# A-SHOJAEI/preference-guided-image-captioning-alignment

Measured on AMD Instinct MI355X. Metric: DPO preference-pairs/sec, CLIP-ViT-B/32+GPT-2-M seq128, higher is better.
Workload: dtype bf16; 1 GPU; Stage-2 DPO step, 4-forward policy/reference x chosen/rejected, openai/clip-vit-base-patch32 (frozen) + gpt2-medium decoder, seq_len 128, beta 0.1, bf16 MFMA / f32 accumulate+master, AdamW+clip; pairs_per_gpu=512, seq_len=128, parallelism=dp1, grad_allreduce=none (1 GPU)

## Files before the change

### include/pgca_hip.h

```cpp
#ifndef PGCA_HIP_H
#define PGCA_HIP_H

#include <stddef.h>
#include <stdint.h>

#ifdef __cplusplus
extern "C" {
#endif

typedef enum pgca_status {
  PGCA_OK = 0,
  PGCA_ERR_INVALID = -1,
  PGCA_ERR_LAUNCH = -2
} pgca_status;

#define PGCA_ABI_VERSION 306
int pgca_version(void);
int pgca_sizeof_gemm_args(void);
const char* pgca_last_error(void);

enum { PGCA_NT = 0, PGCA_NN = 1, PGCA_TN = 2 };

enum {
  PGCA_EPI_NONE = 0,
  PGCA_EPI_GELU_NEW = 1,
  PGCA_EPI_QUICK_GELU = 2,
  PGCA_EPI_RELU = 3,
  PGCA_EPI_TANH = 4,
  PGCA_EPI_DGELU_NEW = 5,
  PGCA_EPI_DRELU = 6,
  PGCA_EPI_DTANH = 7,
  PGCA_EPI_ROWSTATS = 8,
  PGCA_EPI_DLOGITS = 9,
  PGCA_EPI_DQUICK_GELU = 10,
  PGCA_EPI_GELU_NEW_D = 11,
  PGCA_EPI_MUL_AUX = 12
};

typedef struct pgca_gemm_args {
  const void* A;
  const void* B;
  int32_t M, N, K;
  int32_t lda, ldb;
  int32_t layout;
  int32_t epilogue;
  float alpha;
  const float* bias;
  void* out_bf16;
  int32_t ld_out_bf16;
  float* out_f32;
  int32_t ld_out_f32;
  int32_t accumulate;
  const float* residual;
  int32_t ld_res;
  void* aux_out;
  const void* aux_in;
  int32_t ld_aux;
  const int64_t* targets;
  float* stat_max;
  float* stat_sum;
  int32_t stat_ld;
  float* target_val;
  const float* row_lse;
  const float* row_scale;
  int32_t out_cols;
  uint32_t drop_seed;
  uint32_t drop_threshold;
  float drop_scale;
  float* colsum_part;
  int32_t ld_colsum;
  const int32_t* drop_rows;
} pgca_gemm_args;

int pgca_gemm_bf16(const pgca_gemm_args* args, void* stream);
int pgca_gemm_plan(const pgca_gemm_args* args);
int pgca_set_option(const char* name, int32_t value);
int pgca_gemm_bf16_grouped(const pgca_gemm_args* args, int32_t count, void* stream);

#define PGCA_SKINNY_MAX_M 64
typedef struct pgca_skinny_args {
  const void* x;
  const void* W;
  int32_t M, N, K, lda, ldw;
  float* scratch;
  const float* bias;
  int32_t act;
  const float* residual;
  int32_t ld_res;
  float* out_f32;
  int32_t ld_out_f32;
  void* out_bf16;
  int32_t ld_out_bf16;
  const float* ln_gamma;
  const float* ln_beta;
  float ln_eps;
  void* ln_out_bf16;
  int32_t ld_ln;
} pgca_skinny_args;
int pgca_gemm_skinny(const pgca_skinny_args* args, void* stream);
int64_t pgca_gemm_skinny_workspace(int32_t M, int32_t N, int32_t K);
int pgca_sizeof_skinny_args(void);

int pgca_rowstats_combine(const float* stat_max, const float* stat_sum, int32_t stat_ld, int32_t nparts,
                          const float* target_val, int32_t M, float* lse, float* out_logprob, void* stream);

int pgca_layernorm_fwd(const float* x, const int32_t* row_map, int32_t M, int32_t H, const float* gamma,
                       const float* beta, float eps, void* y_bf16, float* y_f32, float* mean, float* rstd,
                       void* stream);

int pgca_layernorm_bwd_blocks(int32_t M);
int pgca_layernorm_bwd(const void* dy_bf16, const float* dy_f32, const float* x, const int32_t* row_map,
                       int32_t M, int32_t H, const float* gamma, const float* mean, const float* rstd,
                       const float* add_to, float* dx_out, void* dx_bf16, float* part, float* part_extra,
                       const uint32_t* drop_add, const uint32_t* drop_dx, const int32_t* drop_rows, void* stream);
int pgca_colsum_finish(const float* part, int32_t nparts, int32_t H, float* out, int32_t accumulate, void* stream);

int pgca_colsum_finish4(const float* part, int32_t nplanes, int32_t nparts, int32_t H, float* out0, float* out1,
                        float* out2, float* out3, int32_t accumulate, void* stream);

int pgca_colsum_blocks(int32_t M);
int pgca_colsum(const void* x_bf16, const float* x_f32, int32_t M, int32_t N, int32_t ld, float* part, void* stream);

#define PGCA_ATTN_MAX_S 512
int pgca_attention_fwd(const void* qkv, const int32_t* key_mask, int32_t B, int32_t S, int32_t heads,
                       int32_t causal, void* out, float* lse, uint32_t drop_seed, uint32_t drop_threshold,
                       float drop_scale, const int32_t* cu_seqlens, void* stream);
int pgca_attention_bwd(const void* qkv, const void* out, const void* dout, const float* lse,
                       const int32_t* key_mask, int32_t B, int32_t S, int32_t heads, int32_t causal,
                       void* dqkv, uint32_t drop_seed, uint32_t drop_threshold, float drop_scale,
                       const int32_t* cu_seqlens, void* stream);
#define PGCA_ATTN_SPLIT_MAX_S 1024
int pgca_attention_bwd_split(const void* qkv, const void* out, const void* dout, const float* lse,
                             const int32_t* key_mask, int32_t B, int32_t S, int32_t heads, int32_t causal,
                             void* dqkv, uint32_t drop_seed, uint32_t drop_threshold, float drop_scale,
                             const int32_t* cu_seqlens, void* stream);

int pgca_embed_fwd(const int64_t* ids, int32_t B, int32_t S, int32_t H, const float* wte, const float* wpe,
                   const float* attended, const float* gamma, const float* beta, float eps, float* h0,
                   float* mean, float* rstd, int32_t att_stride, const float* U, int32_t xheads,
                   const uint32_t* drop_x, const uint32_t* drop_e, const int32_t* row_ids, int32_t n_rows,
                   void* stream);
int pgca_embed_bwd(const float* g, const int64_t* ids, const int32_t* row_mask, int32_t B, int32_t S, int32_t H,
                   const float* wte, const float* attended, const float* gamma, const float* mean,
                   const float* rstd, float* dwte, float* dwpe, float* dattended, float* part, int32_t att_stride,
                   const float* U, float* dU, int32_t xheads, const uint32_t* drop_x, const uint32_t* drop_e,
                   const int32_t* cu_seqlens, void* stream);
int pgca_embed_bwd_blocks(int32_t B, int32_t S);

int pgca_patchify(const float* pixels, int32_t B, int32_t image, int32_t patch, int32_t ld_out, void* out_bf16,
                  void* stream);
int pgca_vit_assemble(const float* patch_embeds, const float* cls, const float* pos, int32_t B, int32_t T,
                      int32_t H, float* x, void* stream);
int pgca_vit_assemble_bwd(const float* dx, int32_t B, int32_t T, int32_t H, void* dpatch_bf16, float* dcls,
                          float* dpos, void* stream);

int pgca_image_preprocess(const uint8_t* images, int32_t B, int32_t H, int32_t W, int32_t S, const int32_t* xbounds,
                          const int32_t* xcoef, int32_t xk, const int32_t* ybounds, const int32_t* ycoef, int32_t yk,
                          float mean0, float mean1, float mean2, float std0, float std1, float std2, uint8_t* tmp,
                          uint8_t* resized_u8, float* out, void* stream);

int pgca_image_train_transform(const uint8_t* images, int32_t B, int32_t H, int32_t W, int32_t S, const int32_t* params,
                               const float* factors, const int32_t* xbounds, const int32_t* xcoef, int32_t xk,
                               const int32_t* ybounds, const int32_t* ycoef, int32_t yk, float mean0, float mean1,
                               float mean2, float std0, float std1, float std2, uint8_t* tmp, uint8_t* resized_u8,
                               uint8_t* aug_u8, float* out, void* stream);

int pgca_seq_reduce(const float* tok_lp, const int32_t* seq_of_row, int32_t nrows, int32_t nseq,
                    const int32_t* seq_count, int32_t mode, float* seq_lp, void* stream);
int pgca_logits_logprob(const float* logits, int32_t ld, int32_t V, const int32_t* row_map, const int64_t* targets,
                        int32_t R, float* out, void* stream);
int pgca_logits_logprob_bwd(const float* logits, int32_t ld, int32_t V, const int32_t* row_map, const int64_t* targets,
                            const float* g, int32_t R, float* dlogits, void* stream);
int pgca_dpo_loss(const float* pol_w, const float* pol_l, const float* ref_w, const float* ref_l, int32_t B,
                  float beta, float label_smoothing, float* loss, float* dpol_w, float* dpol_l, float* metrics,
                  void* stream);
int pgca_seq_batch_prepare(const int64_t* ids, const int64_t* mask, int32_t Bq, int32_t S, int32_t* counts,
                           int32_t* mask32, int32_t* row_map, int64_t* targets, int32_t* seq_of_row, int32_t* n_rows,
                           void* stream);
int pgca_seq_pack_prepare(int32_t* mask32, int32_t Bq, int32_t S, int32_t pad_to, int32_t* lens, int32_t* cu,
                          int32_t* row_ids, int32_t* n_packed, const int32_t* counts, int32_t* row_map, void* stream);
int pgca_row_scale(const float* dseq, const int32_t* seq_of_row, const int32_t* seq_count, int32_t nrows,
                   int32_t mode, float* row_scale, void* stream);

int pgca_masked_mean_fwd(const float* feats, const int32_t* mask, int32_t B, int32_t S, int32_t H, float* pooled,
                         const int32_t* cu_seqlens, void* stream);
int pgca_masked_mean_bwd(const float* dpooled, const int32_t* mask, int32_t B, int32_t S, int32_t H,
                         float* dfeats, const int32_t* cu_seqlens, void* stream);
int pgca_l2norm_fwd(const float* x, int32_t B, int32_t P, float* y, float* norm, void* stream);
int pgca_l2norm_bwd(const float* dy, const float* y, const float* norm, int32_t B, int32_t P, float* dx,
                    void* stream);
int pgca_ntxent_loss(const float* lse_r, const float* lse_c, const float* diag, int32_t n_local, int32_t n_total,
                     float* loss, void* stream);

int pgca_sqnorm_blocks(int64_t n);
int pgca_sqnorm(const float* g, int64_t n, float* part, void* stream);
int pgca_step_control(const float* part, int32_t nparts, float max_norm, float base_lr, int32_t warmup,
                      int32_t total_steps, int32_t sched_stride, float beta1, float beta2, float grad_scale,
                      const float* gate, float* ctrl, void* stream);
int pgca_clip_coef(const float* part, int32_t nparts, float max_norm, float* coef, void* stream);
int pgca_scale_dev(float* x, int64_t n, const float* coef, void* stream);
int pgca_adamw(float* p, const float* g, float* m, float* v, void* p_bf16, int64_t n, const float* ctrl,
               float weight_decay, float beta1, float beta2, float eps, float grad_scale, void* stream);
int pgca_cast_bf16(const float* x, void* y_bf16, int64_t n, void* stream);
int pgca_cast_f32(const void* x_bf16, float* y, int64_t n, void* stream);
int pgca_split_bf16(const float* x, int32_t R, int32_t P, int32_t rows_out, int32_t pattern, void* y_bf16,
                    void* stream);
int pgca_axpy(const float* x, float alpha, float* y, int64_t n, int32_t accumulate, void* stream);
int pgca_gather_rows_bf16(const void* src, const int32_t* row_map, int32_t M, int32_t H, void* dst, void* stream);

int pgca_select_token(const float* logits, int32_t ld, int32_t V, int32_t R, const int64_t* prev, int32_t ld_prev,
                      int32_t n_prev, float repetition_penalty, float temperature, int32_t top_k, float top_p,
                      const float* u, const uint8_t* done, int64_t pad_id, int64_t* next, float* next_logp,
                      void* stream);
int pgca_select_beam_candidates(const float* logits, int32_t ld, int32_t V, int32_t B, int32_t nb, const int64_t* prev,
                                int32_t ld_prev, int32_t n_prev, float repetition_penalty, int32_t warp,
                                float temperature, int32_t top_k, float top_p, const float* beam_scores, int32_t K,
                                int32_t use_noise, uint32_t noise_seed, float* cand_score, int64_t* cand_index,
                                void* stream);
typedef struct pgca_select_opts {
  int32_t no_repeat_ngram_size;
  int32_t n_ban;
  const int64_t* ban_ids;
} pgca_select_opts;
int pgca_sizeof_select_opts(void);
int pgca_select_token_ex(const float* logits, int32_t ld, int32_t V, int32_t R, const int64_t* prev, int32_t ld_prev,
                         int32_t n_prev, float repetition_penalty, float temperature, int32_t top_k, float top_p,
                         const float* u, const uint8_t* done, int64_t pad_id, int64_t* next, float* next_logp,
                         const pgca_select_opts* opts, void* stream);
int pgca_select_beam_candidates_ex(const float* logits, int32_t ld, int32_t V, int32_t B, int32_t nb,
                                   const int64_t* prev, int32_t ld_prev, int32_t n_prev, float repetition_penalty,
                                   int32_t warp, float temperature, int32_t top_k, float top_p,
                                   const float* beam_scores, int32_t K, int32_t use_noise, uint32_t noise_seed,
                                   float* cand_score, int64_t* cand_index, const pgca_select_opts* opts, void* stream);
int pgca_beam_step(const float* cand_score, const int64_t* cand_index, int32_t B, int32_t nb, int32_t V, int32_t cur,
                   int32_t L, int64_t eos, float length_penalty, int32_t early_stopping, const int64_t* running_in,
                   int64_t* running_out, float* running_beam_scores, const int64_t* sequences_in,
                   int64_t* sequences_out, float* beam_scores, uint8_t* is_sent_finished, int64_t* gen_len,
                   uint8_t* unsat, int64_t* tok, int64_t* flat_src, uint8_t* hits_all, void* stream);

#ifdef __cplusplus
}
#endif
#endif
```

### preference-guided-image-captioning-alignment_amd/csrc/gemm.hip

```cpp
#include <string>

#include "gemm_device.h"

namespace {

template <int LA, int LB>
__global__ __launch_bounds__(256, 2) void gemm_kernel(const pgca_gemm_args a, int ntm, int ntn) {
  __shared__ __attribute__((aligned(16))) unsigned char smem[2][2][TILE_BYTES];

  int tm, tn;
  group_m_tile(xcd_remap(blockIdx.x, ntm * ntn), ntm, ntn, tm, tn);
  const int m0 = tm * BM, n0 = tn * BN;

  const int t = threadIdx.x;
  const int lane = t & 63, wave = t >> 6;
  const int wm = wave >> 1, wn = wave & 1;

  const bf16_t* A = reinterpret_cast<const bf16_t*>(a.A);
  const bf16_t* B = reinterpret_cast<const bf16_t*>(a.B);

  Stage<LA> sa;
  Stage<LB> sb;
  sa.init(t, a.lda, m0, LA == 0 ? a.M : ((a.M + 7) & ~7));
  sb.init(t, a.ldb, n0, LB == 0 ? a.N : ((a.N + 7) & ~7));
  const bf16_t* abase = LA == 0 ? A + (size_t)m0 * a.lda : A + m0;
  const bf16_t* bbase = LB == 0 ? B + (size_t)n0 * a.ldb : B + n0;
  const size_t astep = LA == 0 ? (size_t)BK : (size_t)BK * a.lda;
  const size_t bstep = LB == 0 ? (size_t)BK : (size_t)BK * a.ldb;

  f32x4 acc[4][4];
#pragma unroll
  for (int i = 0; i < 4; ++i)
#pragma unroll
    for (int j = 0; j < 4; ++j) acc[i][j] = (f32x4){0.f, 0.f, 0.f, 0.f};

  const int nk = (a.K + BK - 1) / BK;
  u32x4 ra[4], rb[4];
  sa.load(abase, a.K, ra);
  sb.load(bbase, a.K, rb);
  sa.store(smem[0][0], ra);
  sb.store(smem[0][1], rb);
  __syncthreads();

  for (int kt = 0; kt < nk; ++kt) {
    const int cur = kt & 1;
    const bool more = (kt + 1) < nk;
    if (more) {
      sa.load(abase + (size_t)(kt + 1) * astep, a.K - (kt + 1) * BK, ra);
      sb.load(bbase + (size_t)(kt + 1) * bstep, a.K - (kt + 1) * BK, rb);
    }
    const unsigned char* la = smem[cur][0];
    const unsigned char* lb = smem[cur][1];
#pragma unroll
    for (int kk = 0; kk < 2; ++kk) {
      bf16x8 fa[4], fb[4];
#pragma unroll
      for (int i = 0; i < 4; ++i) fa[i] = read_frag<LA>(la, wm * 64, i, kk, lane);
#pragma unroll
      for (int j = 0; j < 4; ++j) fb[j] = read_frag<LB>(lb, wn * 64, j, kk, lane);
#pragma unroll
      for (int i = 0; i < 4; ++i)
#pragma unroll
        for (int j = 0; j < 4; ++j)
          acc[i][j] = __builtin_amdgcn_mfma_f32_16x16x32_bf16(fa[i], fb[j], acc[i][j], 0, 0, 0);
    }
    if (more) {
      sa.store(smem[cur ^ 1][0], ra);
      sb.store(smem[cur ^ 1][1], rb);
    }
    __syncthreads();
  }

  run_epilogue(a, acc, &smem[0][0][0], m0 + wm * 64, n0 + wn * 64, lane, wave);
}

__global__ void rowstats_combine_kernel(const float* __restrict__ smax, const float* __restrict__ ssum, int stat_ld,
                                        int nparts, const float* __restrict__ tval, int M, float* __restrict__ lse,
                                        float* __restrict__ out_lp) {
  const int row = blockIdx.x * (blockDim.x >> 6) + (threadIdx.x >> 6);
  const int lane = threadIdx.x & 63;
  if (row >= M) return;
  float mx = -INFINITY;
  for (int i = lane; i < nparts; i += 64) mx = fmaxf(mx, smax[(size_t)row * stat_ld + i]);
  mx = wave_max(mx);
  float s = 0.f;
  for (int i = lane; i < nparts; i += 64) {
    const float pm = smax[(size_t)row * stat_ld + i];
    if (pm > -INFINITY) s += ssum[(size_t)row * stat_ld + i] * __expf(pm - mx);
  }
  s = wave_sum(s);
  if (lane == 0) {
    const float l = mx + __logf(s);
    if (lse) lse[row] = l;
    if (out_lp) out_lp[row] = tval[row] - l;
  }
}


template <int LA, int LB, bool RAW = false>
__device__ __forceinline__ void gemm256_body(const pgca_gemm_args& a, int ntm, int ntn, int nk_per_split, int bid_in,
                                             int ksplit, unsigned char* smem2) {
  int tm, tn;
  if (RAW) {
    tm = bid_in / ntn;
    tn = bid_in - tm * ntn;
  } else {
    group_m_tile(xcd_remap(bid_in, ntm * ntn), ntm, ntn, tm, tn);
  }
  const int m0 = tm * BM2, n0 = tn * BN2;

  const int t = threadIdx.x;
  const int lane = t & 63;
  const int wave = __builtin_amdgcn_readfirstlane(t >> 6);
  const int wm = wave >> 2, wn = wave & 3;

  const bf16_t* A = reinterpret_cast<const bf16_t*>(a.A);
  const bf16_t* B = reinterpret_cast<const bf16_t*>(a.B);

  Dma<LA, BK> da;
  Dma<LB, BK> db;
  da.init(lane, wave, a.lda, m0, LA == 0 ? a.M : ((a.M + 7) & ~7));
  db.init(lane, wave, a.ldb, n0, LB == 0 ? a.N : ((a.N + 7) & ~7));
  const bf16_t* abase = LA == 0 ? A + (size_t)m0 * a.lda : A + m0;
  const bf16_t* bbase = LB == 0 ? B + (size_t)n0 * a.ldb : B + n0;
  const size_t astep = LA == 0 ? (size_t)BK : (size_t)BK * a.lda;
  const size_t bstep = LB == 0 ? (size_t)BK : (size_t)BK * a.ldb;

  f32x4 acc[2][4][4];
#pragma unroll
  for (int h = 0; h < 2; ++h)
#pragma unroll
    for (int i = 0; i < 4; ++i)
#pragma unroll
      for (int j = 0; j < 4; ++j) acc[h][i][j] = (f32x4){0.f, 0.f, 0.f, 0.f};

  const int kt0 = ksplit * nk_per_split;
  const int nk = min(nk_per_split, a.K / BK - kt0);
  abase += (size_t)kt0 * astep;
  bbase += (size_t)kt0 * bstep;
#ifdef PGCA_GEMM_TIMING
  unsigned long long ts0, ts1, ts2, ts3;
#endif
  TSTAMP(ts0);
  da.issue(abase, smem2, wave);
  db.issue(bbase, smem2 + TILE2_BYTES, wave);
  dma_wait();
  __syncthreads();
  TSTAMP(ts1);

  for (int kt = 0; kt < nk; ++kt) {
    const int cur = kt & 1;
    if (kt + 1 < nk) {
      unsigned char* nxt = smem2 + (cur ^ 1) * 2 * TILE2_BYTES;
      da.issue(abase + (size_t)(kt + 1) * astep, nxt, wave);
      db.issue(bbase + (size_t)(kt + 1) * bstep, nxt + TILE2_BYTES, wave);
    }
    const unsigned char* la = smem2 + cur * 2 * TILE2_BYTES;
    const unsigned char* lb = la + TILE2_BYTES;
#pragma unroll
    for (int kk = 0; kk < 2; ++kk) {
      bf16x8 fb[4];
#pragma unroll
      for (int j = 0; j < 4; ++j) fb[j] = read_frag<LB, 512>(lb, wn * 64, j, kk, lane);
      mma_half<LA>(la, wm * 128, kk, lane, fb, acc[0]);
      mma_half<LA>(la, wm * 128 + 64, kk, lane, fb, acc[1]);
    }
    dma_wait();
    __syncthreads();
  }

  TSTAMP(ts2);
  run_epilogue(a, acc[0], smem2, m0 + wm * 128, n0 + wn * 64, lane, wave);
  run_epilogue(a, acc[1], smem2, m0 + wm * 128 + 64, n0 + wn * 64, lane, wave);
#ifdef PGCA_GEMM_TIMING
  dma_wait();
  TSTAMP(ts3);
  if (a.stat_max && a.epilogue != PGCA_EPI_ROWSTATS && lane == 0) {
    float* o = a.stat_max + ((size_t)blockIdx.x * 8 + wave) * 8;
    o[0] = (float)(ts1 - ts0); o[1] = (float)(ts2 - ts1); o[2] = (float)(ts3 - ts2); o[3] = (float)nk;
  }
#endif
}

template <int LA, int LB>
__global__ __launch_bounds__(512, 2) void gemm256_kernel(const pgca_gemm_args a, int ntm, int ntn, int nk_per_split) {
  extern __shared__ __attribute__((aligned(16))) unsigned char smem2[];
  gemm256_body<LA, LB>(a, ntm, ntn, nk_per_split, blockIdx.x, blockIdx.y, smem2);
}

struct pgca_group_param {
  pgca_gemm_args a[4];
  int start[5];
  int ntm[4], ntn[4];
};

__global__ __launch_bounds__(512, 2) void gemm256_group_tn_kernel(const pgca_group_param gp) {
  extern __shared__ __attribute__((aligned(16))) unsigned char smem2[];
  const int b = xcd_remap(blockIdx.x, gp.start[4]);
  int p = 0;
  if (b >= gp.start[1]) p = 1;
  if (b >= gp.start[2]) p = 2;
  if (b >= gp.start[3]) p = 3;
#define PGCA_SEL(F) (p == 0 ? gp.a[0].F : p == 1 ? gp.a[1].F : p == 2 ? gp.a[2].F : gp.a[3].F)
  pgca_gemm_args a = {};
  a.A = PGCA_SEL(A);
  a.B = PGCA_SEL(B);
  a.M = PGCA_SEL(M);
  a.N = PGCA_SEL(N);
  a.K = PGCA_SEL(K);
  a.lda = PGCA_SEL(lda);
  a.ldb = PGCA_SEL(ldb);
  a.out_f32 = PGCA_SEL(out_f32);
  a.ld_out_f32 = PGCA_SEL(ld_out_f32);
  a.alpha = PGCA_SEL(alpha);
  a.accumulate = PGCA_SEL(accumulate);
  a.layout = PGCA_TN;
  a.epilogue = PGCA_EPI_NONE;
#undef PGCA_SEL
  const int ntm = p == 0 ? gp.ntm[0] : p == 1 ? gp.ntm[1] : p == 2 ? gp.ntm[2] : gp.ntm[3];
  const int ntn = p == 0 ? gp.ntn[0] : p == 1 ? gp.ntn[1] : p == 2 ? gp.ntn[2] : gp.ntn[3];
  const int st = p == 0 ? gp.start[0] : p == 1 ? gp.start[1] : p == 2 ? gp.start[2] : gp.start[3];
  const int l = b - st;
  int tm, tn;
  if (ntm <= ntn) {
    tn = l / ntm;
    tm = l - tn * ntm;
  } else {
    tm = l / ntn;
    tn = l - tm * ntn;
  }
  gemm256_body<1, 1, true>(a, ntm, ntn, a.K / BK, tm * ntn + tn, 0, smem2);
}

constexpr size_t GEMM256_LDS = 4 * TILE2_BYTES;

int plan_variant(const pgca_gemm_args& a) {
  const int forced = gemm_tuning().schedule;
  if (forced >= 0) return forced == 6 ? 6 : 0;
  return a.layout == PGCA_TN ? 0 : 6;
}

}

namespace pgca {
GemmTuning& gemm_tuning() {
  static GemmTuning t = [] {
    auto env = [](const char* name, int dflt) {
      const char* e = getenv(name);
      return e ? atoi(e) : dflt;
    };
    GemmTuning v;
    v.tile = env("PGCA_GEMM_TILE", 0);
    v.schedule = env("PGCA_GEMM_RING", -1);
    v.group = env("PGCA_GEMM_NO_GROUP", 0) ? 0 : 1;
    v.stagger = env("PGCA_GEMM_STAGGER", 0);
    v.pair_order = 0;
    return v;
  }();
  return t;
}

GemmPlan plan_gemm(const pgca_gemm_args& a) {
  GemmPlan p;
  p.ncols = a.epilogue == PGCA_EPI_DLOGITS ? a.out_cols : a.N;
  const int ntm2 = (a.M + BM2 - 1) / BM2, ntn2 = (p.ncols + BN2 - 1) / BN2;
  const int force = gemm_tuning().tile;
  const int nk_total = a.K / BK;
  int splits = 1;
  const bool splittable = a.epilogue == PGCA_EPI_NONE && a.accumulate && a.out_f32 && !a.out_bf16 && !a.bias &&
                          !a.residual;
  if (splittable && ntm2 * ntn2 > 0 && ntm2 * ntn2 < 192) {
    splits = 256 / (ntm2 * ntn2);
    if (splits > nk_total / 8) splits = nk_total / 8;
    if (splits > 16) splits = 16;
    if (splits < 1) splits = 1;
  }
  const bool want256 = force ? force == 256 : (ntm2 * ntn2 * splits >= 192);
  if ((a.K % BK) == 0 && want256 && a.M >= 8 && p.ncols >= 8) {
    p.tile = 256;
    p.variant = plan_variant(a);
    p.splits = splits;
    p.ntm = ntm2;
    p.ntn = ntn2;
    p.nk_per_split = (nk_total + splits - 1) / splits;
    p.grid_y = (nk_total + p.nk_per_split - 1) / p.nk_per_split;
  } else {
    p.tile = 128;
    p.variant = 0;
    p.splits = p.grid_y = 1;
    p.ntm = (a.M + BM - 1) / BM;
    p.ntn = (p.ncols + BN - 1) / BN;
    p.nk_per_split = (a.K + BK - 1) / BK;
  }
  return p;
}
}

extern "C" int pgca_set_option(const char* name, int32_t value) {
  if (!name) {
    set_error("pgca_set_option: null name");
    return PGCA_ERR_INVALID;
  }
  GemmTuning& t = gemm_tuning();
  const std::string n(name);
  if (n == "gemm_tile" && (value == 0 || value == 128 || value == 256)) t.tile = value;
  else if (n == "gemm_schedule" && (value == -1 || value == 0 || value == 6)) t.schedule = value;
  else if (n == "gemm_group" && (value == 0 || value == 1)) t.group = value;
  else if (n == "gemm_stagger" && value >= 0 && value <= 64) t.stagger = value;
  else if (n == "gemm_pair_order" && (value == 0 || value == 1)) t.pair_order = value;
  else {
    set_error("pgca_set_option: unknown option or value out of range (%s = %d)", name, value);
    return PGCA_ERR_INVALID;
  }
  return PGCA_OK;
}

extern "C" int pgca_gemm_plan(const pgca_gemm_args* args) {
  const GemmPlan p = plan_gemm(*args);
  if (p.tile != 256) return 12801;
  return p.variant * 1000000 + 25600 + p.splits;
}

static int check_gemm_args(const pgca_gemm_args& a) {
  if (!a.A || !a.B || a.M <= 0 || a.N <= 0 || a.K <= 0) {
    set_error("pgca_gemm_bf16: null operand or empty shape (M=%d N=%d K=%d)", a.M, a.N, a.K);
    return PGCA_ERR_INVALID;
  }
  if ((a.lda & 7) || (a.ldb & 7) || ((uintptr_t)a.A & 15) || ((uintptr_t)a.B & 15)) {
    set_error("pgca_gemm_bf16: lda/ldb must be multiples of 8 and operands 16-B aligned (lda=%d ldb=%d)", a.lda,
              a.ldb);
    return PGCA_ERR_INVALID;
  }
  const bool a_kcontig = a.layout != PGCA_TN, b_kcontig = a.layout == PGCA_NT;
  if ((a_kcontig || b_kcontig) && (a.K & 7)) {
    set_error("pgca_gemm_bf16: K=%d must be a multiple of 8 for K-contiguous operands", a.K);
    return PGCA_ERR_INVALID;
  }
  if (a_kcontig ? a.lda < a.K : a.lda < ((a.M + 7) & ~7)) {
    set_error("pgca_gemm_bf16: lda=%d too small", a.lda);
    return PGCA_ERR_INVALID;
  }
  if (b_kcontig ? a.ldb < a.K : a.ldb < ((a.N + 7) & ~7)) {
    set_error("pgca_gemm_bf16: ldb=%d too small", a.ldb);
    return PGCA_ERR_INVALID;
  }
  if (a.epilogue == PGCA_EPI_ROWSTATS) {
    if (!a.stat_max || !a.stat_sum || a.stat_ld < 2 * ((a.N + BN - 1) / BN)) {
      set_error("pgca_gemm_bf16: ROWSTATS needs stat buffers with stat_ld >= %d", 2 * ((a.N + BN - 1) / BN));
      return PGCA_ERR_INVALID;
    }
  } else if (a.epilogue == PGCA_EPI_DLOGITS) {
    if (!a.row_lse || !a.row_scale || !a.targets || !a.out_bf16 || a.out_cols < a.N || a.ld_out_bf16 < a.out_cols) {
      set_error("pgca_gemm_bf16: DLOGITS needs row_lse,row_scale,targets,out_bf16 and out_cols >= N");
      return PGCA_ERR_INVALID;
    }
  } else {
    if (!a.out_bf16 && !a.out_f32) {
      set_error("pgca_gemm_bf16: no output buffer");
      return PGCA_ERR_INVALID;
    }
    if (((a.epilogue >= PGCA_EPI_DGELU_NEW && a.epilogue <= PGCA_EPI_DTANH) || a.epilogue == PGCA_EPI_DQUICK_GELU ||
         a.epilogue == PGCA_EPI_MUL_AUX) &&
        !a.aux_in) {
      set_error("pgca_gemm_bf16: derivative epilogue needs aux_in");
      return PGCA_ERR_INVALID;
    }
  }
  if (a.colsum_part && ((a.epilogue != PGCA_EPI_DGELU_NEW && a.epilogue != PGCA_EPI_MUL_AUX) || a.ld_colsum < a.N ||
                        a.accumulate == 2)) {
    set_error("pgca_gemm_bf16: colsum_part needs the DGELU_NEW / MUL_AUX epilogue, ld_colsum >= N and no split-K");
    return PGCA_ERR_INVALID;
  }
  return PGCA_OK;
}

extern "C" int pgca_gemm_bf16(const pgca_gemm_args* args, void* stream) {
  const pgca_gemm_args& a = *args;
  if (const int rc = check_gemm_args(a)) return rc;
  const GemmPlan p = plan_gemm(a);
  hipStream_t s = (hipStream_t)stream;
  if (p.tile == 128)
    return with_layout(a.layout, [&](auto la, auto lb) {
      hipLaunchKernelGGL((gemm_kernel<decltype(la)::value, decltype(lb)::value>), dim3(p.ntm * p.ntn), dim3(256), 0, s,
                         a, p.ntm, p.ntn);
      return check_launch("pgca_gemm_bf16");
    });
  pgca_gemm_args b = a;
  if (p.splits > 1) b.accumulate = 2;
  if (p.variant == 6) return launch_gemm256s(b, p, stream);
  return with_layout(a.layout, [&](auto la, auto lb) {
    constexpr auto kernel = gemm256_kernel<decltype(la)::value, decltype(lb)::value>;
    if (raise_lds_limit<kernel>(GEMM256_LDS, "gemm256")) return (int)PGCA_ERR_LAUNCH;
    hipLaunchKernelGGL(kernel, dim3(p.ntm * p.ntn, p.grid_y), dim3(512), GEMM256_LDS, s, b, p.ntm, p.ntn,
                       p.nk_per_split);
    return check_launch("pgca_gemm_bf16(256)");
  });
}

extern "C" int pgca_gemm_bf16_grouped(const pgca_gemm_args* args, int32_t count, void* stream) {
  if (!args || count <= 0) {
    set_error("pgca_gemm_bf16_grouped: no problems");
    return PGCA_ERR_INVALID;
  }
  if (count == 2 && gemm_tuning().group) {
    const pgca_gemm_args &a = args[0], &b = args[1];
    const bool alike = (a.layout == PGCA_NT || a.layout == PGCA_NN) && b.layout == a.layout && a.M == b.M &&
                       a.N == b.N && a.K == b.K && a.epilogue != PGCA_EPI_DLOGITS && b.epilogue != PGCA_EPI_DLOGITS;
    const GemmPlan pa = alike ? plan_gemm(a) : GemmPlan{}, pb = alike ? plan_gemm(b) : GemmPlan{};
    if (alike && pa.tile == 256 && pb.tile == 256 && pa.splits == 1 && pb.splits == 1 && pa.variant == 6 &&
        pb.variant == 6) {
      for (int i = 0; i < 2; ++i) {
        const int rc = check_gemm_args(args[i]);
        if (rc) return rc;
      }
      return launch_gemm256s_pair(a, b, pa, stream);
    }
  }
  bool groupable = count <= 4 && gemm_tuning().group;
  for (int i = 0; i < count && groupable; ++i) {
    const pgca_gemm_args& a = args[i];
    groupable = a.layout == PGCA_TN && (a.K % BK) == 0 && a.M >= 8 && a.N >= 8 && a.epilogue == PGCA_EPI_NONE &&
                a.out_f32 && !a.out_bf16 && !a.bias && !a.residual && !a.drop_threshold &&
                check_gemm_args(a) == PGCA_OK;
  }
  if (!groupable) {
    for (int i = 0; i < count; ++i) {
      const int rc = pgca_gemm_bf16(&args[i], stream);
      if (rc) return rc;
    }
    return PGCA_OK;
  }
  if (raise_lds_limit<gemm256_group_tn_kernel>(GEMM256_LDS, "gemm256")) return PGCA_ERR_LAUNCH;
  pgca_group_param gp;
  int total = 0;
  for (int i = 0; i < 4; ++i) {
    if (i < count) {
      gp.a[i] = args[i];
      gp.ntm[i] = (args[i].M + BM2 - 1) / BM2;
      gp.ntn[i] = (args[i].N + BN2 - 1) / BN2;
      gp.start[i] = total;
      total += gp.ntm[i] * gp.ntn[i];
    } else {
      gp.a[i] = args[count - 1];
      gp.ntm[i] = gp.ntn[i] = 1;
      gp.start[i] = 0x7fffffff;
    }
  }
  gp.start[4] = total;
  hipLaunchKernelGGL(gemm256_group_tn_kernel, dim3(total), dim3(512), GEMM256_LDS, (hipStream_t)stream, gp);
  return check_launch("pgca_gemm_bf16_grouped");
}

extern "C" int pgca_rowstats_combine(const float* stat_max, const float* stat_sum, int32_t stat_ld, int32_t nparts,
                                     const float* target_val, int32_t M, float* lse, float* out_logprob,
                                     void* stream) {
  if (!stat_max || !stat_sum || M <= 0 || nparts <= 0 || (out_logprob && !target_val)) {
    set_error("pgca_rowstats_combine: bad arguments");
    return PGCA_ERR_INVALID;
  }
  hipLaunchKernelGGL(rowstats_combine_kernel, dim3((M + 3) / 4), dim3(256), 0, (hipStream_t)stream, stat_max,
                     stat_sum, stat_ld, nparts, target_val, M, lse, out_logprob);
  return check_launch("pgca_rowstats_combine");
}
```

### preference-guided-image-captioning-alignment_amd/csrc/gemm_device.h

```cpp
#pragma once
#include <stdlib.h>

#include <type_traits>

#include "common.h"

namespace pgca {
struct GemmPlan {
  int tile;
  int variant;
  int splits;
  int ntm, ntn;
  int nk_per_split;
  int grid_y;
  int ncols;
};
GemmPlan plan_gemm(const pgca_gemm_args& a);
int launch_gemm256s(const pgca_gemm_args& a, const GemmPlan& p, void* stream);
int launch_gemm256s_pair(const pgca_gemm_args& a0, const pgca_gemm_args& a1, const GemmPlan& p, void* stream);

struct GemmTuning {
  int tile;
  int schedule;
  int group;
  int pair_order;
  int stagger;
};
GemmTuning& gemm_tuning();
}

using namespace pgca;

namespace {

template <typename F>
int with_layout(int layout, F&& f) {
  using S0 = std::integral_constant<int, 0>;
  using S1 = std::integral_constant<int, 1>;
  switch (layout) {
    case PGCA_NT: return f(S0{}, S0{});
    case PGCA_NN: return f(S0{}, S1{});
    case PGCA_TN: return f(S1{}, S1{});
    default: set_error("pgca_gemm_bf16: unknown layout %d", layout); return PGCA_ERR_INVALID;
  }
}

template <auto KERNEL>
int raise_lds_limit(size_t bytes, const char* what) {
  static const bool ok = hipFuncSetAttribute((const void*)KERNEL, hipFuncAttributeMaxDynamicSharedMemorySize,
                                             (int)bytes) == hipSuccess;
  if (!ok) {
    (void)hipGetLastError();
    set_error("%s: cannot raise dynamic LDS limit", what);
    return PGCA_ERR_LAUNCH;
  }
  return PGCA_OK;
}

constexpr int BM = 128, BN = 128, BK = 64;
constexpr int TILE_BYTES = 128 * 64 * 2;
constexpr int BM2 = 256, BN2 = 256;
constexpr int TILE2_BYTES = 256 * 64 * 2;
constexpr unsigned OOB = 0x80000000u;

__device__ __forceinline__ int xcd_remap(int b, int total) {
  const int xcd = b & 7, q = total >> 3, r = total & 7;
  return (xcd < r ? xcd * (q + 1) : r * (q + 1) + (xcd - r) * q) + (b >> 3);
}
constexpr int GROUP_M = 8;
__device__ __forceinline__ void group_m_tile(int bid, int ntm, int ntn, int& tm, int& tn) {
  const int per_group = GROUP_M * ntn;
  const int group = bid / per_group;
  const int first_m = group * GROUP_M;
  const int gsize = min(GROUP_M, ntm - first_m);
  const int in_group = bid - group * per_group;
  tm = first_m + in_group % gsize;
  tn = in_group / gsize;
}

#define PGCA_CLOCK(insn, v) asm volatile(insn " %0\n\ts_waitcnt lgkmcnt(0)" : "=s"(v)::"memory")
#ifdef PGCA_GEMM_TIMING
#define TSTAMP(v) PGCA_CLOCK("s_memtime", v)
#define TSTAMP_REAL(v) PGCA_CLOCK("s_memrealtime", v)
#else
#define TSTAMP(v)
#define TSTAMP_REAL(v)
#endif
#ifdef PGCA_GEMM_TIMING2
#define PSTAMP(v) PGCA_CLOCK("s_memtime", v)
#else
#define PSTAMP(v)
#endif

__device__ __forceinline__ __amdgpu_buffer_rsrc_t make_rsrc(const void* p) {
  return __builtin_amdgcn_make_buffer_rsrc(const_cast<void*>(p), 0, 0x7ffffff0, 0x00020000);
}

template <int KS>
struct Stage {
  unsigned goff[4];
  unsigned loff[4];
  bool vspace[4];
  int kpos[4];

  __device__ __forceinline__ void init(int t, int ld, int origin, int extent) {
    if (KS == 0) {
      const int r = t >> 3, c = t & 7;
#pragma unroll
      for (int i = 0; i < 4; ++i) {
        const int row = r + 32 * i;
        goff[i] = (unsigned)(row * ld + c * 8) * 2u;
        loff[i] = (unsigned)(row * 128 + ((c ^ (row & 7)) << 4));
        vspace[i] = (origin + row) < extent;
        kpos[i] = c * 8;
      }
    } else {
      const int kr = t >> 4, c16 = t & 15;
#pragma unroll
      for (int i = 0; i < 4; ++i) {
        const int k = kr + 16 * i;
        const int h = (k & 3) | (((k >> 3) & 1) << 2);
        goff[i] = (unsigned)(k * ld + c16 * 8) * 2u;
        loff[i] = (unsigned)(k * 256 + (((c16 >> 1) ^ h) << 5) + ((c16 & 1) << 4));
        vspace[i] = (origin + c16 * 8) < extent;
        kpos[i] = k;
      }
    }
  }
  __device__ __forceinline__ void load(const bf16_t* base, int krem, u32x4 (&r)[4]) const {
    __amdgpu_buffer_rsrc_t rs = make_rsrc(base);
#pragma unroll
    for (int i = 0; i < 4; ++i) {
      const bool ok = vspace[i] && (kpos[i] < krem);
      r[i] = __builtin_amdgcn_raw_buffer_load_b128(rs, ok ? goff[i] : OOB, 0, 0);
    }
  }
  __device__ __forceinline__ void store(unsigned char* lds, const u32x4 (&r)[4]) const {
#pragma unroll
    for (int i = 0; i < 4; ++i) *reinterpret_cast<u32x4*>(lds + loff[i]) = r[i];
  }
};

template <int KS, int KSTRIDE = 256>
__device__ __forceinline__ bf16x8 read_frag(const unsigned char* lds, int wbase, int sub, int kk, int lane) {
  if (KS == 0) {
    const int row = wbase + sub * 16 + (lane & 15);
    const int c = kk * 4 + (lane >> 4);
    return *reinterpret_cast<const bf16x8*>(lds + row * 128 + ((c ^ (lane & 7)) << 4));
  } else {
    const int g = lane >> 4, q = (lane & 15) >> 2, p = lane & 3;
    const int k = kk * 32 + 8 * g + q;
    const int h = q | ((g & 1) << 2);
    const int s32 = (wbase >> 4) + sub;
    const unsigned char* a0 = lds + k * KSTRIDE + ((s32 ^ h) << 5) + 8 * p;
    return tr_frag(a0, a0 + 4 * KSTRIDE);
  }
}

}

#include "gemm_epilogue.h"

namespace {

__device__ __forceinline__ int swz4p(int q) { return (0x78 >> (2 * q)) & 3; }

template <int KS, int BKT>
struct Dma {
  static constexpr int NP = BKT / 16;
  unsigned goff[NP];
  __device__ __forceinline__ void init(int lane, int wave, int ld, int origin, int extent) {
#pragma unroll
    for (int i = 0; i < NP; ++i) {
      const int j = wave * NP + i;
      if (KS == 0) {
        const int r = BKT == 64 ? 8 * j + (lane >> 3) : 16 * j + (lane >> 2);
        const int c = BKT == 64 ? (lane & 7) ^ (lane >> 3) : (lane & 3) ^ swz4p((lane >> 4) & 3);
        const int rg = min(origin + r, extent - 1) - origin;
        goff[i] = (unsigned)(rg * ld + c * 8) * 2u;
      } else {
        const int k = 2 * j + (lane >> 5);
        const int c16 = lane & 31;
        const int h = (k & 3) | (((k >> 3) & 1) << 2);
        const int col = (((c16 >> 1) ^ h) << 4) + ((c16 & 1) << 3);
        const int cg = min(origin + col, extent - 8) - origin;
        goff[i] = (unsigned)(k * ld + cg) * 2u;
      }
    }
  }
  __device__ __forceinline__ void issue(const bf16_t* base, unsigned char* tile, int wave) const {
    const unsigned long long b = (unsigned long long)base;
    u32x4 rs;
    rs[0] = (unsigned)b;
    rs[1] = (unsigned)(b >> 32) & 0xffffu;
    rs[2] = 0x7ffffff0u;
    rs[3] = 0x00020000u;
    const unsigned lds0 = (unsigned)(size_t)LDS_PTR(tile) + (unsigned)wave * (NP * 1024u);
#pragma unroll
    for (int i = 0; i < NP; ++i) {
      if constexpr (BKT == 64) {
        asm volatile("s_nop 4\n\ts_mov_b32 m0, %0\n\ts_nop 0\n\tbuffer_load_dwordx4 %1, %2, 0 offen lds"
                     :
                     : "s"(lds0 + i * 1024u), "v"(goff[i]), "s"(rs)
                     : "memory");
      } else {
        asm volatile("s_mov_b32 m0, %0\n\ts_nop 0\n\tbuffer_load_dwordx4 %1, %2, 0 offen lds"
                     :
                     : "s"(lds0 + i * 1024u), "v"(goff[i]), "s"(rs)
                     : "memory");
      }
    }
  }
};

__device__ __forceinline__ void dma_wait() { asm volatile("s_waitcnt vmcnt(0)" ::: "memory"); }

template <int LA>
__device__ __forceinline__ void mma_half(const unsigned char* la, int row0, int kk, int lane, const bf16x8 (&fb)[4],
                                         f32x4 (&acc)[4][4]) {
  bf16x8 fa[4];
#pragma unroll
  for (int i = 0; i < 4; ++i) fa[i] = read_frag<LA, 512>(la, row0, i, kk, lane);
#pragma unroll
  for (int i = 0; i < 4; ++i)
#pragma unroll
    for (int j = 0; j < 4; ++j) acc[i][j] = __builtin_amdgcn_mfma_f32_16x16x32_bf16(fa[i], fb[j], acc[i][j], 0, 0, 0);
}

}
```

### preference-guided-image-captioning-alignment_amd/csrc/gemm_pair.hip

```cpp
#include "gemm_phase_body.h"

namespace {

struct pgca_pair_param {
  pgca_gemm_args a[2];
  int ntm, ntn, nk, stagger;
  int order;
};

template <int LA, int LB>
__global__ __launch_bounds__(512, 2) void gemm256s_pair_kernel(const pgca_pair_param gp) {
  extern __shared__ __attribute__((aligned(16))) unsigned char smems[];
  const int ntm = gp.ntm, ntn = gp.ntn, nwg = ntm * ntn;
  const int b = xcd_remap(blockIdx.x, 2 * nwg);
  int p, bid;
  if (gp.order == 0) {
    p = b >= nwg;
    bid = b - (p ? nwg : 0);
  } else {
    const int per_group = GROUP_M * ntn;
    const int g = b / (2 * per_group);
    const int size = min(GROUP_M, ntm - g * GROUP_M) * ntn;
    const int rem = b - g * 2 * per_group;
    p = rem >= size;
    bid = g * per_group + rem - (p ? size : 0);
  }
  p = __builtin_amdgcn_readfirstlane(p);
  bid = __builtin_amdgcn_readfirstlane(bid);
  const char* kernarg = (const char*)__builtin_amdgcn_kernarg_segment_ptr();
  const pgca_gemm_args a = *(const pgca_gemm_args*)(kernarg + offsetof(pgca_pair_param, a) +
                                                    (p ? sizeof(pgca_gemm_args) : 0));
  if (a.epilogue > PGCA_EPI_TANH && a.epilogue != PGCA_EPI_GELU_NEW_D) return;
  gemm256s_body<LA, LB>(a, ntm, ntn, gp.nk, gp.stagger, bid, smems);
}

}

int pgca::launch_gemm256s_pair(const pgca_gemm_args& a0, const pgca_gemm_args& a1, const GemmPlan& p, void* stream) {
  auto forward_epilogue = [](int e) { return (e >= PGCA_EPI_NONE && e <= PGCA_EPI_TANH) || e == PGCA_EPI_GELU_NEW_D; };
  if (!forward_epilogue(a0.epilogue) || !forward_epilogue(a1.epilogue)) {
    const int rc = launch_gemm256s(a0, p, stream);
    return rc ? rc : launch_gemm256s(a1, p, stream);
  }
  pgca_pair_param gp;
  gp.a[0] = a0;
  gp.a[1] = a1;
  gp.ntm = p.ntm;
  gp.ntn = p.ntn;
  gp.nk = p.nk_per_split;
  gp.stagger = 2 * p.ntm * p.ntn >= 3 * 256 ? gemm_tuning().stagger : 0;
  gp.order = gemm_tuning().pair_order;
  auto launch = [&](auto lb) {
    constexpr auto kernel = gemm256s_pair_kernel<0, decltype(lb)::value>;
    if (raise_lds_limit<kernel>(GEMM256S_LDS, "gemm256s pair")) return (int)PGCA_ERR_LAUNCH;
    hipLaunchKernelGGL(kernel, dim3(2 * p.ntm * p.ntn), dim3(512), GEMM256S_LDS, (hipStream_t)stream, gp);
    return check_launch("pgca_gemm_bf16_grouped(256 phase-staggered pair)");
  };
  return a0.layout == PGCA_NT ? launch(std::integral_constant<int, 0>{}) : launch(std::integral_constant<int, 1>{});
}
```

### preference-guided-image-captioning-alignment_amd/csrc/gemm_phase.hip

```cpp
#include "gemm_phase_body.h"

namespace {

template <int LA, int LB>
__global__ __launch_bounds__(512, 2) void gemm256s_kernel(const pgca_gemm_args a, int ntm, int ntn, int nk_per_split,
                                                          int stagger) {
  extern __shared__ __attribute__((aligned(16))) unsigned char smems[];
  gemm256s_body<LA, LB>(a, ntm, ntn, nk_per_split, stagger, xcd_remap(blockIdx.x, ntm * ntn), smems);
}

}

int pgca::launch_gemm256s(const pgca_gemm_args& a, const GemmPlan& p, void* stream) {
  return with_layout(a.layout, [&](auto la, auto lb) {
    constexpr auto kernel = gemm256s_kernel<decltype(la)::value, decltype(lb)::value>;
    if (raise_lds_limit<kernel>(GEMM256S_LDS, "gemm256s")) return (int)PGCA_ERR_LAUNCH;
    const int stagger = (p.ntm * p.ntn >= 3 * 256 && p.grid_y == 1) ? gemm_tuning().stagger : 0;
    hipLaunchKernelGGL(kernel, dim3(p.ntm * p.ntn, p.grid_y), dim3(512), GEMM256S_LDS, (hipStream_t)stream, a, p.ntm,
                       p.ntn, p.nk_per_split, stagger);
    return check_launch("pgca_gemm_bf16(256 phase-staggered)");
  });
}
```

### preference-guided-image-captioning-alignment_amd/csrc/gemm_phase_body.h

```cpp
#pragma once
#include <stddef.h>

#include "gemm_device.h"

namespace {

constexpr int PBK = 32, PSTAGES = 4;
constexpr int PTILE_BYTES = 256 * PBK * 2;

template <int KS>
using DmaP = Dma<KS, PBK>;

template <int KS>
__device__ __forceinline__ bf16x8 read_frag_p(const unsigned char* lds, int wbase, int sub, int lane) {
  if (KS == 0) {
    const int row = wbase + sub * 16 + (lane & 15);
    const int pos = (lane >> 4) ^ swz4p((lane >> 2) & 3);
    return *reinterpret_cast<const bf16x8*>(lds + row * 64 + pos * 16);
  } else {
    return read_frag<1, 512>(lds, wbase, sub, 0, lane);
  }
}


template <int N>
__device__ __forceinline__ void wait_vm_p() {
  asm volatile("s_waitcnt vmcnt(%0)" ::"n"(N) : "memory");
}

#ifndef PGCA_FILL_L
#define PGCA_FILL_L 0
#endif
#ifndef PGCA_FILL_M
#define PGCA_FILL_M 0
#endif
template <int N>
__device__ __forceinline__ void valu_fill(float (&d)[8]) {
#pragma unroll
  for (int i = 0; i < N; ++i) asm volatile("v_fmac_f32 %0, %1, %1" : "+v"(d[i & 7]) : "v"(d[(i + 3) & 7]));
}
#define PGCA_PBAR()                       \
  do {                                    \
    __builtin_amdgcn_sched_barrier(0);    \
    __builtin_amdgcn_s_barrier();         \
    __builtin_amdgcn_sched_barrier(0);    \
  } while (0)

template <int LA, int LB>
__device__ __forceinline__ void gemm256s_body(const pgca_gemm_args& a, int ntm, int ntn, int nk_per_split, int stagger,
                                              int bid, unsigned char* smems) {
#ifdef PGCA_GEMM_TIMING
  unsigned long long ts0, ts1, ts2, ts3, tr0, tr3;
#endif
  TSTAMP(ts0);
  TSTAMP_REAL(tr0);

  if (stagger > 0 && gridDim.y == 1 && blockIdx.x < 256) {
    const int slot = (blockIdx.x >> 3) & 3;
    for (int i = 0; i < slot * stagger; ++i) __builtin_amdgcn_s_sleep(16);
  }

  int tm, tn;
  group_m_tile(bid, ntm, ntn, tm, tn);
  const int m0 = tm * BM2, n0 = tn * BN2;

  const int t = threadIdx.x;
  const int lane = t & 63;
  const int wave = __builtin_amdgcn_readfirstlane(t >> 6);
  const int wm = wave >> 2, wn = wave & 3;

  const bf16_t* A = reinterpret_cast<const bf16_t*>(a.A);
  const bf16_t* B = reinterpret_cast<const bf16_t*>(a.B);

  DmaP<LA> da;
  DmaP<LB> db;
  da.init(lane, wave, a.lda, m0, LA == 0 ? a.M : ((a.M + 7) & ~7));
  db.init(lane, wave, a.ldb, n0, LB == 0 ? a.N : ((a.N + 7) & ~7));
  const bf16_t* abase = LA == 0 ? A + (size_t)m0 * a.lda : A + m0;
  const bf16_t* bbase = LB == 0 ? B + (size_t)n0 * a.ldb : B + n0;
  const size_t astep = LA == 0 ? (size_t)PBK : (size_t)PBK * a.lda;
  const size_t bstep = LB == 0 ? (size_t)PBK : (size_t)PBK * a.ldb;

  f32x4 acc[2][4][4];
#pragma unroll
  for (int h = 0; h < 2; ++h)
#pragma unroll
    for (int i = 0; i < 4; ++i)
#pragma unroll
      for (int j = 0; j < 4; ++j) acc[h][i][j] = (f32x4){0.f, 0.f, 0.f, 0.f};

  const int kt0 = blockIdx.y * nk_per_split * 2;
  const int nk = min(nk_per_split * 2, a.K / PBK - kt0);
  abase += (size_t)kt0 * astep;
  bbase += (size_t)kt0 * bstep;

  da.issue(abase, smems, wave);
  db.issue(bbase, smems + PTILE_BYTES, wave);
  da.issue(abase + astep, smems + 2 * PTILE_BYTES, wave);
  db.issue(bbase + bstep, smems + 3 * PTILE_BYTES, wave);
  if (2 < nk) {
    da.issue(abase + 2 * astep, smems + 4 * PTILE_BYTES, wave);
    wait_vm_p<6>();
  } else {
    wait_vm_p<4>();
  }
  PGCA_PBAR();
  PGCA_PBAR();
  if (wm == 1) PGCA_PBAR();

  TSTAMP(ts1);
#ifdef PGCA_GEMM_TIMING2
  unsigned long long q0 = 0, q1 = 0, q2 = 0, q3 = 0, q4 = 0, q5 = 0, q6 = 0, q7 = 0, q8 = 0;
  unsigned long long aL0 = 0, aB1 = 0, aM0 = 0, aB2 = 0, aL1 = 0, aB3 = 0, aM1 = 0, aB4 = 0;
#endif
  float fill[8] = {1.f, 2.f, 3.f, 4.f, 5.f, 6.f, 7.f, 8.f};
  for (int kt = 0; kt < nk; ++kt) {
    PSTAMP(q0);
    const unsigned char* la = smems + (kt & 3) * 2 * PTILE_BYTES;
    const unsigned char* lb = la + PTILE_BYTES;
    bf16x8 fa[4], fb[4];
#pragma unroll
    for (int j = 0; j < 4; ++j) fb[j] = read_frag_p<LB>(lb, wn * 64, j, lane);
#pragma unroll
    for (int i = 0; i < 4; ++i) fa[i] = read_frag_p<LA>(la, wm * 128, i, lane);
    __builtin_amdgcn_sched_barrier(0);
    if (kt >= 1 && kt + 2 < nk) db.issue(bbase + (size_t)(kt + 2) * bstep, smems + ((kt + 2) & 3) * 2 * PTILE_BYTES + PTILE_BYTES, wave);
    if (kt == 0 && 2 < nk) db.issue(bbase + 2 * bstep, smems + 5 * PTILE_BYTES, wave);
    if (PGCA_FILL_L) valu_fill<PGCA_FILL_L>(fill);
    PSTAMP(q1);
    PGCA_PBAR();
    asm volatile("s_waitcnt lgkmcnt(0)" ::: "memory");
    __builtin_amdgcn_sched_barrier(0);
    PSTAMP(q2);
    __builtin_amdgcn_s_setprio(1);
#pragma unroll
    for (int i = 0; i < 4; ++i)
#pragma unroll
      for (int j = 0; j < 4; ++j) {
        acc[0][i][j] = __builtin_amdgcn_mfma_f32_16x16x32_bf16(fa[i], fb[j], acc[0][i][j], 0, 0, 0);
        if (PGCA_FILL_M) valu_fill<PGCA_FILL_M>(fill);
      }
    __builtin_amdgcn_s_setprio(0);
    PSTAMP(q3);
    PGCA_PBAR();
    PSTAMP(q4);
#pragma unroll
    for (int i = 0; i < 4; ++i) fa[i] = read_frag_p<LA>(la, wm * 128 + 64, i, lane);
    __builtin_amdgcn_sched_barrier(0);
    if (kt + 3 < nk) {
      da.issue(abase + (size_t)(kt + 3) * astep, smems + ((kt + 3) & 3) * 2 * PTILE_BYTES, wave);
      wait_vm_p<6>();
    } else if (kt + 2 < nk) {
      wait_vm_p<4>();
    } else {
      wait_vm_p<0>();
    }
    if (PGCA_FILL_L) valu_fill<PGCA_FILL_L>(fill);
    PSTAMP(q5);
    PGCA_PBAR();
    asm volatile("s_waitcnt lgkmcnt(0)" ::: "memory");
    __builtin_amdgcn_sched_barrier(0);
    PSTAMP(q6);
    __builtin_amdgcn_s_setprio(1);
#pragma unroll
    for (int i = 0; i < 4; ++i)
#pragma unroll
      for (int j = 0; j < 4; ++j) {
        acc[1][i][j] = __builtin_amdgcn_mfma_f32_16x16x32_bf16(fa[i], fb[j], acc[1][i][j], 0, 0, 0);
        if (PGCA_FILL_M) valu_fill<PGCA_FILL_M>(fill);
      }
    __builtin_amdgcn_s_setprio(0);
    PSTAMP(q7);
    PGCA_PBAR();
    PSTAMP(q8);
#ifdef PGCA_GEMM_TIMING2
    aL0 += q1 - q0; aB1 += q2 - q1; aM0 += q3 - q2; aB2 += q4 - q3;
    aL1 += q5 - q4; aB3 += q6 - q5; aM1 += q7 - q6; aB4 += q8 - q7;
#endif
  }
#ifdef PGCA_GEMM_TIMING2
  if (a.stat_sum && a.epilogue != PGCA_EPI_ROWSTATS && lane == 0) {
    float* o = a.stat_sum + ((size_t)blockIdx.x * 8 + wave) * 8;
    const float inv = 1.f / (float)nk;
    o[0] = aL0 * inv; o[1] = aB1 * inv; o[2] = aM0 * inv; o[3] = aB2 * inv;
    o[4] = aL1 * inv; o[5] = aB3 * inv; o[6] = aM1 * inv; o[7] = aB4 * inv;
  }
#endif
  if (PGCA_FILL_L || PGCA_FILL_M) {
    if (fill[0] + fill[1] + fill[2] + fill[3] + fill[4] + fill[5] + fill[6] + fill[7] == 12345.678f) acc[0][0][0][0] += 1.f;
  }
  if (wm == 0) PGCA_PBAR();
  __syncthreads();

  TSTAMP(ts2);
  run_epilogue(a, acc[0], smems, m0 + wm * 128, n0 + wn * 64, lane, wave);
  run_epilogue(a, acc[1], smems, m0 + wm * 128 + 64, n0 + wn * 64, lane, wave);
#ifdef PGCA_GEMM_TIMING
  dma_wait();
  TSTAMP(ts3);
  if (a.stat_max && a.epilogue != PGCA_EPI_ROWSTATS && lane == 0) {
    float* o = a.stat_max + ((size_t)blockIdx.x * 8 + wave) * 8;
    o[0] = (float)(ts1 - ts0); o[1] = (float)(ts2 - ts1); o[2] = (float)(ts3 - ts2); o[3] = (float)(nk / 2);
    o[4] = (float)(ts0 & 0xFFFFFFFull); o[5] = (float)(ts3 & 0xFFFFFFFull);
    TSTAMP_REAL(tr3);
    o[6] = (float)(ts3 - ts0); o[7] = (float)(tr3 - tr0);
  }
#endif
}

constexpr size_t GEMM256S_LDS = (size_t)2 * PSTAGES * PTILE_BYTES;

}
```

### preference-guided-image-captioning-alignment_amd/engine.py

```python
from __future__ import annotations

import logging
import math
import os
from contextlib import contextmanager
from dataclasses import dataclass
from types import SimpleNamespace
from typing import Dict, List, Optional, Tuple

import torch

from . import hip
from .arch import GptArch, ModelArch, VitArch
from .params import ParamStore, Segment, VOCAB_TILE

logger = logging.getLogger(__name__)

F32, BF16, I32, I64 = torch.float32, torch.bfloat16, torch.int32, torch.int64
ATTN_BWD_MAX_S = 1024
ATTN_BWD_ONEPASS_MAX_S = 512


def attention_backward(qkv, out, dout, lse, key_mask, B, S, heads, causal, dqkv, drop=None, cu=None):
    fn = hip.attention_bwd if S <= ATTN_BWD_ONEPASS_MAX_S else hip.attention_bwd_split
    fn(qkv, out, dout, lse, key_mask, B, S, heads, causal, dqkv, drop=drop, cu=cu)


class Workspace:

    GROW = 1.125

    def __init__(self, device):
        self.device = torch.device(device)
        self.bufs: Dict[str, torch.Tensor] = {}
        self._stamps: Dict[str, tuple] = {}
        self.serial: Dict[str, int] = {}
        self._recorders: List[set] = []

    def _touch(self, key: str, fresh: bool) -> None:
        if fresh:
            self.serial[key] = self.serial.get(key, 0) + 1
        for r in self._recorders:
            r.add(key)

    def get(self, key: str, shape, dtype, zero: bool = False) -> torch.Tensor:
        shape = tuple(int(s) for s in shape)
        n = 1
        for s in shape:
            n *= s
        t = self.bufs.get(key)
        fresh = t is None or t.dtype != dtype or t.numel() < n
        if fresh:
            grow = t is not None and t.dtype == dtype
            t = torch.empty(max(int(n * self.GROW) if grow else n, 1), dtype=dtype, device=self.device)
            self.bufs[key] = t
        self._touch(key, fresh)
        v = t[:n].view(shape)
        if zero:
            v.zero_()
        return v

    def cached(self, key: str, stamp: tuple, make) -> torch.Tensor:
        fresh = key not in self.bufs or self._stamps.get(key) != stamp
        if fresh:
            self.bufs[key] = make()
            self._stamps[key] = stamp
        self._touch(key, fresh)
        return self.bufs[key]

    @contextmanager
    def recording(self):
        keys: set = set()
        self._recorders.append(keys)
        try:
            yield keys
        finally:
            self._recorders.remove(keys)

    def stamp(self, keys) -> tuple:
        return tuple((k, self.serial.get(k, 0)) for k in sorted(keys))

    def nbytes(self) -> int:
        return sum(t.numel() * t.element_size() for t in self.bufs.values())


KIND_EMBD, KIND_ATTN, KIND_RESID_ATTN, KIND_RESID_MLP, KIND_VPROJ, KIND_XATTN, KIND_HEAD = range(7)
TOWER_DECODER, TOWER_TEXT, TOWER_VHEAD, TOWER_THEAD = range(4)
_M32 = 0xFFFFFFFF


def _hash32(x: int) -> int:
    x &= _M32
    x ^= x >> 16
    x = (x * 0x7FEB352D) & _M32
    x ^= x >> 15
    x = (x * 0x846CA68B) & _M32
    x ^= x >> 16
    return x


class DropoutPlan:

    GPT_KINDS = (KIND_EMBD, KIND_ATTN, KIND_RESID_ATTN, KIND_RESID_MLP)

    def __init__(self, p: float = 0.0, base_seed: int = 0, p_gpt: Optional[float] = None):
        self.p, self.base_seed, self.step, self.active = float(p), int(base_seed), 0, True
        self.p_gpt = float(p) if p_gpt is None else float(p_gpt)

    def _p(self, kind: int) -> float:
        return self.p_gpt if kind in self.GPT_KINDS else self.p

    def _site(self, step: int, tower: int, layer: int, kind: int):
        seed = _hash32(_hash32(self.base_seed * 0x9E3779B1 + step) ^ ((tower << 24) | ((layer & 0xFFFF) << 8) | kind))
        return hip.drop_args(seed, self._p(kind))

    @property
    def on(self) -> bool:
        return self.active and (self.p > 0.0 or self.p_gpt > 0.0)

    def site(self, tower: int, layer: int, kind: int):
        if not self.on:
            return None
        return self._site(self.step, tower, layer, kind)

    def bind(self, tower: int):
        if not self.on:
            return None
        step = self.step
        return lambda layer, kind: self._site(step, tower, layer, kind)


PACK_PAD = 64


@dataclass
class RowPack:
    cu: torch.Tensor
    row_ids: torch.Tensor
    mask: torch.Tensor
    lens: torch.Tensor
    n: int
    Mp: int
    Bq: int
    S: int

    @property
    def nseq(self) -> int:
        return self.Bq + n_filler_seqs(self.S)


def n_filler_seqs(S: int) -> int:
    return (PACK_PAD - 1 + S - 1) // S


@dataclass
class SeqBatch:
    ids: torch.Tensor
    mask: torch.Tensor
    row_map: torch.Tensor
    targets: torch.Tensor
    seq_of_row: torch.Tensor
    counts: torch.Tensor
    n_rows: int
    Bq: int
    S: int
    pack: Optional[RowPack] = None
    row_map_packed: Optional[torch.Tensor] = None


class PendingRowPack:

    def __init__(self, mask1, lens, cu, row_ids, n_host, event, Bq, S):
        self._f, self._n, self._ev, self.Bq, self.S = (mask1, lens, cu, row_ids), n_host, event, Bq, S

    def result(self) -> RowPack:
        self._ev.synchronize()
        n, Mp = int(self._n[0]), int(self._n[1])
        mask1, lens, cu, row_ids = self._f
        return RowPack(cu=cu, row_ids=row_ids[:max(Mp, 1)], mask=mask1, lens=lens, n=n, Mp=Mp, Bq=self.Bq, S=self.S)


def _issue_pack(mask1: torch.Tensor, Bq: int, S: int, counts=None, row_map=None):
    dev = mask1.device
    cap = (Bq * S + PACK_PAD - 1) // PACK_PAD * PACK_PAD
    lens = torch.empty(Bq, dtype=I32, device=dev)
    cu = torch.empty(Bq + n_filler_seqs(S) + 1, dtype=I32, device=dev)
    row_ids = torch.empty(cap, dtype=I32, device=dev)
    n_dev = torch.empty(2, dtype=I32, device=dev)
    hip.seq_pack_prepare(mask1, Bq, S, PACK_PAD, lens, cu, row_ids, n_dev, counts=counts, row_map=row_map)
    return lens, cu, row_ids, n_dev


def prepare_row_pack_async(mask32: torch.Tensor) -> PendingRowPack:
    Bq, S = mask32.shape
    mask1 = torch.empty(Bq + n_filler_seqs(S), S, dtype=I32, device=mask32.device)
    mask1[:Bq].copy_(mask32)
    lens, cu, row_ids, n_dev = _issue_pack(mask1, Bq, S)
    n_host = torch.empty(2, dtype=I32, pin_memory=True)
    n_host.copy_(n_dev, non_blocking=True)
    ev = torch.cuda.Event()
    ev.record()
    return PendingRowPack(mask1, lens, cu, row_ids, n_host, ev, Bq, S)


def make_row_pack(mask32: torch.Tensor) -> RowPack:
    return prepare_row_pack_async(mask32).result()


class PendingSeqBatch:

    def __init__(self, ids, mask1, row_map, targets, seq_of_row, counts, n_host, event, Bq, S, pack=None):
        self._f = (ids, mask1, row_map, targets, seq_of_row, counts)
        self._n, self._ev, self.Bq, self.S, self._pack = n_host, event, Bq, S, pack

    def result(self) -> "SeqBatch":
        self._ev.synchronize()
        n = int(self._n[0])
        if n <= 0:
            raise ValueError("no scored token in the batch (every caption has <= 1 real token)")
        ids, mask1, row_map, targets, seq_of_row, counts = self._f
        pack, rmp = None, None
        if self._pack is not None:
            lens, cu, row_ids, rmp = self._pack
            npk, Mp = int(self._n[1]), int(self._n[2])
            pack = RowPack(cu=cu, row_ids=row_ids[:Mp], mask=mask1, lens=lens, n=npk, Mp=Mp, Bq=self.Bq, S=self.S)
            rmp = rmp[:n]
        return SeqBatch(ids=ids, mask=mask1[:self.Bq], row_map=row_map[:n], targets=targets[:n],
                        seq_of_row=seq_of_row[:n], counts=counts, n_rows=n, Bq=self.Bq, S=self.S, pack=pack,
                        row_map_packed=rmp)


def prepare_seq_batch_async(ids: torch.Tensor, mask: torch.Tensor, device, pack: bool = True) -> PendingSeqBatch:
    dev = torch.device(device)
    ids_d = ids.detach().to(dev, I64, non_blocking=True).contiguous()
    mask_d = mask.detach().to(dev, I64, non_blocking=True).contiguous()
    Bq, S = ids_d.shape
    if S < 2:
        raise ValueError("sequences need at least 2 positions (the first token is never scored)")
    cap = Bq * (S - 1)
    mask1 = torch.empty(Bq + n_filler_seqs(S), S, dtype=I32, device=dev)
    counts = torch.empty(Bq, dtype=I32, device=dev)
    row_map = torch.empty(cap, dtype=I32, device=dev)
    targets = torch.empty(cap, dtype=I64, device=dev)
    seq_of_row = torch.empty(cap, dtype=I32, device=dev)
    n_dev = torch.empty(3, dtype=I32, device=dev)
    hip.seq_batch_prepare(ids_d, mask_d, Bq, S, counts, mask1, row_map, targets, seq_of_row, n_dev)
    pk = None
    if pack:
        rmp = row_map.clone()
        lens, cu, row_ids, n2 = _issue_pack(mask1, Bq, S, counts=counts, row_map=rmp)
        n_dev[1:].copy_(n2)
        pk = (lens, cu, row_ids, rmp)
    n_host = torch.empty(3, dtype=I32, pin_memory=True)
    n_host.copy_(n_dev, non_blocking=True)
    ev = torch.cuda.Event()
    ev.record()
    return PendingSeqBatch(ids_d, mask1, row_map, targets, seq_of_row, counts, n_host, ev, Bq, S, pk)


def make_seq_batch(ids: torch.Tensor, mask: torch.Tensor, device, pack: bool = True) -> SeqBatch:
    return prepare_seq_batch_async(ids, mask, device, pack).result()


def _bias_grad(ws: Workspace, M: int, N: int, ld: int, gout: torch.Tensor, x_bf16=None, x_f32=None) -> None:
    nb = hip.colsum_blocks(M)
    part = ws.get("colsum_part", (nb, N), F32)
    hip.colsum(M, N, ld, part, x_bf16=x_bf16, x_f32=x_f32)
    hip.colsum_finish(part, nb, N, gout, accumulate=True)


def _ln_param_grads(part: torch.Tensor, nb: int, H: int, *outs: torch.Tensor) -> None:
    hip.colsum_finish4(part, len(outs), nb, H, outs, accumulate=True)


def _rows(pack: Optional[RowPack], Bq: int, S: int) -> SimpleNamespace:
    if pack is None:
        return SimpleNamespace(M=Bq * S, cu=None, ids=None, nseq=Bq, embed={})
    return SimpleNamespace(M=pack.Mp, cu=pack.cu, ids=pack.row_ids, nseq=pack.nseq,
                           embed=dict(row_ids=pack.row_ids, n_rows=pack.Mp))


def _dsite(drop, layer: int, kind: int):
    return drop(layer, kind) if drop is not None else None


class _P:
    __slots__ = ("w", "b", "g")

    def __init__(self, seg: Segment, name: Optional[str], at=None):
        offset, shape = at if at is not None else seg.index[name]
        n = math.prod(shape)
        self.w, self.b, self.g = (None if flat is None else flat[offset:offset + n].view(shape)
                                  for flat in (seg.fp32, seg.bf16, seg.grad))

    @classmethod
    def span(cls, seg: Segment, offset: int, shape) -> "_P":
        return cls(seg, None, (offset, tuple(shape)))


RECOMPUTE_MODES = ("none", "mlp", "block")


def check_recompute(mode) -> str:
    if mode not in RECOMPUTE_MODES:
        raise ValueError(f"recompute must be one of {RECOMPUTE_MODES}, got {mode!r}")
    return mode


@dataclass
class DecodeState:
    kv: List[torch.Tensor]
    kv_all: torch.Tensor
    att: torch.Tensor
    cu: torch.Tensor
    R: int
    smax: int
    t: int = 0
    lnf_done: bool = False
    keys: frozenset = frozenset()


def _drive(steps):
    while True:
        try:
            args, kw = next(steps)
        except StopIteration as e:
            return e.value
        hip.gemm(*args, **kw)


def _drive_pair(steps0, steps1):
    out = [None, None]
    while True:
        g = []
        for i, steps in enumerate((steps0, steps1)):
            try:
                g.append(next(steps))
            except StopIteration as e:
                out[i] = e.value
        if not g:
            return out
        if len(g) != 2:
            raise RuntimeError("paired forward: the two trunks do not have the same sequence of GEMMs")
        hip.gemm_pair(g[0], g[1])


class GptTrunk:

    GELU_PAIR = os.environ.get("PGCA_GELU_PAIR", "1") != "0"

    def __init__(self, store: ParamStore, prefix: str, arch: GptArch, ws: Workspace, tag: str):
        self.arch, self.ws, self.tag = arch, ws, tag
        seg = store.seg_of(prefix + ".ln_f.weight")
        self.seg = seg
        self.layers = []
        for i in range(arch.layers):
            p = f"{prefix}.h.{i}"
            self.layers.append({k: _P(seg, p + n) for k, n in (
                ("ln1w", ".ln_1.weight"), ("ln1b", ".ln_1.bias"), ("wqkv", ".attn.c_attn.weight"),
                ("bqkv", ".attn.c_attn.bias"), ("wo", ".attn.c_proj.weight"), ("bo", ".attn.c_proj.bias"),
                ("ln2w", ".ln_2.weight"), ("ln2b", ".ln_2.bias"), ("wfc", ".mlp.c_fc.weight"),
                ("bfc", ".mlp.c_fc.bias"), ("wpr", ".mlp.c_proj.weight"), ("bpr", ".mlp.c_proj.bias"))})
        self.lnf_w, self.lnf_b = _P(seg, prefix + ".ln_f.weight"), _P(seg, prefix + ".ln_f.bias")
        self.saved: Optional[dict] = None
        starts = [seg.index[f"{prefix}.h.{i}.ln_1.weight"][0] for i in range(arch.layers)]
        starts.append(seg.index[prefix + ".ln_f.weight"][0])
        self.layer_ranges = [(starts[i], starts[i + 1]) for i in range(arch.layers)]
        self.grad_hook = None
        self.overlap_wgrad = True
        self._recompute_mode = "none"
        self._wgrad_stream: Optional[torch.cuda.Stream] = None

    @property
    def recompute(self) -> str:
        return self._recompute_mode

    @recompute.setter
    def recompute(self, mode: str) -> None:
        self._recompute_mode = check_recompute(mode)
        self.saved = None

    def _buf(self, name, shape, dtype, zero=False):
        return self.ws.get(f"{self.tag}.{name}", shape, dtype, zero)

    def forward(self, h0: torch.Tensor, mask: Optional[torch.Tensor], Bq: int, S: int, save: bool,
                drop=None, pack: Optional[RowPack] = None) -> torch.Tensor:
        return _drive(self.forward_steps(h0, mask, Bq, S, save, drop, pack))

    def forward_steps(self, h0: torch.Tensor, mask: Optional[torch.Tensor], Bq: int, S: int, save: bool,
                      drop=None, pack: Optional[RowPack] = None):
        a, H = self.arch, self.arch.hidden
        if S > a.n_pos:
            raise ValueError(f"sequence length {S} exceeds GPT-2's {a.n_pos} learned positions")
        if save and S > ATTN_BWD_MAX_S:
            raise ValueError(f"training needs sequence length <= {ATTN_BWD_MAX_S} (the longest the attention backward is "
                             f"built and tested for); got {S}")
        rw = _rows(pack, Bq, S)
        M = rw.M
        if pack is not None:
            mask = pack.mask
        sv = {"M": M, "Bq": Bq, "S": S, "mask": mask, "drop": drop, "pack": pack} if save else None
        h = h0
        for li in range(len(self.layers)):
            hn = self._buf(f"l{li + 1}.hin", (M, H), F32) if save else None
            s, hn = yield from self._layer_steps(li, h, rw, mask, S, drop, save, hn=hn)
            if save:
                sv[li] = s if self.recompute == "none" else {k: s[k] for k in self._KEPT[self.recompute]}
            h = hn
        if save:
            sv["hL"] = h
            self.saved = sv
        return h

    _KEPT = {"mlp": ("hin", "ln1", "m1", "r1", "qkv", "att", "lse", "hm", "m2", "r2"), "block": ("hin",)}
    _WGRAD_OPERANDS = ("ln1", "att", "ln2", "act")

    def _key(self, li: int, name: str, save: bool) -> str:
        if not save:
            return name
        if self.recompute == "none" or name in self._KEPT[self.recompute]:
            return f"l{li}.{name}"
        return (f"rc{li & 1}." if name in self._WGRAD_OPERANDS else "rc.") + name

    def _layer_fwd(self, *args, **kw):
        return _drive(self._layer_steps(*args, **kw))

    def _layer_steps(self, li: int, h: torch.Tensor, rw: SimpleNamespace, mask, S: int, drop, save: bool,
                     hn: Optional[torch.Tensor] = None, hm: Optional[torch.Tensor] = None, proj: bool = True):
        a, H, I = self.arch, self.arch.hidden, self.arch.inner
        P, M = self.layers[li], rw.M
        s = {"hin": h}

        def buf(name, shape, dtype):
            s[name] = self._buf(self._key(li, name, save), shape, dtype)
            return s[name]

        if hm is None:
            ln1, m1, r1 = buf("ln1", (M, H), BF16), buf("m1", (M,), F32), buf("r1", (M,), F32)
            hip.layernorm_fwd(h, M, H, P["ln1w"].w, P["ln1b"].w, a.eps, y_bf16=ln1, mean=m1, rstd=r1)
            qkv = buf("qkv", (M, 3 * H), BF16)
            yield (ln1, P["wqkv"].b, M, 3 * H, H, hip.NN), dict(bias=P["bqkv"].w, out_bf16=qkv)
            att = buf("att", (M, H), BF16)
            lse = buf("lse", (rw.nseq, a.heads, S), F32)
            hip.attention_fwd(qkv, mask, rw.nseq, S, a.heads, True, att, lse, drop=_dsite(drop, li, KIND_ATTN), cu=rw.cu)
            hm = buf("hm", (M, H), F32) if save else h
            yield (att, P["wo"].b, M, H, H, hip.NN), dict(bias=P["bo"].w, residual=h, out_f32=hm,
                                                          drop=_dsite(drop, li, KIND_RESID_ATTN), drop_rows=rw.ids)
        s["hm"] = hm
        ln2, m2, r2 = buf("ln2", (M, H), BF16), buf("m2", (M,), F32), buf("r2", (M,), F32)
        hip.layernorm_fwd(hm, M, H, P["ln2w"].w, P["ln2b"].w, a.eps, y_bf16=ln2, mean=m2, rstd=r2)
        act = buf("act", (M, I), BF16)
        pre = buf("pre", (M, I), BF16) if save else None
        s["pre"] = pre
        yield (ln2, P["wfc"].b, M, I, H, hip.NN), dict(
            epilogue=hip.EPI_GELU_NEW_D if (save and self.GELU_PAIR) else hip.EPI_GELU_NEW,
            bias=P["bfc"].w, out_bf16=act, aux_out=pre)
        if not proj:
            return s, None
        if hn is None:
            hn = hm
        yield (act, P["wpr"].b, M, H, I, hip.NN), dict(bias=P["bpr"].w, residual=hm, out_f32=hn,
                                                       drop=_dsite(drop, li, KIND_RESID_MLP), drop_rows=rw.ids)
        return s, hn

    def _recompute(self, li: int, sv: dict, rw: SimpleNamespace) -> dict:
        kept = sv[li]
        s, _ = self._layer_fwd(li, kept["hin"], rw, sv["mask"], sv["S"], sv["drop"], True,
                               hm=kept.get("hm"), proj=False)
        return {**s, **kept}

    SKINNY_ROWS = 32

    def decode_cache(self, R: int, smax: int) -> DecodeState:
        a, H = self.arch, self.arch.hidden
        if smax > a.n_pos:
            raise ValueError(f"{smax} positions exceed GPT-2's {a.n_pos} learned positions")
        kv_all = self._buf("gen.kv", (len(self.layers), R * smax, 3 * H), BF16)
        att = self._buf("gen.att", (R * smax, H), BF16)
        cu = self.ws.cached(f"{self.tag}.gen.cu.{R}x{smax}", (R, smax),
                            lambda: (torch.arange(R + 1, dtype=I32, device=self.ws.device) * smax).contiguous())
        return DecodeState(kv=list(kv_all), kv_all=kv_all, att=att, cu=cu, R=R, smax=smax)

    def decode_step(self, x: torch.Tensor, st: DecodeState, t: int) -> torch.Tensor:
        a, H, I = self.arch, self.arch.hidden, self.arch.inner
        R, smax = st.R, st.smax
        if not 0 <= t < smax:
            raise ValueError(f"position {t} outside the cache ({smax})")
        y = self._buf("gen.y", (R, H), BF16)
        act = self._buf("gen.act", (R, I), BF16)
        att = st.att
        att_t = att.view(-1)[t * H:]
        L = len(self.layers)
        if R <= min(self.SKINNY_ROWS, hip.SKINNY_MAX_M) and I <= 8192 and 3 * H <= 8192:
            need = max(hip.gemm_skinny_workspace(R, n, k) for n, k in ((3 * H, H), (H, H), (I, H), (H, I))) // 4
            sc = self._buf("gen.scratch", (need,), F32)
            P0 = self.layers[0]
            hip.layernorm_fwd(x, R, H, P0["ln1w"].w, P0["ln1b"].w, a.eps, y_bf16=y)
            for li, P in enumerate(self.layers):
                kv = st.kv[li]
                hip.gemm_skinny(y, P["wqkv"].b, R, 3 * H, H, sc, bias=P["bqkv"].w, out_bf16=kv.view(-1)[t * 3 * H:],
                                ld_out_bf16=smax * 3 * H)
                hip.attention_fwd(kv, None, R, t + 1, a.heads, True, att, None, cu=st.cu)
                hip.gemm_skinny(att_t, P["wo"].b, R, H, H, sc, lda=smax * H, bias=P["bo"].w, residual=x, out_f32=x,
                                ln=(P["ln2w"].w, P["ln2b"].w, a.eps), ln_out=y)
                hip.gemm_skinny(y, P["wfc"].b, R, I, H, sc, bias=P["bfc"].w, act=hip.EPI_GELU_NEW, out_bf16=act)
                nxt = (self.layers[li + 1]["ln1w"].w, self.layers[li + 1]["ln1b"].w) if li + 1 < L else \
                    (self.lnf_w.w, self.lnf_b.w)
                hip.gemm_skinny(act, P["wpr"].b, R, H, I, sc, bias=P["bpr"].w, residual=x, out_f32=x,
                                ln=(nxt[0], nxt[1], a.eps), ln_out=y)
            st.lnf_done = True
            return x
        st.lnf_done = False
        for li, P in enumerate(self.layers):
            kv = st.kv[li]
            hip.layernorm_fwd(x, R, H, P["ln1w"].w, P["ln1b"].w, a.eps, y_bf16=y)
            hip.gemm(y, P["wqkv"].b, R, 3 * H, H, hip.NN, bias=P["bqkv"].w, out_bf16=kv.view(-1)[t * 3 * H:],
                     ld_out_bf16=smax * 3 * H)
            hip.attention_fwd(kv, None, R, t + 1, a.heads, True, att, None, cu=st.cu)
            hip.gemm(att_t, P["wo"].b, R, H, H, hip.NN, lda=smax * H, bias=P["bo"].w, residual=x, out_f32=x)
            hip.layernorm_fwd(x, R, H, P["ln2w"].w, P["ln2b"].w, a.eps, y_bf16=y)
            hip.gemm(y, P["wfc"].b, R, I, H, hip.NN, epilogue=hip.EPI_GELU_NEW, bias=P["bfc"].w, out_bf16=act)
            hip.gemm(act, P["wpr"].b, R, H, I, hip.NN, bias=P["bpr"].w, residual=x, out_f32=x)
        return x

    def decode_reorder(self, st: DecodeState, src: torch.Tensor) -> None:
        v = st.kv_all.view(len(self.layers), st.R, st.smax, -1)[:, :, :st.t + 1]
        v.copy_(v.index_select(1, src))

    def top_drop(self):
        drop = self.saved.get("drop") if self.saved else None
        return drop(len(self.layers) - 1, KIND_RESID_MLP) if drop is not None else None

    def backward(self, g: torch.Tensor, g_bf: torch.Tensor) -> torch.Tensor:
        sv = self.saved
        assert sv is not None, "forward(save=True) must precede backward"
        a, H, I = self.arch, self.arch.hidden, self.arch.inner
        M, Bq, S = sv["M"], sv["Bq"], sv["S"]
        rw = _rows(sv["pack"], Bq, S)
        ws = self.ws
        nb = hip.layernorm_bwd_blocks(M)
        part4 = ws.get("ln_part", (4, nb, H), F32)
        part, partx = part4[:2], part4[2:]
        drop = sv["drop"]
        L = len(self.layers)
        main = torch.cuda.current_stream()
        side = None
        if self.overlap_wgrad and g.is_cuda:
            if self._wgrad_stream is None:
                self._wgrad_stream = torch.cuda.Stream()
            side = self._wgrad_stream
        done: Dict[int, torch.cuda.Event] = {}

        def settle(layer: int) -> None:
            ev = done.pop(layer, None)
            if ev is not None:
                main.wait_event(ev)
                if self.grad_hook is not None:
                    self.grad_hook(layer)

        for li in range(L - 1, -1, -1):
            P = self.layers[li]
            par = "1" if (li & 1) else "0"
            settle(li + 2)
            s = sv[li] if self.recompute == "none" else self._recompute(li, sv, rw)
            dpre = self._buf("dpre" + par, (M, I), BF16)
            nbr = (M + 63) // 64
            dpre_cs = self._buf("dpre_colsum", (nbr, I), F32)
            hip.gemm(g_bf, P["wpr"].b, M, I, H, hip.NT, epilogue=hip.EPI_MUL_AUX if self.GELU_PAIR else hip.EPI_DGELU_NEW,
                     aux_in=s["pre"], out_bf16=dpre, colsum_part=dpre_cs)
            hip.colsum_finish(dpre_cs, nbr, I, P["bfc"].g, accumulate=True)
            wgrads = [(s["act"], g_bf, I, H, M, P["wpr"].g)]
            dln = self._buf("dln", (M, H), BF16)
            hip.gemm(dpre, P["wfc"].b, M, H, I, hip.NT, out_bf16=dln)
            wgrads.append((s["ln2"], dpre, H, I, M, P["wfc"].g))
            g2 = self._buf("g_b" if (li & 1) else "g_a", (M, H), F32)
            g2_bf = self._buf("gbf_b" if (li & 1) else "gbf_a", (M, H), BF16)
            hip.layernorm_bwd(s["hm"], M, H, P["ln2w"].w, s["m2"], s["r2"], g2, dy_bf16=dln, add_to=g, dx_bf16=g2_bf,
                              part=part, part_extra=partx, drop_add=_dsite(drop, li, KIND_RESID_MLP),
                              drop_dx=_dsite(drop, li, KIND_RESID_ATTN), drop_rows=rw.ids)
            _ln_param_grads(part4, nb, H, P["ln2w"].g, P["ln2b"].g, P["bpr"].g, P["bo"].g)
            datt = self._buf("datt", (M, H), BF16)
            hip.gemm(g2_bf, P["wo"].b, M, H, H, hip.NT, out_bf16=datt)
            wgrads.append((s["att"], g2_bf, H, H, M, P["wo"].g))
            dqkv = self._buf("dqkv" + par, (M, 3 * H), BF16)
            attention_backward(s["qkv"], s["att"], datt, s["lse"], sv["mask"], rw.nseq, S, a.heads, True, dqkv,
                               drop=_dsite(drop, li, KIND_ATTN), cu=rw.cu)
            hip.gemm(dqkv, P["wqkv"].b, M, H, 3 * H, hip.NT, out_bf16=dln)
            wgrads.append((s["ln1"], dqkv, H, 3 * H, M, P["wqkv"].g))
            if side is not None:
                side.wait_stream(main)
                with torch.cuda.stream(side):
                    hip.gemm_wgrad_group(wgrads)
                    ev = torch.cuda.Event()
                    ev.record(side)
                done[li] = ev
            else:
                hip.gemm_wgrad_group(wgrads)
            _bias_grad(ws, M, 3 * H, 3 * H, P["bqkv"].g, x_bf16=dqkv)
            g3 = self._buf("g_c" if (li & 1) else "g_d", (M, H), F32)
            g3_bf = self._buf("gbf_c" if (li & 1) else "gbf_d", (M, H), BF16)
            settle(li + 1)
            hip.layernorm_bwd(s["hin"], M, H, P["ln1w"].w, s["m1"], s["r1"], g3, dy_bf16=dln, add_to=g2,
                              dx_bf16=g3_bf, part=part,
                              drop_dx=_dsite(drop, li - 1, KIND_RESID_MLP) if li > 0 else None, drop_rows=rw.ids)
            _ln_param_grads(part, nb, H, P["ln1w"].g, P["ln1b"].g)
            g, g_bf = g3, g3_bf
            if side is None and self.grad_hook is not None:
                self.grad_hook(li)
        for layer in sorted(done, reverse=True):
            settle(layer)
        return g


class ProjHead:

    def __init__(self, store: ParamStore, prefix: str, in_dim: int, proj: int, ws: Workspace, tag: str):
        seg = store.seg_of(prefix + ".0.weight")
        self.seg, self.ws, self.tag, self.inn, self.P = seg, ws, tag, in_dim, proj
        self.w0, self.b0 = _P(seg, prefix + ".0.weight"), _P(seg, prefix + ".0.bias")
        self.w3, self.b3 = _P(seg, prefix + ".3.weight"), _P(seg, prefix + ".3.bias")
        self.lnw, self.lnb = _P(seg, prefix + ".4.weight"), _P(seg, prefix + ".4.bias")
        self.saved = None

    def forward(self, x_bf: torch.Tensor, B: int, save: bool, drop=None) -> torch.Tensor:
        ws, t, Pd = self.ws, self.tag, self.P
        h1 = ws.get(t + ".h1", (B, Pd), BF16)
        hip.gemm(x_bf, self.w0.b, B, Pd, self.inn, hip.NT, epilogue=hip.EPI_RELU, bias=self.b0.w, out_bf16=h1,
                 drop=drop)
        h2 = ws.get(t + ".h2", (B, Pd), F32)
        hip.gemm(h1, self.w3.b, B, Pd, Pd, hip.NT, bias=self.b3.w, out_f32=h2)
        emb = ws.get(t + ".emb", (B, Pd), F32)
        mean, rstd = ws.get(t + ".mean", (B,), F32), ws.get(t + ".rstd", (B,), F32)
        hip.layernorm_fwd(h2, B, Pd, self.lnw.w, self.lnb.w, 1e-5, y_f32=emb, mean=mean, rstd=rstd)
        if save:
            self.saved = dict(x=x_bf, h1=h1, h2=h2, mean=mean, rstd=rstd, B=B, drop=drop)
        return emb

    def backward(self, demb: torch.Tensor, need_dx: bool) -> Optional[torch.Tensor]:
        s, ws, t, Pd = self.saved, self.ws, self.tag, self.P
        B = s["B"]
        nb = hip.layernorm_bwd_blocks(B)
        part = ws.get("ln_part_small", (2, nb, Pd), F32)
        dh2 = ws.get(t + ".dh2", (B, Pd), F32)
        dh2_bf = ws.get(t + ".dh2bf", (B, Pd), BF16)
        hip.layernorm_bwd(s["h2"], B, Pd, self.lnw.w, s["mean"], s["rstd"], dh2, dy_f32=demb, dx_bf16=dh2_bf, part=part)
        _ln_param_grads(part, nb, Pd, self.lnw.g, self.lnb.g)
        hip.gemm(dh2_bf, s["h1"], Pd, Pd, B, hip.TN, lda=Pd, ldb=Pd, out_f32=self.w3.g, accumulate=True)
        _bias_grad(ws, B, Pd, Pd, self.b3.g, x_f32=dh2)
        dh1 = ws.get(t + ".dh1", (B, Pd), BF16)
        hip.gemm(dh2_bf, self.w3.b, B, Pd, Pd, hip.NN, epilogue=hip.EPI_DRELU, aux_in=s["h1"], out_bf16=dh1,
                 drop=s["drop"])
        hip.gemm(dh1, s["x"], Pd, self.inn, B, hip.TN, lda=Pd, ldb=self.inn, out_f32=self.w0.g, accumulate=True)
        _bias_grad(ws, B, Pd, Pd, self.b0.g, x_bf16=dh1)
        if not need_dx:
            return None
        dx = ws.get(t + ".dx", (B, self.inn), F32)
        hip.gemm(dh1, self.w0.b, B, self.inn, Pd, hip.NN, out_f32=dx)
        return dx


class VisionTower:

    def __init__(self, store: ParamStore, arch: VitArch, ws: Workspace):
        self.arch, self.ws = arch, ws
        p = "vision_encoder.vision_model"
        seg = store.seg_of(p + ".post_layernorm.weight")
        self.seg = seg
        self.trainable = seg.grad is not None
        self.cls, self.pos, self.wpatch, self.pre_w, self.pre_b, self.post_w, self.post_b = (_P(seg, p + n) for n in (
            ".embeddings.class_embedding", ".embeddings.position_embedding.weight", ".embeddings.patch_embedding.weight",
            ".pre_layrnorm.weight", ".pre_layrnorm.bias", ".post_layernorm.weight", ".post_layernorm.bias"))
        self.patch_k = arch.patch_dim if arch.patch_dim % 8 == 0 else (arch.patch_dim + 63) // 64 * 64
        self._wpatch_pad, self._wpatch_ver = None, -1
        H = arch.hidden
        self.layers = []
        for i in range(arch.layers):
            q = f"{p}.encoder.layers.{i}"
            wq_off = seg.index[q + ".self_attn.q_proj.weight"][0]
            bq_off = seg.index[q + ".self_attn.q_proj.bias"][0]
            assert seg.index[q + ".self_attn.v_proj.weight"][0] == wq_off + 2 * H * H, "q,k,v must be contiguous"
            assert seg.index[q + ".self_attn.v_proj.bias"][0] == bq_off + 2 * H
            L = {k: _P(seg, q + n) for k, n in (
                ("wo", ".self_attn.out_proj.weight"), ("bo", ".self_attn.out_proj.bias"),
                ("ln1w", ".layer_norm1.weight"), ("ln1b", ".layer_norm1.bias"),
                ("ln2w", ".layer_norm2.weight"), ("ln2b", ".layer_norm2.bias"),
                ("w1", ".mlp.fc1.weight"), ("b1", ".mlp.fc1.bias"), ("w2", ".mlp.fc2.weight"), ("b2", ".mlp.fc2.bias"))}
            L["wqkv"], L["bqkv"] = _P.span(seg, wq_off, (3 * H, H)), _P.span(seg, bq_off, (3 * H,))
            self.layers.append(L)
        self.saved: Optional[dict] = None

    def _patch_weight(self) -> torch.Tensor:
        w = self.wpatch.b.view(self.arch.hidden, self.arch.patch_dim)
        if self.patch_k == self.arch.patch_dim:
            return w
        if self._wpatch_pad is None or self._wpatch_ver != self.seg.bf16_version:
            if self._wpatch_pad is None:
                self._wpatch_pad = torch.zeros(self.arch.hidden, self.patch_k, dtype=BF16, device=self.ws.device)
            self._wpatch_pad[:, :self.arch.patch_dim].copy_(w)
            self._wpatch_ver = self.seg.bf16_version
        return self._wpatch_pad

    def forward(self, pixels: torch.Tensor, save: bool = False) -> Tuple[torch.Tensor, torch.Tensor, torch.Tensor]:
        a, ws = self.arch, self.ws
        save = bool(save) and self.trainable
        B = pixels.shape[0]
        H, T, G, D = a.hidden, a.tokens, a.grid, a.patch_dim
        if save and T > ATTN_BWD_MAX_S:
            raise ValueError(f"a trainable vision tower needs <= {ATTN_BWD_MAX_S} tokens per image (the longest the "
                             f"attention backward is built and tested for); got {T}")
        M = B * T
        Kp = self.patch_k
        cols = ws.get("vit.cols", (B * G * G, Kp), BF16)
        hip.patchify(pixels, B, a.image, a.patch, cols, ld_out=Kp)
        pe = ws.get("vit.pe", (B * G * G, H), F32)
        hip.gemm(cols, self._patch_weight(), B * G * G, H, Kp, hip.NT, out_f32=pe)
        x0 = ws.get("vit.x0", (M, H), F32)
        hip.vit_assemble(pe, self.cls.w, self.pos.w, B, T, H, x0)
        x = ws.get("vit.x", (M, H), F32)
        m0, r0 = (ws.get(n, (M,), F32) if save else None for n in ("vit.m0", "vit.r0"))
        hip.layernorm_fwd(x0, M, H, self.pre_w.w, self.pre_b.w, a.eps, y_f32=x, mean=m0, rstd=r0)
        sv = dict(B=B, M=M, cols=cols, x0=x0, m0=m0, r0=r0) if save else None
        for li, P in enumerate(self.layers):
            k = f"vit.l{li}." if save else "vit."
            y = ws.get(k + "y", (M, H), BF16)
            qkv = ws.get(k + "qkv", (M, 3 * H), BF16)
            att = ws.get(k + "att", (M, H), BF16)
            act = ws.get(k + "act", (M, a.mlp), BF16)
            m1, r1, m2, r2 = (ws.get(k + n, (M,), F32) if save else None for n in ("m1", "r1", "m2", "r2"))
            lse = ws.get(k + "lse", (B, a.heads, T), F32) if save else None
            hip.layernorm_fwd(x, M, H, P["ln1w"].w, P["ln1b"].w, a.eps, y_bf16=y, mean=m1, rstd=r1)
            hip.gemm(y, P["wqkv"].b, M, 3 * H, H, hip.NT, bias=P["bqkv"].w, out_bf16=qkv)
            hip.attention_fwd(qkv, None, B, T, a.heads, False, att, lse)
            xm = ws.get(k + "xm", (M, H), F32) if save else x
            hip.gemm(att, P["wo"].b, M, H, H, hip.NT, bias=P["bo"].w, residual=x, out_f32=xm)
            y2 = ws.get(k + "y2", (M, H), BF16) if save else y
            hip.layernorm_fwd(xm, M, H, P["ln2w"].w, P["ln2b"].w, a.eps, y_bf16=y2, mean=m2, rstd=r2)
            pre = ws.get(k + "pre", (M, a.mlp), BF16) if save else None
            hip.gemm(y2, P["w1"].b, M, a.mlp, H, hip.NT, epilogue=hip.EPI_QUICK_GELU, bias=P["b1"].w, out_bf16=act,
                     aux_out=pre)
            xn = ws.get(f"vit.l{li + 1}.xin", (M, H), F32) if save else x
            hip.gemm(act, P["w2"].b, M, H, a.mlp, hip.NT, bias=P["b2"].w, residual=xm, out_f32=xn)
            if save:
                sv[li] = dict(xin=x, y1=y, qkv=qkv, att=att, act=act, m1=m1, r1=r1, m2=m2, r2=r2, lse=lse, xm=xm, y2=y2,
                              pre=pre)
            x = xn
        cls_rows = ws.cached("vit.clsrows", (B, T), lambda: (torch.arange(B, dtype=I32, device=ws.device) * T).contiguous())
        pooled = ws.get("vit.pooled", (B, H), F32)
        pooled_bf = ws.get("vit.pooledbf", (B, H), BF16)
        mp, rp = (ws.get(n, (B,), F32) if save else None for n in ("vit.mp", "vit.rp"))
        hip.layernorm_fwd(x, B, H, self.post_w.w, self.post_b.w, a.eps, row_map=cls_rows, y_f32=pooled, y_bf16=pooled_bf,
                          mean=mp, rstd=rp)
        if save:
            sv.update(xL=x, cls_rows=cls_rows, mp=mp, rp=rp)
        self.saved = sv
        return x.view(B, T, H), pooled, pooled_bf

    def backward(self, dpooled: torch.Tensor) -> None:
        sv = self.saved
        if sv is None:
            raise RuntimeError("VisionTower.backward needs forward(save=True) on a trainable tower")
        a, ws = self.arch, self.ws
        B, M = sv["B"], sv["M"]
        H, T, I = a.hidden, a.tokens, a.mlp
        nb = hip.layernorm_bwd_blocks(M)
        part = ws.get("vit.ln_part", (2, nb, H), F32)
        g = ws.get("vit.g_a", (M, H), F32)
        g.zero_()
        nbp = hip.layernorm_bwd_blocks(B)
        partp = ws.get("vit.ln_part_cls", (2, nbp, H), F32)
        hip.layernorm_bwd(sv["xL"], B, H, self.post_w.w, sv["mp"], sv["rp"], g, dy_f32=dpooled, row_map=sv["cls_rows"],
                          part=partp)
        _ln_param_grads(partp, nbp, H, self.post_w.g, self.post_b.g)
        g_bf = ws.get("vit.gbf_a", (M, H), BF16)
        hip.cast_bf16(g, g_bf, M * H)
        dpre = ws.get("vit.dpre", (M, I), BF16)
        dln = ws.get("vit.dln", (M, H), BF16)
        datt = ws.get("vit.datt", (M, H), BF16)
        dqkv = ws.get("vit.dqkv", (M, 3 * H), BF16)
        for li in range(len(self.layers) - 1, -1, -1):
            P, s = self.layers[li], sv[li]
            hip.gemm(g_bf, P["w2"].b, M, I, H, hip.NN, epilogue=hip.EPI_DQUICK_GELU, aux_in=s["pre"], out_bf16=dpre)
            hip.gemm(g_bf, s["act"], H, I, M, hip.TN, lda=H, ldb=I, out_f32=P["w2"].g, accumulate=True)
            _bias_grad(ws, M, H, H, P["b2"].g, x_f32=g)
            hip.gemm(dpre, P["w1"].b, M, H, I, hip.NN, out_bf16=dln)
            hip.gemm(dpre, s["y2"], I, H, M, hip.TN, lda=I, ldb=H, out_f32=P["w1"].g, accumulate=True)
            _bias_grad(ws, M, I, I, P["b1"].g, x_bf16=dpre)
            g2 = ws.get("vit.g_b", (M, H), F32)
            g2_bf = ws.get("vit.gbf_b", (M, H), BF16)
            hip.layernorm_bwd(s["xm"], M, H, P["ln2w"].w, s["m2"], s["r2"], g2, dy_bf16=dln, add_to=g, dx_bf16=g2_bf,
                              part=part)
            _ln_param_grads(part, nb, H, P["ln2w"].g, P["ln2b"].g)
            hip.gemm(g2_bf, P["wo"].b, M, H, H, hip.NN, out_bf16=datt)
            hip.gemm(g2_bf, s["att"], H, H, M, hip.TN, lda=H, ldb=H, out_f32=P["wo"].g, accumulate=True)
            _bias_grad(ws, M, H, H, P["bo"].g, x_f32=g2)
            attention_backward(s["qkv"], s["att"], datt, s["lse"], None, B, T, a.heads, False, dqkv)
            hip.gemm(dqkv, P["wqkv"].b, M, H, 3 * H, hip.NN, out_bf16=dln)
            hip.gemm(dqkv, s["y1"], 3 * H, H, M, hip.TN, lda=3 * H, ldb=H, out_f32=P["wqkv"].g, accumulate=True)
            _bias_grad(ws, M, 3 * H, 3 * H, P["bqkv"].g, x_bf16=dqkv)
            hip.layernorm_bwd(s["xin"], M, H, P["ln1w"].w, s["m1"], s["r1"], g, dy_bf16=dln, add_to=g2, dx_bf16=g_bf,
                              part=part)
            _ln_param_grads(part, nb, H, P["ln1w"].g, P["ln1b"].g)
        dx0 = ws.get("vit.g_b", (M, H), F32)
        hip.layernorm_bwd(sv["x0"], M, H, self.pre_w.w, sv["m0"], sv["r0"], dx0, dy_f32=g, part=part)
        _ln_param_grads(part, nb, H, self.pre_w.g, self.pre_b.g)
        Np, D, Kp = B * (T - 1), a.patch_dim, self.patch_k
        dpe = ws.get("vit.dpe", (Np, H), BF16)
        hip.vit_assemble_bwd(dx0, B, T, H, dpe, self.cls.g, self.pos.g)
        hip.gemm(dpe, sv["cols"], H, D, Np, hip.TN, lda=H, ldb=Kp, out_f32=self.wpatch.g.view(H, D),
                 accumulate=True)


class CaptionDecoderEngine:

    LM_CHUNK = int(os.environ.get("PGCA_LM_CHUNK", "8192"))

    def __init__(self, store: ParamStore, arch: ModelArch, ws: Workspace, tag: str):
        self.arch, self.ws, self.tag = arch, ws, tag
        g = arch.gpt
        p = "caption_decoder"
        t = p + ".lm_model.transformer"
        seg = store.seg_of(t + ".wte.weight")
        self.seg = seg
        self.trunk = GptTrunk(store, t, g, ws, tag + ".trunk")
        self.wte, self.wpe = _P(seg, t + ".wte.weight"), _P(seg, t + ".wpe.weight")
        self.V = arch.dec_vocab
        self.Vp = (self.V + VOCAB_TILE - 1) // VOCAB_TILE * VOCAB_TILE
        self.wte_pad_bf = seg.padded(seg.bf16, t + ".wte.weight")
        self.vp_w, self.vp_b = _P(seg, p + ".vision_projection.0.weight"), _P(seg, p + ".vision_projection.0.bias")
        self.inw, self.inb = _P(seg, p + ".cross_attention.in_proj_weight"), _P(seg, p + ".cross_attention.in_proj_bias")
        self.ow, self.ob = _P(seg, p + ".cross_attention.out_proj.weight"), _P(seg, p + ".cross_attention.out_proj.bias")
        self.anw, self.anb = _P(seg, p + ".attention_norm.weight"), _P(seg, p + ".attention_norm.bias")
        self.saved = None
        self._dec: Optional[DecodeState] = None
        self._graphs: dict = {}
        self.graph_captures = 0
        self.graph_replays = 0

    def _buf(self, name, shape, dtype, zero=False):
        return self.ws.get(f"{self.tag}.{name}", shape, dtype, zero)

    def _prefix(self, emb: torch.Tensor, Bq: int, drop=None):
        H, Pd, XH = self.arch.gpt.hidden, self.arch.proj_dim, self.arch.xattn_heads
        dh = H // XH
        emb_bf = self._buf("emb_bf", (Bq, Pd), BF16)
        hip.cast_bf16(emb, emb_bf, Bq * Pd)
        pv = self._buf("pv", (Bq, H), BF16)
        pv_raw = self._buf("pv_raw", (Bq, H), BF16) if drop is not None else None
        hip.gemm(emb_bf, self.vp_w.b, Bq, H, Pd, hip.NT, epilogue=hip.EPI_TANH, bias=self.vp_b.w, out_bf16=pv,
                 aux_out=pv_raw, drop=_dsite(drop, 0, KIND_VPROJ))
        vv = self._buf("vv", (Bq, H), BF16)
        hip.gemm(pv, self.inw.b[2 * H:], Bq, H, H, hip.NT, bias=self.inb.w[2 * H:], out_bf16=vv)
        if drop is None:
            att = self._buf("attended", (Bq, H), F32)
            hip.gemm(vv, self.ow.b, Bq, H, H, hip.NT, bias=self.ob.w, out_f32=att)
            return dict(emb_bf=emb_bf, pv=pv, pv_raw=pv, vv=vv, att=att, U=None)
        U = self._buf("U", (Bq, XH, H), F32)
        for h in range(XH):
            hip.gemm(vv[:, h * dh:], self.ow.b[:, h * dh:], Bq, H, dh, hip.NT, lda=H, ldb=H, out_f32=U[:, h],
                     ld_out_f32=XH * H)
        return dict(emb_bf=emb_bf, pv=pv, pv_raw=pv_raw, vv=vv, att=None, U=U)

    def hidden(self, emb: torch.Tensor, sb: SeqBatch, save: bool, drop=None, packed: bool = False) -> torch.Tensor:
        Bq, S = sb.Bq, sb.S
        pack = sb.pack if packed else None
        if packed and pack is None:
            raise ValueError("packed=True needs a SeqBatch prepared with pack=True")
        h0, keep = self._embed(emb, sb, drop, pack)
        hL = self.trunk.forward(h0, sb.mask, Bq, S, save, drop, pack=pack)
        if save:
            self.saved = dict(hL=hL, **keep)
        return hL

    def _embed(self, emb: torch.Tensor, sb: SeqBatch, drop, pack: Optional[RowPack]):
        H, Bq, S, XH = self.arch.gpt.hidden, sb.Bq, sb.S, self.arch.xattn_heads
        rw = _rows(pack, Bq, S)
        M = rw.M
        pf = self._prefix(emb, Bq, drop)
        h0 = self._buf("h0", (M, H), F32)
        m0, r0 = self._buf("m0", (M,), F32), self._buf("r0", (M,), F32)
        if drop is None:
            hip.embed_fwd(sb.ids, Bq, S, H, self.wte.w, self.wpe.w, h0, attended=pf["att"], gamma=self.anw.w,
                          beta=self.anb.w, eps=1e-5, mean=m0, rstd=r0, **rw.embed)
        else:
            hip.embed_fwd(sb.ids, Bq, S, H, self.wte.w, self.wpe.w, h0, attended=self.ob.w, att_stride=0,
                          gamma=self.anw.w, beta=self.anb.w, eps=1e-5, mean=m0, rstd=r0, U=pf["U"], xheads=XH,
                          drop_x=drop(0, KIND_XATTN), drop_e=drop(0, KIND_EMBD), **rw.embed)
        return h0, dict(sb=sb, m0=m0, r0=r0, drop=drop, pack=pack, **pf)

    def token_logprobs(self, hL: torch.Tensor, sb: SeqBatch, save: bool, packed: bool = False) -> torch.Tensor:
        a = self.arch.gpt
        H, Mc = a.hidden, sb.n_rows
        hf = self._buf("hf", (Mc, H), BF16)
        mf, rf = self._buf("mf", (Mc,), F32), self._buf("rf", (Mc,), F32)
        hip.layernorm_fwd(hL, Mc, H, self.trunk.lnf_w.w, self.trunk.lnf_b.w, a.eps,
                          row_map=sb.row_map_packed if packed else sb.row_map, y_bf16=hf, mean=mf, rstd=rf)
        nparts = 2 * (self.Vp // 128)
        smax = self._buf("smax", (Mc, nparts), F32)
        ssum = self._buf("ssum", (Mc, nparts), F32)
        tval = self._buf("tval", (Mc,), F32)
        hip.gemm(hf, self.wte.b, Mc, self.V, H, hip.NT, epilogue=hip.EPI_ROWSTATS, targets=sb.targets, stat_max=smax,
                 stat_sum=ssum, stat_ld=nparts, target_val=tval)
        lse = self._buf("lse", (Mc,), F32)
        tok = self._buf("tok_lp", (Mc,), F32)
        hip.rowstats_combine(smax, ssum, nparts, 2 * ((self.V + 127) // 128), tval, Mc, lse=lse, out_logprob=tok)
        if save:
            self.saved.update(hf=hf, mf=mf, rf=rf, lse=lse)
        return tok

    def sequence_logprobs(self, emb: torch.Tensor, sb: SeqBatch, reduce: str, save: bool, drop=None,
                          packed: Optional[bool] = None) -> torch.Tensor:
        packed = (sb.pack is not None) if packed is None else bool(packed)
        return self._reduce(self.hidden(emb, sb, save, drop, packed), sb, reduce, save, packed)

    def _reduce(self, hL: torch.Tensor, sb: SeqBatch, reduce: str, save: bool, packed: bool) -> torch.Tensor:
        tok = self.token_logprobs(hL, sb, save, packed)
        out = self._buf("seq_lp", (sb.Bq,), F32)
        hip.seq_reduce(tok, sb.seq_of_row, sb.n_rows, sb.Bq, sb.counts, 1 if reduce == "mean" else 0, out)
        if save:
            self.saved["reduce"] = reduce
        return out

    @staticmethod
    def sequence_logprobs_pair(pol: "CaptionDecoderEngine", ref: "CaptionDecoderEngine", emb: torch.Tensor,
                               remb: torch.Tensor, sb: SeqBatch, reduce: str, save: bool, drop, packed: bool):
        pack = sb.pack if packed else None
        if packed and pack is None:
            raise ValueError("packed=True needs a SeqBatch prepared with pack=True")
        rh0, _ = ref._embed(remb, sb, None, pack)
        h0, keep = pol._embed(emb, sb, drop, pack)
        hL, rhL = _drive_pair(pol.trunk.forward_steps(h0, sb.mask, sb.Bq, sb.S, save, drop, pack=pack),
                              ref.trunk.forward_steps(rh0, sb.mask, sb.Bq, sb.S, False, None, pack=pack))
        if save:
            pol.saved = dict(hL=hL, **keep)
        ref_lp = ref._reduce(rhL, sb, reduce, False, packed)
        return pol._reduce(hL, sb, reduce, save, packed), ref_lp

    def logits(self, emb: torch.Tensor, sb: SeqBatch) -> torch.Tensor:
        a = self.arch.gpt
        H, M = a.hidden, sb.Bq * sb.S
        hL = self.hidden(emb, sb, False)
        hf = self._buf("hf_full", (M, H), BF16)
        hip.layernorm_fwd(hL, M, H, self.trunk.lnf_w.w, self.trunk.lnf_b.w, a.eps, y_bf16=hf)
        out = torch.empty(M, self.V, dtype=F32, device=self.ws.device)
        hip.gemm(hf, self.wte.b, M, self.V, H, hip.NT, out_f32=out)
        return out.view(sb.Bq, sb.S, self.V)

    def prefix_embedding(self, emb: torch.Tensor) -> torch.Tensor:
        B = emb.shape[0]
        H, Pd = self.arch.gpt.hidden, self.arch.proj_dim
        emb_bf = self._buf("gen.emb_bf", (B, Pd), BF16)
        hip.cast_bf16(emb.contiguous(), emb_bf, B * Pd)
        pv = torch.empty(B, H, dtype=F32, device=self.ws.device)
        hip.gemm(emb_bf, self.vp_w.b, B, H, Pd, hip.NT, epilogue=hip.EPI_TANH, bias=self.vp_b.w, out_f32=pv)
        return pv

    def next_token_logits(self, pv: torch.Tensor, ids: torch.Tensor) -> torch.Tensor:
        a = self.arch.gpt
        B, t = ids.shape
        H, S = a.hidden, t + 1
        full = torch.zeros(B, S, dtype=I64, device=self.ws.device)
        if t:
            full[:, 1:] = ids
        h0 = self._buf("gen.h0", (B * S, H), F32)
        hip.embed_fwd(full, B, S, H, self.wte.w, self.wpe.w, h0)
        h0.view(B, S, H)[:, 0, :] = pv + self.wpe.w[0]
        hL = self.trunk.forward(h0, None, B, S, save=False)
        rows = (torch.arange(B, dtype=I32, device=self.ws.device) * S + (S - 1)).contiguous()
        hf = self._buf("gen.hf", (B, H), BF16)
        hip.layernorm_fwd(hL, B, H, self.trunk.lnf_w.w, self.trunk.lnf_b.w, a.eps, row_map=rows, y_bf16=hf)
        ldv = (self.V + 3) // 4 * 4
        out = torch.empty(B, ldv, dtype=F32, device=self.ws.device)
        hip.gemm(hf, self.wte.b, B, self.V, H, hip.NT, out_f32=out, ld_out_f32=ldv)
        return out[:, :self.V]

    def decode_begin(self, pv: torch.Tensor, max_positions: int) -> torch.Tensor:
        R = pv.shape[0]
        with self.ws.recording() as keys:
            self._dec = self.trunk.decode_cache(R, int(max_positions))
            x = self._buf("gen.x", (R, self.arch.gpt.hidden), F32)
            torch.add(pv, self.wpe.w[0], out=x)
            out = self._decode_logits(x)
        self._dec.keys = frozenset(keys)
        return out

    use_graphs = True

    def _advance_eager(self, tok: torch.Tensor, t: int) -> torch.Tensor:
        st = self._dec
        x = self._buf("gen.x", (st.R, self.arch.gpt.hidden), F32)
        torch.index_select(self.wte.w, 0, tok, out=x)
        x.add_(self.wpe.w[t])
        return self._decode_logits(x)

    def _graph_stamp(self, keys) -> tuple:
        return (self.ws.stamp(keys), self.seg.bf16.data_ptr(), self.wte.w.data_ptr(), self.wpe.w.data_ptr())

    def decode_advance(self, tokens: torch.Tensor) -> torch.Tensor:
        st = self._dec
        st.t += 1
        t = st.t
        if not (self.use_graphs and tokens.is_cuda):
            return self._advance_eager(tokens, t)
        with self.ws.recording() as keys:
            tok_in = self._buf("gen.tok_in", (st.R,), I64)
        tok_in.copy_(tokens)
        cache = self._graphs
        key = (st.R, st.smax, t)
        g = cache.get(key)
        if g is not None:
            if g[2] == self._graph_stamp(g[3]):
                g[0].replay()
                self.graph_replays += 1
                return g[1]
            for k in [k for k, v in cache.items() if v[2] != self._graph_stamp(v[3])]:
                del cache[k]
        with self.ws.recording() as step_keys:
            out = self._advance_eager(tok_in, t)
        keys = frozenset(keys | st.keys | step_keys)
        try:
            graph = torch.cuda.CUDAGraph()
            with torch.cuda.graph(graph):
                out_g = self._advance_eager(tok_in, t)
            cache[key] = (graph, out_g, self._graph_stamp(keys), keys)
            self.graph_captures += 1
        except Exception as e:
            logger.warning("decode graphs turned off, every step now launches eagerly: capturing step %d of a %d x %d "
                           "decode raised %s: %s", t, st.R, st.smax, type(e).__name__, e)
            self.use_graphs = False
            torch.cuda.synchronize()
        return out

    def decode_reorder(self, src: torch.Tensor) -> None:
        self.trunk.decode_reorder(self._dec, src)

    def _decode_logits(self, x: torch.Tensor) -> torch.Tensor:
        a, st = self.arch.gpt, self._dec
        R, H = st.R, a.hidden
        self.trunk.decode_step(x, st, st.t)
        if st.lnf_done:
            hf = self.trunk._buf("gen.y", (R, H), BF16)
        else:
            hf = self._buf("gen.hf", (R, H), BF16)
            hip.layernorm_fwd(x, R, H, self.trunk.lnf_w.w, self.trunk.lnf_b.w, a.eps, y_bf16=hf)
        ldv = (self.V + 3) // 4 * 4
        out = self._buf("gen.logits", (R, ldv), F32)
        hip.gemm(hf, self.wte.b, R, self.V, H, hip.NT, out_f32=out, ld_out_f32=ldv)
        return out[:, :self.V]

    def backward(self, dseq: torch.Tensor) -> torch.Tensor:
        s = self.saved
        sb: SeqBatch = s["sb"]
        a = self.arch.gpt
        H, Pd, Bq, S, Mc = a.hidden, self.arch.proj_dim, sb.Bq, sb.S, sb.n_rows
        pack: Optional[RowPack] = s["pack"]
        rw = _rows(pack, Bq, S)
        M = rw.M
        ws = self.ws
        rs = self._buf("row_scale", (Mc,), F32)
        hip.row_scale(dseq, sb.seq_of_row, sb.counts, Mc, (1 if s["reduce"] == "mean" else 0) | 2, rs)
        dhf = self._buf("dhf32", (Mc, H), F32, zero=True)
        ck = min(self.LM_CHUNK, Mc)
        dl = self._buf("dlogits", (ck, self.Vp), BF16)
        for r0 in range(0, Mc, ck):
            n = min(ck, Mc - r0)
            hfc = s["hf"][r0:r0 + n]
            hip.gemm(hfc, self.wte.b, n, self.V, H, hip.NT, epilogue=hip.EPI_DLOGITS, targets=sb.targets[r0:r0 + n],
                     row_lse=s["lse"][r0:r0 + n], row_scale=rs[r0:r0 + n], out_bf16=dl, ld_out_bf16=self.Vp,
                     out_cols=self.Vp)
            hip.gemm(dl, self.wte_pad_bf, n, H, self.Vp, hip.NN, lda=self.Vp, ldb=H, out_f32=dhf[r0:r0 + n], accumulate=True)
            hip.gemm(dl, hfc, self.V, H, n, hip.TN, lda=self.Vp, ldb=H, out_f32=self.wte.g, accumulate=True)
        g = self.trunk._buf("g_top", (M, H), F32, zero=True)
        g_bf = self.trunk._buf("gbf_top", (M, H), BF16, zero=True)
        nb = hip.layernorm_bwd_blocks(Mc)
        part = ws.get("ln_part_f", (2, nb, H), F32)
        hip.layernorm_bwd(s["hL"], Mc, H, self.trunk.lnf_w.w, s["mf"], s["rf"], g, dy_f32=dhf,
                          row_map=sb.row_map_packed if pack is not None else sb.row_map, dx_bf16=g_bf, part=part,
                          drop_dx=self.trunk.top_drop(), drop_rows=rw.ids)
        _ln_param_grads(part, nb, H, self.trunk.lnf_w.g, self.trunk.lnf_b.g)
        g0 = self.trunk.backward(g, g_bf)
        drop = s["drop"]
        XH = self.arch.xattn_heads
        dh = H // XH
        datt = self._buf("datt", (Bq, H), F32, zero=True)
        nbe = hip.embed_bwd_blocks(Bq, S)
        parte = ws.get("ln_part_e", (2, nbe, H), F32)
        dvv = self._buf("dvv", (Bq, H), BF16)
        if drop is None:
            hip.embed_bwd(g0, sb.ids, sb.mask, Bq, S, H, self.wte.g, self.wpe.g, wte=self.wte.w, attended=s["att"],
                          gamma=self.anw.w, mean=s["m0"], rstd=s["r0"], dattended=datt, part=parte, cu=rw.cu)
            _ln_param_grads(parte, nbe, H, self.anw.g, self.anb.g)
            datt_bf = self._buf("datt_bf", (Bq, H), BF16)
            hip.cast_bf16(datt, datt_bf, Bq * H)
            hip.gemm(datt_bf, s["vv"], H, H, Bq, hip.TN, lda=H, ldb=H, out_f32=self.ow.g, accumulate=True)
            _bias_grad(ws, Bq, H, H, self.ob.g, x_f32=datt)
            hip.gemm(datt_bf, self.ow.b, Bq, H, H, hip.NN, out_bf16=dvv)
        else:
            dU = self._buf("dU", (Bq, XH, H), F32, zero=True)
            hip.embed_bwd(g0, sb.ids, sb.mask, Bq, S, H, self.wte.g, self.wpe.g, wte=self.wte.w, attended=self.ob.w,
                          att_stride=0, gamma=self.anw.w, mean=s["m0"], rstd=s["r0"], dattended=datt, part=parte,
                          U=s["U"], dU=dU, xheads=XH, drop_x=drop(0, KIND_XATTN), drop_e=drop(0, KIND_EMBD), cu=rw.cu)
            _ln_param_grads(parte, nbe, H, self.anw.g, self.anb.g)
            _bias_grad(ws, Bq, H, H, self.ob.g, x_f32=datt)
            dU_bf = self._buf("dU_bf", (Bq, XH, H), BF16)
            hip.cast_bf16(dU, dU_bf, Bq * XH * H)
            for h in range(XH):
                hip.gemm(dU_bf[:, h], s["vv"][:, h * dh:], H, dh, Bq, hip.TN, lda=XH * H, ldb=H,
                         out_f32=self.ow.g[:, h * dh:], ld_out_f32=H, accumulate=True)
                hip.gemm(dU_bf[:, h], self.ow.b[:, h * dh:], Bq, dh, H, hip.NN, lda=XH * H, ldb=H,
                         out_bf16=dvv[:, h * dh:], ld_out_bf16=H)
        hip.gemm(dvv, s["pv"], H, H, Bq, hip.TN, lda=H, ldb=H, out_f32=self.inw.g[2 * H:], accumulate=True)
        _bias_grad(ws, Bq, H, H, self.inb.g[2 * H:], x_bf16=dvv)
        dpv = self._buf("dpv", (Bq, H), BF16)
        hip.gemm(dvv, self.inw.b[2 * H:], Bq, H, H, hip.NN, epilogue=hip.EPI_DTANH, aux_in=s["pv_raw"], out_bf16=dpv,
                 drop=_dsite(drop, 0, KIND_VPROJ))
        hip.gemm(dpv, s["emb_bf"], H, Pd, Bq, hip.TN, lda=H, ldb=Pd, out_f32=self.vp_w.g, accumulate=True)
        _bias_grad(ws, Bq, H, H, self.vp_b.g, x_bf16=dpv)
        demb = self._buf("demb", (Bq, Pd), F32)
        hip.gemm(dpv, self.vp_w.b, Bq, Pd, H, hip.NN, out_f32=demb)
        return demb


class TextTowerEngine:

    def __init__(self, store: ParamStore, arch: ModelArch, ws: Workspace, tag: str):
        self.arch, self.ws, self.tag = arch, ws, tag
        t = "text_encoder.text_model"
        seg = store.seg_of(t + ".wte.weight")
        self.seg = seg
        self.trunk = GptTrunk(store, t, arch.gpt, ws, tag + ".trunk")
        self.wte, self.wpe = _P(seg, t + ".wte.weight"), _P(seg, t + ".wpe.weight")
        self.head = ProjHead(store, "text_encoder.projection", arch.gpt.hidden, arch.proj_dim, ws, tag + ".head")
        self.saved = None

    def _buf(self, name, shape, dtype, zero=False):
        return self.ws.get(f"{self.tag}.{name}", shape, dtype, zero)

    def forward(self, ids: torch.Tensor, mask: torch.Tensor, save: bool, drop=None, head_drop=None,
                pack: Optional[RowPack] = None):
        a = self.arch.gpt
        B, S = ids.shape
        H = a.hidden
        rw = _rows(pack, B, S)
        M = rw.M
        h0 = self._buf("h0", (M, H), F32)
        hip.embed_fwd(ids, B, S, H, self.wte.w, self.wpe.w, h0, drop_e=_dsite(drop, 0, KIND_EMBD), **rw.embed)
        hL = self.trunk.forward(h0, mask, B, S, save and self.seg.grad is not None, drop, pack=pack)
        feats = self._buf("feats", (M, H), F32)
        mf, rf = self._buf("mf", (M,), F32), self._buf("rf", (M,), F32)
        hip.layernorm_fwd(hL, M, H, self.trunk.lnf_w.w, self.trunk.lnf_b.w, a.eps, y_f32=feats, mean=mf, rstd=rf)
        pooled = self._buf("pooled", (B, H), F32)
        hip.masked_mean_fwd(feats, mask, B, S, H, pooled, cu=rw.cu)
        pooled_bf = self._buf("pooled_bf", (B, H), BF16)
        hip.cast_bf16(pooled, pooled_bf, B * H)
        emb = self.head.forward(pooled_bf, B, save, head_drop)
        if save:
            self.saved = dict(ids=ids, mask=mask, hL=hL, mf=mf, rf=rf, B=B, S=S, drop=drop, pack=pack)
        return (feats if pack is not None else feats.view(B, S, H)), pooled, emb

    def backward(self, demb: torch.Tensor) -> None:
        s, a, ws = self.saved, self.arch.gpt, self.ws
        B, S, H = s["B"], s["S"], a.hidden
        pack: Optional[RowPack] = s["pack"]
        rw = _rows(pack, B, S)
        M = rw.M
        if self.seg.grad is None:
            self.head.backward(demb, need_dx=False)
            return
        dpooled = self.head.backward(demb, need_dx=True)
        dfeats = self._buf("dfeats", (M, H), F32)
        hip.masked_mean_bwd(dpooled, s["mask"], B, S, H, dfeats, cu=rw.cu)
        if pack is not None and pack.Mp > pack.n:
            dfeats[pack.n:].zero_()
        g = self.trunk._buf("g_top", (M, H), F32)
        g_bf = self.trunk._buf("gbf_top", (M, H), BF16)
        nb = hip.layernorm_bwd_blocks(M)
        part = ws.get("ln_part_f", (2, nb, H), F32)
        hip.layernorm_bwd(s["hL"], M, H, self.trunk.lnf_w.w, s["mf"], s["rf"], g, dy_f32=dfeats, dx_bf16=g_bf, part=part,
                          drop_dx=self.trunk.top_drop(), drop_rows=rw.ids)
        _ln_param_grads(part, nb, H, self.trunk.lnf_w.g, self.trunk.lnf_b.g)
        g0 = self.trunk.backward(g, g_bf)
        hip.embed_bwd(g0, s["ids"], s["mask"], B, S, H, self.wte.g, self.wpe.g, drop_e=_dsite(s["drop"], 0, KIND_EMBD),
                      cu=rw.cu)


class NTXentEngine:

    def __init__(self, ws: Workspace, proj_dim: int, temperature: float, tag: str = "ntx"):
        self.ws, self.P, self.tau, self.tag = ws, proj_dim, float(temperature), tag
        if proj_dim % 8:
            raise ValueError("projection_dim must be a multiple of 8 (K alignment of the similarity GEMM)")
        self.saved = None
        self._consts = {}

    def _buf(self, name, shape, dtype, zero=False):
        return self.ws.get(f"{self.tag}.{name}", shape, dtype, zero)

    def normalize(self, emb: torch.Tensor, which: str):
        B, P = emb.shape
        y, n = self._buf(which + ".y", (B, P), F32), self._buf(which + ".n", (B,), F32)
        hip.l2norm_fwd(emb, B, P, y, n)
        return y, n

    def _stats(self, a_bf, b_all_bf, B, N, targets, which):
        nparts = 2 * ((N + 127) // 128)
        smax, ssum = self._buf(which + ".smax", (B, nparts), F32), self._buf(which + ".ssum", (B, nparts), F32)
        tval, lse = self._buf(which + ".tval", (B,), F32), self._buf(which + ".lse", (B,), F32)
        hip.gemm(a_bf, b_all_bf, B, N, 3 * self.P, hip.NT, epilogue=hip.EPI_ROWSTATS, alpha=1.0 / self.tau,
                 targets=targets, stat_max=smax, stat_sum=ssum, stat_ld=nparts, target_val=tval)
        hip.rowstats_combine(smax, ssum, nparts, nparts, tval, B, lse=lse)
        return lse, tval

    def forward(self, img_n: torch.Tensor, txt_n: torch.Tensor, img_all: Optional[torch.Tensor] = None,
                txt_all: Optional[torch.Tensor] = None, offset: int = 0):
        B, P = img_n.shape
        img_all = img_n if img_all is None else img_all
        txt_all = txt_n if txt_all is None else txt_all
        N = img_all.shape[0]
        bf = {}
        Np = (N + 7) // 8 * 8
        for k, t, rows, pattern in (("i", img_n, B, 0), ("t", txt_n, B, 0), ("ia", img_all, Np, 1), ("ta", txt_all, Np, 1)):
            bf[k] = self._buf("bf3." + k, (rows, 3 * P), BF16)
            hip.split_bf16(t, t.shape[0], P, rows, pattern, bf[k])
        tg = self.ws.cached(self.tag + ".targets", (B, offset),
                            lambda: (torch.arange(B, dtype=I64, device=self.ws.device) + offset).contiguous())
        lse_r, diag = self._stats(bf["i"], bf["ta"], B, N, tg, "r")
        lse_c, _ = self._stats(bf["t"], bf["ia"], B, N, tg, "c")
        loss = self._buf("loss", (1,), F32)
        hip.ntxent_loss(lse_r, lse_c, diag, B, N, loss)
        self.saved = dict(bf=bf, B=B, N=N, offset=offset, lse_r=lse_r, lse_c=lse_c, tg=tg)
        return loss, lse_r, lse_c

    def _const(self, name: str, n: int, value: float) -> torch.Tensor:
        key = (n, float(value))
        t = self._buf(name, (n,), F32)
        if self._consts.get(name) != key:
            t.fill_(value)
            self._consts[name] = key
        return t

    def backward(self, lse_r_all: Optional[torch.Tensor] = None, lse_c_all: Optional[torch.Tensor] = None,
                 loss_scale: float = 1.0):
        s, P = self.saved, self.P
        B, N, off, bf = s["B"], s["N"], s["offset"], s["bf"]
        lse_r_all = s["lse_r"] if lse_r_all is None else lse_r_all
        lse_c_all = s["lse_c"] if lse_c_all is None else lse_c_all
        c = loss_scale / (2.0 * N)
        inv_tau = 1.0 / self.tau
        Np = (N + 7) // 8 * 8
        Bp = (B + 7) // 8 * 8
        K3 = 3 * P
        cB = self._const("cB", B, c)
        cN = self._const("cN", N, c)
        def local_targets():
            j = torch.arange(N, dtype=I64, device=self.ws.device) - off
            return torch.where((j >= 0) & (j < B), j, torch.full_like(j, -1)).contiguous()
        tgN = self.ws.cached(self.tag + ".targetsN", (N, off, B), local_targets)
        def G(name, shape):
            return self._buf(name, shape, BF16), self._buf(name + "_lo", shape, BF16)
        g1, g1l = G("g1", (B, Np))
        g2, g2l = G("g2", (B, Np))
        hip.gemm(bf["i"], bf["ta"], B, N, K3, hip.NT, epilogue=hip.EPI_DLOGITS, alpha=inv_tau, targets=s["tg"],
                 row_lse=s["lse_r"], row_scale=cB, out_bf16=g1, ld_out_bf16=Np, out_cols=Np, aux_out=g1l, ld_aux=Np)
        hip.gemm(bf["t"], bf["ia"], B, N, K3, hip.NT, epilogue=hip.EPI_DLOGITS, alpha=inv_tau, targets=s["tg"],
                 row_lse=s["lse_c"], row_scale=cB, out_bf16=g2, ld_out_bf16=Np, out_cols=Np, aux_out=g2l, ld_aux=Np)
        g1t, g1tl = G("g1t", (N, Bp))
        g2t, g2tl = G("g2t", (N, Bp))
        hip.gemm(bf["ia"], bf["t"], N, B, K3, hip.NT, epilogue=hip.EPI_DLOGITS, alpha=inv_tau, targets=tgN,
                 row_lse=lse_r_all, row_scale=cN, out_bf16=g1t, ld_out_bf16=Bp, out_cols=Bp, aux_out=g1tl, ld_aux=Bp)
        hip.gemm(bf["ta"], bf["i"], N, B, K3, hip.NT, epilogue=hip.EPI_DLOGITS, alpha=inv_tau, targets=tgN,
                 row_lse=lse_c_all, row_scale=cN, out_bf16=g2t, ld_out_bf16=Bp, out_cols=Bp, aux_out=g2tl, ld_aux=Bp)
        dI = self._buf("dI", (B, P), F32)
        dT = self._buf("dT", (B, P), F32)
        first = True
        for part in (0, 1):
            ta, ia = bf["ta"][:, part * P:], bf["ia"][:, part * P:]
            for a1, a2t, b2, b1t in ((g1, g2t, g2, g1t), (g1l, g2tl, g2l, g1tl)):
                hip.gemm(a1, ta, B, P, Np, hip.NN, lda=Np, ldb=K3, alpha=inv_tau, out_f32=dI, accumulate=not first)
                hip.gemm(a2t, ta, B, P, N, hip.TN, lda=Bp, ldb=K3, alpha=inv_tau, out_f32=dI, accumulate=True)
                hip.gemm(b2, ia, B, P, Np, hip.NN, lda=Np, ldb=K3, alpha=inv_tau, out_f32=dT, accumulate=not first)
                hip.gemm(b1t, ia, B, P, N, hip.TN, lda=Bp, ldb=K3, alpha=inv_tau, out_f32=dT, accumulate=True)
                first = False
        return dI, dT
```

### preference-guided-image-captioning-alignment_amd/hip.py

```python
from __future__ import annotations

import ctypes as C
import os
from typing import Optional

import torch

_HERE = os.path.dirname(os.path.abspath(__file__))
LIB_PATH = os.environ.get("PGCA_LIB") or os.path.join(_HERE, "libpgca_hip.so")

NT, NN, TN = 0, 1, 2
EPI_NONE, EPI_GELU_NEW, EPI_QUICK_GELU, EPI_RELU, EPI_TANH = 0, 1, 2, 3, 4
EPI_DGELU_NEW, EPI_DRELU, EPI_DTANH, EPI_ROWSTATS, EPI_DLOGITS, EPI_DQUICK_GELU = 5, 6, 7, 8, 9, 10
EPI_GELU_NEW_D, EPI_MUL_AUX = 11, 12

_vp, _i32, _i64, _f32 = C.c_void_p, C.c_int32, C.c_int64, C.c_float


class GemmArgs(C.Structure):
    _fields_ = [
        ("A", _vp), ("B", _vp),
        ("M", _i32), ("N", _i32), ("K", _i32),
        ("lda", _i32), ("ldb", _i32),
        ("layout", _i32), ("epilogue", _i32),
        ("alpha", _f32),
        ("bias", _vp),
        ("out_bf16", _vp), ("ld_out_bf16", _i32),
        ("out_f32", _vp), ("ld_out_f32", _i32),
        ("accumulate", _i32),
        ("residual", _vp), ("ld_res", _i32),
        ("aux_out", _vp), ("aux_in", _vp), ("ld_aux", _i32),
        ("targets", _vp), ("stat_max", _vp), ("stat_sum", _vp), ("stat_ld", _i32),
        ("target_val", _vp), ("row_lse", _vp), ("row_scale", _vp),
        ("out_cols", _i32),
        ("drop_seed", C.c_uint32), ("drop_threshold", C.c_uint32), ("drop_scale", _f32),
        ("colsum_part", _vp), ("ld_colsum", _i32),
        ("drop_rows", _vp),
    ]


class SkinnyArgs(C.Structure):
    _fields_ = [
        ("x", _vp), ("W", _vp),
        ("M", _i32), ("N", _i32), ("K", _i32), ("lda", _i32), ("ldw", _i32),
        ("scratch", _vp), ("bias", _vp), ("act", _i32),
        ("residual", _vp), ("ld_res", _i32),
        ("out_f32", _vp), ("ld_out_f32", _i32),
        ("out_bf16", _vp), ("ld_out_bf16", _i32),
        ("ln_gamma", _vp), ("ln_beta", _vp), ("ln_eps", _f32),
        ("ln_out_bf16", _vp), ("ld_ln", _i32),
    ]


class SelectOpts(C.Structure):
    _fields_ = [("no_repeat_ngram_size", _i32), ("n_ban", _i32), ("ban_ids", _vp)]


SKINNY_MAX_M = 64

_SIGS = {
    "pgca_gemm_bf16": [C.POINTER(GemmArgs), _vp],
    "pgca_gemm_plan": [C.POINTER(GemmArgs)],
    "pgca_set_option": [C.c_char_p, _i32],
    "pgca_gemm_bf16_grouped": [C.POINTER(GemmArgs), _i32, _vp],
    "pgca_gemm_skinny": [C.POINTER(SkinnyArgs), _vp],
    "pgca_rowstats_combine": [_vp, _vp, _i32, _i32, _vp, _i32, _vp, _vp, _vp],
    "pgca_layernorm_fwd": [_vp, _vp, _i32, _i32, _vp, _vp, _f32, _vp, _vp, _vp, _vp, _vp],
    "pgca_layernorm_bwd_blocks": [_i32],
    "pgca_layernorm_bwd": [_vp, _vp, _vp, _vp, _i32, _i32, _vp, _vp, _vp, _vp, _vp, _vp, _vp, _vp, _vp, _vp, _vp, _vp],
    "pgca_colsum_finish": [_vp, _i32, _i32, _vp, _i32, _vp],
    "pgca_colsum_finish4": [_vp, _i32, _i32, _i32, _vp, _vp, _vp, _vp, _i32, _vp],
    "pgca_colsum_blocks": [_i32],
    "pgca_colsum": [_vp, _vp, _i32, _i32, _i32, _vp, _vp],
    "pgca_attention_fwd": [_vp, _vp, _i32, _i32, _i32, _i32, _vp, _vp, C.c_uint32, C.c_uint32, _f32, _vp, _vp],
    "pgca_attention_bwd": [_vp, _vp, _vp, _vp, _vp, _i32, _i32, _i32, _i32, _vp, C.c_uint32, C.c_uint32, _f32, _vp, _vp],
    "pgca_attention_bwd_split": [_vp, _vp, _vp, _vp, _vp, _i32, _i32, _i32, _i32, _vp, C.c_uint32, C.c_uint32, _f32, _vp,
                                 _vp],
    "pgca_embed_fwd": [_vp, _i32, _i32, _i32, _vp, _vp, _vp, _vp, _vp, _f32, _vp, _vp, _vp, _i32, _vp, _i32, _vp, _vp,
                       _vp, _i32, _vp],
    "pgca_embed_bwd": [_vp, _vp, _vp, _i32, _i32, _i32, _vp, _vp, _vp, _vp, _vp, _vp, _vp, _vp, _vp, _i32, _vp, _vp,
                       _i32, _vp, _vp, _vp, _vp],
    "pgca_embed_bwd_blocks": [_i32, _i32],
    "pgca_patchify": [_vp, _i32, _i32, _i32, _i32, _vp, _vp],
    "pgca_image_preprocess": [_vp, _i32, _i32, _i32, _i32, _vp, _vp, _i32, _vp, _vp, _i32, _f32, _f32, _f32, _f32, _f32, _f32,
                              _vp, _vp, _vp, _vp],
    "pgca_image_train_transform": [_vp, _i32, _i32, _i32, _i32, _vp, _vp, _vp, _vp, _i32, _vp, _vp, _i32, _f32, _f32, _f32,
                                   _f32, _f32, _f32, _vp, _vp, _vp, _vp, _vp],
    "pgca_vit_assemble": [_vp, _vp, _vp, _i32, _i32, _i32, _vp, _vp],
    "pgca_vit_assemble_bwd": [_vp, _i32, _i32, _i32, _vp, _vp, _vp, _vp],
    "pgca_seq_reduce": [_vp, _vp, _i32, _i32, _vp, _i32, _vp, _vp],
    "pgca_logits_logprob": [_vp, _i32, _i32, _vp, _vp, _i32, _vp, _vp],
    "pgca_logits_logprob_bwd": [_vp, _i32, _i32, _vp, _vp, _vp, _i32, _vp, _vp],
    "pgca_dpo_loss": [_vp, _vp, _vp, _vp, _i32, _f32, _f32, _vp, _vp, _vp, _vp, _vp],
    "pgca_row_scale": [_vp, _vp, _vp, _i32, _i32, _vp, _vp],
    "pgca_seq_batch_prepare": [_vp, _vp, _i32, _i32, _vp, _vp, _vp, _vp, _vp, _vp, _vp],
    "pgca_seq_pack_prepare": [_vp, _i32, _i32, _i32, _vp, _vp, _vp, _vp, _vp, _vp, _vp],
    "pgca_masked_mean_fwd": [_vp, _vp, _i32, _i32, _i32, _vp, _vp, _vp],
    "pgca_masked_mean_bwd": [_vp, _vp, _i32, _i32, _i32, _vp, _vp, _vp],
    "pgca_l2norm_fwd": [_vp, _i32, _i32, _vp, _vp, _vp],
    "pgca_l2norm_bwd": [_vp, _vp, _vp, _i32, _i32, _vp, _vp],
    "pgca_ntxent_loss": [_vp, _vp, _vp, _i32, _i32, _vp, _vp],
    "pgca_sqnorm_blocks": [_i64],
    "pgca_sqnorm": [_vp, _i64, _vp, _vp],
    "pgca_step_control": [_vp, _i32, _f32, _f32, _i32, _i32, _i32, _f32, _f32, _f32, _vp, _vp, _vp],
    "pgca_clip_coef": [_vp, _i32, _f32, _vp, _vp],
    "pgca_scale_dev": [_vp, _i64, _vp, _vp],
    "pgca_adamw": [_vp, _vp, _vp, _vp, _vp, _i64, _vp, _f32, _f32, _f32, _f32, _f32, _vp],
    "pgca_cast_bf16": [_vp, _vp, _i64, _vp],
    "pgca_cast_f32": [_vp, _vp, _i64, _vp],
    "pgca_split_bf16": [_vp, _i32, _i32, _i32, _i32, _vp, _vp],
    "pgca_axpy": [_vp, _f32, _vp, _i64, _i32, _vp],
    "pgca_gather_rows_bf16": [_vp, _vp, _i32, _i32, _vp, _vp],
    "pgca_select_token": [_vp, _i32, _i32, _i32, _vp, _i32, _i32, _f32, _f32, _i32, _f32, _vp, _vp, _i64, _vp, _vp, _vp],
    "pgca_select_beam_candidates": [_vp, _i32, _i32, _i32, _i32, _vp, _i32, _i32, _f32, _i32, _f32, _i32, _f32, _vp, _i32,
                                    _i32, C.c_uint32, _vp, _vp, _vp],
    "pgca_select_token_ex": [_vp, _i32, _i32, _i32, _vp, _i32, _i32, _f32, _f32, _i32, _f32, _vp, _vp, _i64, _vp, _vp,
                             C.POINTER(SelectOpts), _vp],
    "pgca_select_beam_candidates_ex": [_vp, _i32, _i32, _i32, _i32, _vp, _i32, _i32, _f32, _i32, _f32, _i32, _f32, _vp,
                                       _i32, _i32, C.c_uint32, _vp, _vp, C.POINTER(SelectOpts), _vp],
    "pgca_beam_step": [_vp, _vp, _i32, _i32, _i32, _i32, _i32, _i64, _f32, _i32, _vp, _vp, _vp, _vp, _vp, _vp, _vp, _vp,
                       _vp, _vp, _vp, _vp, _vp],
}
EXPORTS = ["pgca_version", "pgca_last_error", "pgca_sizeof_gemm_args", "pgca_sizeof_skinny_args",
           "pgca_sizeof_select_opts", "pgca_gemm_skinny_workspace"] + list(_SIGS)
ABI_VERSION = 306

_lib = None


def load() -> C.CDLL:
    global _lib
    if _lib is not None:
        return _lib
    if not os.path.exists(LIB_PATH):
        raise RuntimeError(
            f"{LIB_PATH} is missing: the MI355X path has no fallback. Build it with "
            "`python -m pgca_amd.build` (hipcc --offload-arch=gfx950).")
    lib = C.CDLL(LIB_PATH)
    lib.pgca_version.restype = C.c_int
    lib.pgca_last_error.restype = C.c_char_p
    if lib.pgca_version() != ABI_VERSION:
        raise RuntimeError(f"{LIB_PATH} has ABI version {lib.pgca_version()}, this binding expects {ABI_VERSION}: "
                           "rebuild it with `python -m pgca_amd.build --force`")
    lib.pgca_sizeof_gemm_args.restype = C.c_int
    if lib.pgca_sizeof_gemm_args() != C.sizeof(GemmArgs):
        raise RuntimeError(f"pgca_gemm_args is {lib.pgca_sizeof_gemm_args()} bytes in {LIB_PATH} but "
                           f"{C.sizeof(GemmArgs)} in the binding: stale library, rebuild it")
    lib.pgca_sizeof_skinny_args.restype = C.c_int
    if lib.pgca_sizeof_skinny_args() != C.sizeof(SkinnyArgs):
        raise RuntimeError(f"pgca_skinny_args is {lib.pgca_sizeof_skinny_args()} bytes in {LIB_PATH} but "
                           f"{C.sizeof(SkinnyArgs)} in the binding: stale library, rebuild it")
    lib.pgca_sizeof_select_opts.restype = C.c_int
    if lib.pgca_sizeof_select_opts() != C.sizeof(SelectOpts):
        raise RuntimeError(f"pgca_select_opts is {lib.pgca_sizeof_select_opts()} bytes in {LIB_PATH} but "
                           f"{C.sizeof(SelectOpts)} in the binding: stale library, rebuild it")
    lib.pgca_gemm_skinny_workspace.restype = C.c_int64
    lib.pgca_gemm_skinny_workspace.argtypes = [_i32, _i32, _i32]
    for name, sig in _SIGS.items():
        fn = getattr(lib, name)
        fn.argtypes = sig
        fn.restype = C.c_int
    _lib = lib
    return lib


def _check(rc: int, what: str) -> None:
    if rc != 0:
        raise RuntimeError(f"{what} failed ({rc}): {load().pgca_last_error().decode()}")


def _p(t: Optional[torch.Tensor]):
    return None if t is None else t.data_ptr()


def _stream():
    return torch.cuda.current_stream().cuda_stream


def _gemm_args(A: torch.Tensor, B: torch.Tensor, M: int, N: int, K: int, layout: int, *, lda: int = None,
               ldb: int = None, epilogue: int = EPI_NONE, alpha: float = 1.0, bias: torch.Tensor = None,
               out_bf16: torch.Tensor = None, ld_out_bf16: int = None, out_f32: torch.Tensor = None,
               ld_out_f32: int = None, accumulate: bool = False, residual: torch.Tensor = None, ld_res: int = None,
               aux_out: torch.Tensor = None, aux_in: torch.Tensor = None, ld_aux: int = None,
               targets: torch.Tensor = None, stat_max: torch.Tensor = None, stat_sum: torch.Tensor = None,
               stat_ld: int = 0, target_val: torch.Tensor = None, row_lse: torch.Tensor = None,
               row_scale: torch.Tensor = None, out_cols: int = 0, drop=None, colsum_part: torch.Tensor = None,
               drop_rows: torch.Tensor = None, into: GemmArgs = None) -> GemmArgs:
    a = GemmArgs() if into is None else into
    a.A, a.B = A.data_ptr(), B.data_ptr()
    a.M, a.N, a.K = M, N, K
    a.lda = lda if lda is not None else (K if layout != TN else M)
    a.ldb = ldb if ldb is not None else (K if layout == NT else N)
    a.layout, a.epilogue, a.alpha = layout, epilogue, alpha
    a.bias = _p(bias)
    a.out_bf16, a.ld_out_bf16 = _p(out_bf16), (ld_out_bf16 if ld_out_bf16 is not None else N)
    a.out_f32, a.ld_out_f32 = _p(out_f32), (ld_out_f32 if ld_out_f32 is not None else N)
    a.accumulate = 1 if accumulate else 0
    a.residual, a.ld_res = _p(residual), (ld_res if ld_res is not None else N)
    a.aux_out, a.aux_in, a.ld_aux = _p(aux_out), _p(aux_in), (ld_aux if ld_aux is not None else N)
    a.targets, a.stat_max, a.stat_sum, a.stat_ld = _p(targets), _p(stat_max), _p(stat_sum), stat_ld
    a.target_val, a.row_lse, a.row_scale = _p(target_val), _p(row_lse), _p(row_scale)
    a.out_cols = out_cols
    if drop is not None:
        a.drop_seed, a.drop_threshold, a.drop_scale = drop
        a.drop_rows = _p(drop_rows)
    if colsum_part is not None:
        a.colsum_part, a.ld_colsum = colsum_part.data_ptr(), colsum_part.shape[1]
    return a


def _probe_begin(first: GemmArgs):
    probe = gemm_probe
    if probe is None or not probe.want(first.layout, first.epilogue, load().pgca_gemm_plan(C.byref(first))):
        return None
    e0, e1 = torch.cuda.Event(enable_timing=True), torch.cuda.Event(enable_timing=True)
    e0.record()
    return probe, e0, e1


def _probe_end(bracket, flops: float) -> None:
    if bracket is not None:
        probe, e0, e1 = bracket
        e1.record()
        probe.add(e0, e1, flops)


def gemm(A: torch.Tensor, B: torch.Tensor, M: int, N: int, K: int, layout: int, **kw) -> None:
    a = _gemm_args(A, B, M, N, K, layout, **kw)
    bracket = _probe_begin(a)
    _check(load().pgca_gemm_bf16(C.byref(a), _stream()), "pgca_gemm_bf16")
    _probe_end(bracket, 2.0 * M * N * K)


def gemm_pair(g0, g1) -> None:
    arr = (GemmArgs * 2)()
    for a, (args, kw) in zip(arr, (g0, g1)):
        _gemm_args(*args, **kw, into=a)
    bracket = _probe_begin(arr[0])
    _check(load().pgca_gemm_bf16_grouped(arr, 2, _stream()), "pgca_gemm_bf16_grouped")
    _probe_end(bracket, sum(2.0 * a.M * a.N * a.K for a in arr))


def _wgrad_group_args(problems):
    arr = (GemmArgs * len(problems))()
    for a, (X, dY, M, N, K, gout) in zip(arr, problems):
        _gemm_args(X, dY, M, N, K, TN, out_f32=gout, accumulate=True, into=a)
    return arr


def gemm_wgrad_group(problems) -> None:
    _check(load().pgca_gemm_bf16_grouped(_wgrad_group_args(problems), len(problems), _stream()),
           "pgca_gemm_bf16_grouped")


def gemm_skinny(x, W, M, N, K, scratch, *, lda=None, ldw=None, bias=None, act=EPI_NONE, residual=None, ld_res=None,
                out_f32=None, ld_out_f32=None, out_bf16=None, ld_out_bf16=None, ln=None, ln_out=None, ld_ln=None):
    a = SkinnyArgs()
    a.x, a.W = x.data_ptr(), W.data_ptr()
    a.M, a.N, a.K = M, N, K
    a.lda, a.ldw = (K if lda is None else lda), (N if ldw is None else ldw)
    a.scratch, a.bias, a.act = scratch.data_ptr(), _p(bias), act
    a.residual, a.ld_res = _p(residual), (N if ld_res is None else ld_res)
    a.out_f32, a.ld_out_f32 = _p(out_f32), (N if ld_out_f32 is None else ld_out_f32)
    a.out_bf16, a.ld_out_bf16 = _p(out_bf16), (N if ld_out_bf16 is None else ld_out_bf16)
    if ln is not None:
        a.ln_gamma, a.ln_beta, a.ln_eps = ln[0].data_ptr(), ln[1].data_ptr(), float(ln[2])
        a.ln_out_bf16, a.ld_ln = ln_out.data_ptr(), (N if ld_ln is None else ld_ln)
    _check(load().pgca_gemm_skinny(C.byref(a), _stream()), "pgca_gemm_skinny")


def gemm_skinny_workspace(M: int, N: int, K: int) -> int:
    return int(load().pgca_gemm_skinny_workspace(M, N, K))


def drop_args(seed: int, p: float):
    if p <= 0.0:
        return None
    return (seed & 0xFFFFFFFF, min(0xFFFFFFFF, int(p * 4294967296.0)), 1.0 / (1.0 - p))


def set_option(name: str, value: int) -> None:
    _check(load().pgca_set_option(name.encode(), int(value)), "pgca_set_option")


gemm_probe = None


def rowstats_combine(stat_max, stat_sum, stat_ld, nparts, target_val, M, lse=None, out_logprob=None):
    _check(load().pgca_rowstats_combine(_p(stat_max), _p(stat_sum), stat_ld, nparts, _p(target_val), M, _p(lse),
                                        _p(out_logprob), _stream()), "pgca_rowstats_combine")


def layernorm_fwd(x, M, H, gamma, beta, eps=1e-5, row_map=None, y_bf16=None, y_f32=None, mean=None, rstd=None):
    _check(load().pgca_layernorm_fwd(_p(x), _p(row_map), M, H, _p(gamma), _p(beta), eps, _p(y_bf16), _p(y_f32),
                                     _p(mean), _p(rstd), _stream()), "pgca_layernorm_fwd")


def layernorm_bwd_blocks(M: int) -> int:
    return load().pgca_layernorm_bwd_blocks(M)


def layernorm_bwd(x, M, H, gamma, mean, rstd, dx_out, *, dy_bf16=None, dy_f32=None, row_map=None, add_to=None,
                  dx_bf16=None, part=None, part_extra=None, drop_add=None, drop_dx=None, drop_rows=None):
    _check(load().pgca_layernorm_bwd(_p(dy_bf16), _p(dy_f32), _p(x), _p(row_map), M, H, _p(gamma), _p(mean),
                                     _p(rstd), _p(add_to), _p(dx_out), _p(dx_bf16), _p(part), _p(part_extra),
                                     _drop_words(drop_add), _drop_words(drop_dx), _p(drop_rows), _stream()),
           "pgca_layernorm_bwd")


def colsum_finish(part, nparts, H, out, accumulate=False):
    _check(load().pgca_colsum_finish(_p(part), nparts, H, _p(out), 1 if accumulate else 0, _stream()),
           "pgca_colsum_finish")


def colsum_finish4(part, nplanes, nparts, H, outs, accumulate=False):
    o = list(outs) + [None] * (4 - len(outs))
    _check(load().pgca_colsum_finish4(_p(part), nplanes, nparts, H, _p(o[0]), _p(o[1]), _p(o[2]), _p(o[3]),
                                      1 if accumulate else 0, _stream()), "pgca_colsum_finish4")


def colsum_blocks(M: int) -> int:
    return load().pgca_colsum_blocks(M)


def colsum(M, N, ld, part, x_bf16=None, x_f32=None):
    _check(load().pgca_colsum(_p(x_bf16), _p(x_f32), M, N, ld, _p(part), _stream()), "pgca_colsum")


_NODROP = (0, 0, 1.0)


def _drop_words(d):
    if d is None:
        return None
    import struct
    arr = (C.c_uint32 * 3)(d[0], d[1], struct.unpack("<I", struct.pack("<f", d[2]))[0])
    return C.cast(arr, C.c_void_p)


def attention_fwd(qkv, key_mask, B, S, heads, causal, out, lse=None, drop=None, cu=None):
    d = drop or _NODROP
    _check(load().pgca_attention_fwd(_p(qkv), _p(key_mask), B, S, heads, 1 if causal else 0, _p(out), _p(lse),
                                     d[0], d[1], d[2], _p(cu), _stream()), "pgca_attention_fwd")


def attention_bwd(qkv, out, dout, lse, key_mask, B, S, heads, causal, dqkv, drop=None, cu=None):
    d = drop or _NODROP
    _check(load().pgca_attention_bwd(_p(qkv), _p(out), _p(dout), _p(lse), _p(key_mask), B, S, heads,
                                     1 if causal else 0, _p(dqkv), d[0], d[1], d[2], _p(cu), _stream()),
           "pgca_attention_bwd")


def attention_bwd_split(qkv, out, dout, lse, key_mask, B, S, heads, causal, dqkv, drop=None, cu=None):
    d = drop or _NODROP
    _check(load().pgca_attention_bwd_split(_p(qkv), _p(out), _p(dout), _p(lse), _p(key_mask), B, S, heads,
                                           1 if causal else 0, _p(dqkv), d[0], d[1], d[2], _p(cu), _stream()),
           "pgca_attention_bwd_split")


def embed_fwd(ids, B, S, H, wte, wpe, h0, attended=None, gamma=None, beta=None, eps=1e-5, mean=None, rstd=None,
              att_stride=None, U=None, xheads=0, drop_x=None, drop_e=None, row_ids=None, n_rows=0):
    _check(load().pgca_embed_fwd(_p(ids), B, S, H, _p(wte), _p(wpe), _p(attended), _p(gamma), _p(beta), eps, _p(h0),
                                 _p(mean), _p(rstd), H if att_stride is None else att_stride, _p(U), xheads,
                                 _drop_words(drop_x), _drop_words(drop_e), _p(row_ids), n_rows, _stream()),
           "pgca_embed_fwd")


def embed_bwd_blocks(B: int, S: int) -> int:
    return load().pgca_embed_bwd_blocks(B, S)


def embed_bwd(g, ids, row_mask, B, S, H, dwte, dwpe, wte=None, attended=None, gamma=None, mean=None, rstd=None,
              dattended=None, part=None, att_stride=None, U=None, dU=None, xheads=0, drop_x=None, drop_e=None,
              cu=None):
    _check(load().pgca_embed_bwd(_p(g), _p(ids), _p(row_mask), B, S, H, _p(wte), _p(attended), _p(gamma), _p(mean),
                                 _p(rstd), _p(dwte), _p(dwpe), _p(dattended), _p(part),
                                 H if att_stride is None else att_stride, _p(U), _p(dU), xheads, _drop_words(drop_x),
                                 _drop_words(drop_e), _p(cu), _stream()), "pgca_embed_bwd")


def patchify(pixels, B, image, patch, out_bf16, ld_out=None):
    ld = 3 * patch * patch if ld_out is None else ld_out
    _check(load().pgca_patchify(_p(pixels), B, image, patch, ld, _p(out_bf16), _stream()), "pgca_patchify")


def image_preprocess(images_u8, B, H, W, S, xbounds, xcoef, ybounds, ycoef, mean, std, tmp, out, resized_u8=None):
    _check(load().pgca_image_preprocess(_p(images_u8), B, H, W, S, _p(xbounds), _p(xcoef), xcoef.shape[1], _p(ybounds),
                                        _p(ycoef), ycoef.shape[1], mean[0], mean[1], mean[2], std[0], std[1], std[2],
                                        _p(tmp), _p(resized_u8), _p(out), _stream()), "pgca_image_preprocess")


def image_train_transform(images_u8, B, H, W, S, params, factors, xbounds, xcoef, ybounds, ycoef, mean, std, tmp, resized_u8,
                          out, aug_u8=None):
    _check(load().pgca_image_train_transform(_p(images_u8), B, H, W, S, _p(params), _p(factors), _p(xbounds), _p(xcoef),
                                             xcoef.shape[-1], _p(ybounds), _p(ycoef), ycoef.shape[-1], mean[0], mean[1],
                                             mean[2], std[0], std[1], std[2], _p(tmp), _p(resized_u8), _p(aug_u8), _p(out),
                                             _stream()), "pgca_image_train_transform")


def vit_assemble(patch_embeds, cls, pos, B, T, H, x):
    _check(load().pgca_vit_assemble(_p(patch_embeds), _p(cls), _p(pos), B, T, H, _p(x), _stream()),
           "pgca_vit_assemble")


def vit_assemble_bwd(dx, B, T, H, dpatch_bf16, dcls, dpos):
    _check(load().pgca_vit_assemble_bwd(_p(dx), B, T, H, _p(dpatch_bf16), _p(dcls), _p(dpos), _stream()),
           "pgca_vit_assemble_bwd")


def seq_reduce(tok_lp, seq_of_row, nrows, nseq, seq_count, mode, seq_lp):
    _check(load().pgca_seq_reduce(_p(tok_lp), _p(seq_of_row), nrows, nseq, _p(seq_count), mode, _p(seq_lp),
                                  _stream()), "pgca_seq_reduce")


def logits_logprob_bwd(logits, ld, V, row_map, targets, g, R, dlogits):
    _check(load().pgca_logits_logprob_bwd(_p(logits), ld, V, _p(row_map), _p(targets), _p(g), R, _p(dlogits), _stream()),
           "pgca_logits_logprob_bwd")


def logits_logprob(logits, ld, V, row_map, targets, R, out):
    _check(load().pgca_logits_logprob(_p(logits), ld, V, _p(row_map), _p(targets), R, _p(out), _stream()),
           "pgca_logits_logprob")


def _select_opts(no_repeat_ngram_size, ban_ids):
    n_ban = 0 if ban_ids is None else int(ban_ids.numel())
    return SelectOpts(int(no_repeat_ngram_size), n_ban, _p(ban_ids) if n_ban else None)


def select_token(logits, V, R, prev, n_prev, repetition_penalty, temperature, top_k, top_p, u, done, pad_id, next_ids,
                 next_logp, no_repeat_ngram_size=0, ban_ids=None):
    opts = _select_opts(no_repeat_ngram_size, ban_ids)
    _check(load().pgca_select_token_ex(_p(logits), logits.stride(0), V, R, _p(prev), prev.stride(0) if n_prev else 0,
                                       n_prev, repetition_penalty, temperature, top_k, top_p, _p(u), _p(done), pad_id,
                                       _p(next_ids), _p(next_logp), C.byref(opts), _stream()), "pgca_select_token_ex")


def select_beam_candidates(logits, V, B, nb, prev, n_prev, repetition_penalty, warp, temperature, top_k, top_p,
                           beam_scores, K, use_noise, noise_seed, cand_score, cand_index, no_repeat_ngram_size=0,
                           ban_ids=None):
    opts = _select_opts(no_repeat_ngram_size, ban_ids)
    _check(load().pgca_select_beam_candidates_ex(_p(logits), logits.stride(0), V, B, nb, _p(prev),
                                                 prev.stride(0) if n_prev else 0, n_prev, repetition_penalty, int(warp),
                                                 temperature, top_k, top_p, _p(beam_scores), K, int(use_noise),
                                                 noise_seed & 0xFFFFFFFF, _p(cand_score), _p(cand_index),
                                                 C.byref(opts), _stream()),
           "pgca_select_beam_candidates_ex")


EARLY_STOPPING = {False: 0, True: 1, "never": 2}


def beam_step(cand_score, cand_index, B, nb, V, cur, L, eos, length_penalty, early_stopping, running_in, running_out,
              running_beam_scores, sequences_in, sequences_out, beam_scores, is_sent_finished, gen_len, unsat, tok,
              flat_src, hits_all):
    _check(load().pgca_beam_step(_p(cand_score), _p(cand_index), B, nb, V, cur, L, eos, length_penalty,
                                 EARLY_STOPPING[early_stopping], _p(running_in), _p(running_out),
                                 _p(running_beam_scores), _p(sequences_in), _p(sequences_out), _p(beam_scores),
                                 _p(is_sent_finished), _p(gen_len), _p(unsat), _p(tok), _p(flat_src), _p(hits_all),
                                 _stream()), "pgca_beam_step")


def dpo_loss(pol_w, pol_l, ref_w, ref_l, B, beta, label_smoothing, loss, dpol_w=None, dpol_l=None, metrics=None):
    _check(load().pgca_dpo_loss(_p(pol_w), _p(pol_l), _p(ref_w), _p(ref_l), B, beta, label_smoothing, _p(loss),
                                _p(dpol_w), _p(dpol_l), _p(metrics), _stream()), "pgca_dpo_loss")


def seq_batch_prepare(ids, mask, Bq, S, counts, mask32, row_map, targets, seq_of_row, n_rows, stream=None):
    _check(load().pgca_seq_batch_prepare(_p(ids), _p(mask), Bq, S, _p(counts), _p(mask32), _p(row_map), _p(targets),
                                         _p(seq_of_row), _p(n_rows), _stream() if stream is None else stream),
           "pgca_seq_batch_prepare")


def seq_pack_prepare(mask32, Bq, S, pad_to, lens, cu, row_ids, n_packed, counts=None, row_map=None):
    _check(load().pgca_seq_pack_prepare(_p(mask32), Bq, S, pad_to, _p(lens), _p(cu), _p(row_ids), _p(n_packed),
                                        _p(counts), _p(row_map), _stream()), "pgca_seq_pack_prepare")


def row_scale(dseq, seq_of_row, seq_count, nrows, mode, out):
    _check(load().pgca_row_scale(_p(dseq), _p(seq_of_row), _p(seq_count), nrows, mode, _p(out), _stream()),
           "pgca_row_scale")


def masked_mean_fwd(feats, mask, B, S, H, pooled, cu=None):
    _check(load().pgca_masked_mean_fwd(_p(feats), _p(mask), B, S, H, _p(pooled), _p(cu), _stream()),
           "pgca_masked_mean_fwd")


def masked_mean_bwd(dpooled, mask, B, S, H, dfeats, cu=None):
    _check(load().pgca_masked_mean_bwd(_p(dpooled), _p(mask), B, S, H, _p(dfeats), _p(cu), _stream()),
           "pgca_masked_mean_bwd")


def l2norm_fwd(x, B, P, y, norm=None):
    _check(load().pgca_l2norm_fwd(_p(x), B, P, _p(y), _p(norm), _stream()), "pgca_l2norm_fwd")


def l2norm_bwd(dy, y, norm, B, P, dx):
    _check(load().pgca_l2norm_bwd(_p(dy), _p(y), _p(norm), B, P, _p(dx), _stream()), "pgca_l2norm_bwd")


def ntxent_loss(lse_r, lse_c, diag, n_local, n_total, loss):
    _check(load().pgca_ntxent_loss(_p(lse_r), _p(lse_c), _p(diag), n_local, n_total, _p(loss), _stream()),
           "pgca_ntxent_loss")


def sqnorm_blocks(n: int) -> int:
    return load().pgca_sqnorm_blocks(n)


def sqnorm(g, n, part):
    _check(load().pgca_sqnorm(_p(g), n, _p(part), _stream()), "pgca_sqnorm")


def step_control(part, nparts, max_norm, base_lr, warmup, total_steps, sched_stride, beta1, beta2, grad_scale, ctrl,
                 gate=None):
    _check(load().pgca_step_control(_p(part), nparts, max_norm, base_lr, warmup, total_steps, sched_stride, beta1,
                                    beta2, grad_scale, _p(gate), _p(ctrl), _stream()), "pgca_step_control")


def clip_coef(part, nparts, max_norm, coef):
    _check(load().pgca_clip_coef(_p(part), nparts, max_norm, _p(coef), _stream()), "pgca_clip_coef")


def scale_dev(x, n, coef):
    _check(load().pgca_scale_dev(_p(x), n, _p(coef), _stream()), "pgca_scale_dev")


def adamw(p, g, m, v, p_bf16, n, ctrl, weight_decay, beta1, beta2, eps, grad_scale=1.0):
    _check(load().pgca_adamw(_p(p), _p(g), _p(m), _p(v), _p(p_bf16), n, _p(ctrl), weight_decay, beta1, beta2, eps,
                             grad_scale, _stream()), "pgca_adamw")


def cast_bf16(x, y, n):
    _check(load().pgca_cast_bf16(_p(x), _p(y), n, _stream()), "pgca_cast_bf16")


def cast_f32(x_bf16, y, n):
    _check(load().pgca_cast_f32(_p(x_bf16), _p(y), n, _stream()), "pgca_cast_f32")


def split_bf16(x, R, P, rows_out, pattern, y):
    _check(load().pgca_split_bf16(_p(x), R, P, rows_out, pattern, _p(y), _stream()), "pgca_split_bf16")


def axpy(x, alpha, y, n, accumulate=False):
    _check(load().pgca_axpy(_p(x), alpha, _p(y), n, 1 if accumulate else 0, _stream()), "pgca_axpy")


def gather_rows_bf16(src, row_map, M, H, dst):
    _check(load().pgca_gather_rows_bf16(_p(src), _p(row_map), M, H, _p(dst), _stream()), "pgca_gather_rows_bf16")
```

Before: 2007 pairs/s.

## Split-K the partial last wave of 256-tile GEMMs with atomic-counter reduction

When a 256x256-tile GEMM has more tiles than CUs and a partial final wave, the leftover tail tiles are split along K across several workgroups. Each split writes its f32 partial accumulator to a global workspace slot and bumps a per-tile atomic counter. The last arriving split sums all partials and runs the normal epilogue. A cost model picks the split count. The aim is to fill idle CUs during the tail wave, at the cost of extra global traffic, a workspace buffer per stream, and fence/atomic synchronisation.

```diff
diff --git a/include/pgca_hip.h b/include/pgca_hip.h
--- a/include/pgca_hip.h
+++ b/include/pgca_hip.h
@@ -70,10 +70,15 @@
   float* colsum_part;
   int32_t ld_colsum;
   const int32_t* drop_rows;
+  void* tail_ws;
+  int64_t tail_ws_bytes;
 } pgca_gemm_args;
+#define PGCA_GEMM_TAIL_WS_HEADER 4096
+#define PGCA_GEMM_TAIL_SLOT_BYTES 262144
 
 int pgca_gemm_bf16(const pgca_gemm_args* args, void* stream);
 int pgca_gemm_plan(const pgca_gemm_args* args);
+int pgca_gemm_tail_plan(const pgca_gemm_args* args, int32_t* tail_tiles, int32_t* splits);
 int pgca_set_option(const char* name, int32_t value);
 int pgca_gemm_bf16_grouped(const pgca_gemm_args* args, int32_t count, void* stream);
 
diff --git a/preference-guided-image-captioning-alignment_amd/csrc/gemm.hip b/preference-guided-image-captioning-alignment_amd/csrc/gemm.hip
--- a/preference-guided-image-captioning-alignment_amd/csrc/gemm.hip
+++ b/preference-guided-image-captioning-alignment_amd/csrc/gemm.hip
@@ -99,7 +99,8 @@
 
 template <int LA, int LB, bool RAW = false>
 __device__ __forceinline__ void gemm256_body(const pgca_gemm_args& a, int ntm, int ntn, int nk_per_split, int bid_in,
-                                             int ksplit, unsigned char* smem2) {
+                                             int ksplit, int tail_tt, int tail_split, int tail_s,
+                                             unsigned char* smem2) {
   int tm, tn;
   if (RAW) {
     tm = bid_in / ntn;
@@ -170,6 +171,16 @@
   }
 
   TSTAMP(ts2);
+  if (tail_s > 1 && tail_split >= 0) {
+    const bool last = tail_meet(a, acc, tail_tt, tail_split, tail_s, smem2 + TAIL_FLAG_LDS);
+#ifdef PGCA_GEMM_TIMING
+    TSTAMP(ts3);
+    if (a.stat_sum && a.epilogue != PGCA_EPI_ROWSTATS && lane == 0)
+      a.stat_sum[((size_t)blockIdx.x * 8 + wave) * 8 + (last ? 1 : 0)] = (float)(ts3 - ts2);
+    ts2 = ts3;
+#endif
+    if (!last) return;
+  }
   run_epilogue(a, acc[0], smem2, m0 + wm * 128, n0 + wn * 64, lane, wave);
   run_epilogue(a, acc[1], smem2, m0 + wm * 128 + 64, n0 + wn * 64, lane, wave);
 #ifdef PGCA_GEMM_TIMING
@@ -183,9 +194,13 @@
 }
 
 template <int LA, int LB>
-__global__ __launch_bounds__(512, 2) void gemm256_kernel(const pgca_gemm_args a, int ntm, int ntn, int nk_per_split) {
+__global__ __launch_bounds__(512, 2) void gemm256_kernel(const pgca_gemm_args a, int ntm, int ntn, int nk_per_split,
+                                                         const TailCut tc) {
   extern __shared__ __attribute__((aligned(16))) unsigned char smem2[];
-  gemm256_body<LA, LB>(a, ntm, ntn, nk_per_split, blockIdx.x, blockIdx.y, smem2);
+  int tt, split;
+  const int b = tail_place(tc, blockIdx.x, tt, split);
+  gemm256_body<LA, LB>(a, ntm, ntn, split >= 0 ? tc.nk : nk_per_split, b, split >= 0 ? split : (int)blockIdx.y, tt, split,
+                       tc.s, smem2);
 }
 
 struct pgca_group_param {
@@ -229,7 +244,7 @@
     tm = l / ntn;
     tn = l - tm * ntn;
   }
-  gemm256_body<1, 1, true>(a, ntm, ntn, a.K / BK, tm * ntn + tn, 0, smem2);
+  gemm256_body<1, 1, true>(a, ntm, ntn, a.K / BK, tm * ntn + tn, 0, 0, -1, 1, smem2);
 }
 
 constexpr size_t GEMM256_LDS = 4 * TILE2_BYTES;
@@ -255,9 +270,50 @@
     v.group = env("PGCA_GEMM_NO_GROUP", 0) ? 0 : 1;
     v.stagger = env("PGCA_GEMM_STAGGER", 0);
     v.pair_order = 0;
+    v.tail_split = env("PGCA_GEMM_TAIL_SPLIT", 1) ? 1 : 0;
+    v.tail_force = 0;
     return v;
   }();
   return t;
+}
+
+namespace {
+struct TailModel {
+  int P, L, E;
+  int W0, W1;
+  int F0, F1;
+};
+constexpr TailModel TAIL_MODEL[2] = {
+    {4500, 3000, 11000, 7000, 24000, 3000, 5000},
+    {4500, 3200, 11000, 7000, 24000, 3000, 5000},
+};
+constexpr int TAIL_MIN_NK = 8, TAIL_MAX_SPLITS = 16;
+
+void plan_tail(const pgca_gemm_args& a, GemmPlan& p) {
+  const int T = p.ntm * p.ntn, Tt = T % GEMM_CUS, nk = p.nk_per_split;
+  if (T <= GEMM_CUS || Tt == 0) return;
+  p.tail_tiles = Tt;
+  if (!gemm_tuning().tail_split || !a.tail_ws || ((uintptr_t)a.tail_ws & 15) || Tt > PGCA_GEMM_TAIL_WS_HEADER / 4) return;
+  const long long slots = (a.tail_ws_bytes - PGCA_GEMM_TAIL_WS_HEADER) / PGCA_GEMM_TAIL_SLOT_BYTES;
+  const TailModel& m = TAIL_MODEL[p.variant == 6 ? 0 : 1];
+  const long long uncut = m.P + (long long)nk * m.L + m.E;
+  long long best = uncut - uncut / 10;
+  const int force = gemm_tuning().tail_force;
+  for (int s = 2; s <= (force ? force : TAIL_MAX_SPLITS); ++s) {
+    const int per = (nk + s - 1) / s;
+    if (per < TAIL_MIN_NK || (long long)Tt * s > slots) break;
+    if ((nk + per - 1) / per != s) continue;
+    const int wgs = Tt * s, rounds = (wgs + GEMM_CUS - 1) / GEMM_CUS;
+    const long long W = m.W0 + (long long)m.W1 * (wgs < GEMM_CUS ? wgs : GEMM_CUS) / GEMM_CUS;
+    const long long F = m.F0 + (long long)s * m.F1 * (GEMM_CUS + Tt) / GEMM_CUS;
+    const long long cut = rounds * (m.P + (long long)per * m.L + W) + F + m.E;
+    if (cut < best || force) {
+      best = cut;
+      p.tail_splits = s;
+      p.tail_nk = per;
+    }
+  }
+}
 }
 
 GemmPlan plan_gemm(const pgca_gemm_args& a) {
@@ -270,7 +326,7 @@
   const bool splittable = a.epilogue == PGCA_EPI_NONE && a.accumulate && a.out_f32 && !a.out_bf16 && !a.bias &&
                           !a.residual;
   if (splittable && ntm2 * ntn2 > 0 && ntm2 * ntn2 < 192) {
-    splits = 256 / (ntm2 * ntn2);
+    splits = GEMM_CUS / (ntm2 * ntn2);
     if (splits > nk_total / 8) splits = nk_total / 8;
     if (splits > 16) splits = 16;
     if (splits < 1) splits = 1;
@@ -292,6 +348,10 @@
     p.ntn = (p.ncols + BN - 1) / BN;
     p.nk_per_split = (a.K + BK - 1) / BK;
   }
+  p.tail_tiles = 0;
+  p.tail_splits = 1;
+  p.tail_nk = p.nk_per_split;
+  if (p.tile == 256 && p.splits == 1) plan_tail(a, p);
   return p;
 }
 }
@@ -308,6 +368,8 @@
   else if (n == "gemm_group" && (value == 0 || value == 1)) t.group = value;
   else if (n == "gemm_stagger" && value >= 0 && value <= 64) t.stagger = value;
   else if (n == "gemm_pair_order" && (value == 0 || value == 1)) t.pair_order = value;
+  else if (n == "gemm_tail_split" && (value == 0 || value == 1)) t.tail_split = value;
+  else if (n == "gemm_tail_force" && (value == 0 || (value >= 2 && value <= TAIL_MAX_SPLITS))) t.tail_force = value;
   else {
     set_error("pgca_set_option: unknown option or value out of range (%s = %d)", name, value);
     return PGCA_ERR_INVALID;
@@ -319,6 +381,17 @@
   const GemmPlan p = plan_gemm(*args);
   if (p.tile != 256) return 12801;
   return p.variant * 1000000 + 25600 + p.splits;
+}
+
+extern "C" int pgca_gemm_tail_plan(const pgca_gemm_args* args, int32_t* tail_tiles, int32_t* splits) {
+  if (!args || !tail_tiles || !splits) {
+    set_error("pgca_gemm_tail_plan: null argument");
+    return PGCA_ERR_INVALID;
+  }
+  const GemmPlan p = plan_gemm(*args);
+  *tail_tiles = p.tail_tiles;
+  *splits = p.tail_splits;
+  return PGCA_OK;
 }
 
 static int check_gemm_args(const pgca_gemm_args& a) {
@@ -391,8 +464,9 @@
   return with_layout(a.layout, [&](auto la, auto lb) {
     constexpr auto kernel = gemm256_kernel<decltype(la)::value, decltype(lb)::value>;
     if (raise_lds_limit<kernel>(GEMM256_LDS, "gemm256")) return (int)PGCA_ERR_LAUNCH;
-    hipLaunchKernelGGL(kernel, dim3(p.ntm * p.ntn, p.grid_y), dim3(512), GEMM256_LDS, s, b, p.ntm, p.ntn,
-                       p.nk_per_split);
+    const TailCut tc = {p.ntm * p.ntn - p.tail_tiles, p.tail_splits, p.tail_nk};
+    hipLaunchKernelGGL(kernel, dim3(tc.full + p.tail_tiles * tc.s, p.grid_y), dim3(512), GEMM256_LDS, s, b, p.ntm, p.ntn,
+                       p.nk_per_split, tc);
     return check_launch("pgca_gemm_bf16(256)");
   });
 }
diff --git a/preference-guided-image-captioning-alignment_amd/csrc/gemm_device.h b/preference-guided-image-captioning-alignment_amd/csrc/gemm_device.h
--- a/preference-guided-image-captioning-alignment_amd/csrc/gemm_device.h
+++ b/preference-guided-image-captioning-alignment_amd/csrc/gemm_device.h
@@ -14,6 +14,7 @@
   int nk_per_split;
   int grid_y;
   int ncols;
+  int tail_tiles, tail_splits, tail_nk;
 };
 GemmPlan plan_gemm(const pgca_gemm_args& a);
 int launch_gemm256s(const pgca_gemm_args& a, const GemmPlan& p, void* stream);
@@ -25,6 +26,8 @@
   int group;
   int pair_order;
   int stagger;
+  int tail_force;
+  int tail_split;
 };
 GemmTuning& gemm_tuning();
 }
@@ -62,6 +65,7 @@
 constexpr int BM2 = 256, BN2 = 256;
 constexpr int TILE2_BYTES = 256 * 64 * 2;
 constexpr unsigned OOB = 0x80000000u;
+constexpr int GEMM_CUS = 256;
 
 __device__ __forceinline__ int xcd_remap(int b, int total) {
   const int xcd = b & 7, q = total >> 3, r = total & 7;
@@ -215,6 +219,62 @@
 
 __device__ __forceinline__ void dma_wait() { asm volatile("s_waitcnt vmcnt(0)" ::: "memory"); }
 
+struct TailCut {
+  int full, s, nk;
+};
+__device__ __forceinline__ int tail_place(const TailCut& tc, int b, int& tt, int& split) {
+  tt = 0;
+  split = -1;
+  if (tc.s > 1 && b >= tc.full) {
+    const int r = b - tc.full;
+    tt = r / tc.s;
+    split = r - tt * tc.s;
+    b = tc.full + tt;
+  }
+  return b;
+}
+
+constexpr size_t TAIL_SLOT_F32X4 = (size_t)BM2 * BN2 / 4;
+__device__ __forceinline__ bool tail_meet(const pgca_gemm_args& a, f32x4 (&acc)[2][4][4], int tt, int split, int s,
+                                          unsigned char* lds) {
+  const int t = threadIdx.x;
+  unsigned* counter = reinterpret_cast<unsigned*>(a.tail_ws) + tt;
+  f32x4* slots = reinterpret_cast<f32x4*>(reinterpret_cast<unsigned char*>(a.tail_ws) + PGCA_GEMM_TAIL_WS_HEADER) +
+                 (size_t)tt * s * TAIL_SLOT_F32X4 + t;
+  f32x4* mine = slots + (size_t)split * TAIL_SLOT_F32X4;
+#pragma unroll
+  for (int h = 0; h < 2; ++h)
+#pragma unroll
+    for (int i = 0; i < 4; ++i)
+#pragma unroll
+      for (int j = 0; j < 4; ++j) mine[((h * 4 + i) * 4 + j) * 512] = acc[h][i][j];
+  __builtin_amdgcn_fence(__ATOMIC_RELEASE, "agent");
+  __syncthreads();
+  unsigned* flag = reinterpret_cast<unsigned*>(lds);
+  if (t == 0) *flag = __hip_atomic_fetch_add(counter, 1u, __ATOMIC_ACQ_REL, __HIP_MEMORY_SCOPE_AGENT);
+  __syncthreads();
+  if (__builtin_amdgcn_readfirstlane(*flag) != (unsigned)(s - 1)) return false;
+  __builtin_amdgcn_fence(__ATOMIC_ACQUIRE, "agent");
+#pragma unroll
+  for (int h = 0; h < 2; ++h)
+#pragma unroll
+    for (int i = 0; i < 4; ++i)
+#pragma unroll
+      for (int j = 0; j < 4; ++j) acc[h][i][j] = (f32x4){0.f, 0.f, 0.f, 0.f};
+  for (int k = 0; k < s; ++k) {
+    const f32x4* p = slots + (size_t)k * TAIL_SLOT_F32X4;
+#pragma unroll
+    for (int h = 0; h < 2; ++h)
+#pragma unroll
+      for (int i = 0; i < 4; ++i)
+#pragma unroll
+        for (int j = 0; j < 4; ++j) acc[h][i][j] += p[((h * 4 + i) * 4 + j) * 512];
+  }
+  if (t == 0) __hip_atomic_store(counter, 0u, __ATOMIC_RELAXED, __HIP_MEMORY_SCOPE_AGENT);
+  return true;
+}
+constexpr int TAIL_FLAG_LDS = 8 * 4096;
+
 template <int LA>
 __device__ __forceinline__ void mma_half(const unsigned char* la, int row0, int kk, int lane, const bf16x8 (&fb)[4],
                                          f32x4 (&acc)[4][4]) {
diff --git a/preference-guided-image-captioning-alignment_amd/csrc/gemm_pair.hip b/preference-guided-image-captioning-alignment_amd/csrc/gemm_pair.hip
--- a/preference-guided-image-captioning-alignment_amd/csrc/gemm_pair.hip
+++ b/preference-guided-image-captioning-alignment_amd/csrc/gemm_pair.hip
@@ -31,7 +31,7 @@
   const pgca_gemm_args a = *(const pgca_gemm_args*)(kernarg + offsetof(pgca_pair_param, a) +
                                                     (p ? sizeof(pgca_gemm_args) : 0));
   if (a.epilogue > PGCA_EPI_TANH && a.epilogue != PGCA_EPI_GELU_NEW_D) return;
-  gemm256s_body<LA, LB>(a, ntm, ntn, gp.nk, gp.stagger, bid, smems);
+  gemm256s_body<LA, LB>(a, ntm, ntn, gp.nk, 0, gp.stagger, bid, 0, -1, 1, smems);
 }
 
 }
@@ -48,7 +48,7 @@
   gp.ntm = p.ntm;
   gp.ntn = p.ntn;
   gp.nk = p.nk_per_split;
-  gp.stagger = 2 * p.ntm * p.ntn >= 3 * 256 ? gemm_tuning().stagger : 0;
+  gp.stagger = 2 * p.ntm * p.ntn >= 3 * GEMM_CUS ? gemm_tuning().stagger : 0;
   gp.order = gemm_tuning().pair_order;
   auto launch = [&](auto lb) {
     constexpr auto kernel = gemm256s_pair_kernel<0, decltype(lb)::value>;
diff --git a/preference-guided-image-captioning-alignment_amd/csrc/gemm_phase.hip b/preference-guided-image-captioning-alignment_amd/csrc/gemm_phase.hip
--- a/preference-guided-image-captioning-alignment_amd/csrc/gemm_phase.hip
+++ b/preference-guided-image-captioning-alignment_amd/csrc/gemm_phase.hip
@@ -4,9 +4,12 @@
 
 template <int LA, int LB>
 __global__ __launch_bounds__(512, 2) void gemm256s_kernel(const pgca_gemm_args a, int ntm, int ntn, int nk_per_split,
-                                                          int stagger) {
+                                                          int stagger, const TailCut tc) {
   extern __shared__ __attribute__((aligned(16))) unsigned char smems[];
-  gemm256s_body<LA, LB>(a, ntm, ntn, nk_per_split, stagger, xcd_remap(blockIdx.x, ntm * ntn), smems);
+  int tt, split;
+  const int b = tail_place(tc, blockIdx.x, tt, split);
+  gemm256s_body<LA, LB>(a, ntm, ntn, split >= 0 ? tc.nk : nk_per_split, split >= 0 ? split : (int)blockIdx.y, stagger,
+                        xcd_remap(b, ntm * ntn), tt, split, tc.s, smems);
 }
 
 }
@@ -15,9 +18,10 @@
   return with_layout(a.layout, [&](auto la, auto lb) {
     constexpr auto kernel = gemm256s_kernel<decltype(la)::value, decltype(lb)::value>;
     if (raise_lds_limit<kernel>(GEMM256S_LDS, "gemm256s")) return (int)PGCA_ERR_LAUNCH;
-    const int stagger = (p.ntm * p.ntn >= 3 * 256 && p.grid_y == 1) ? gemm_tuning().stagger : 0;
-    hipLaunchKernelGGL(kernel, dim3(p.ntm * p.ntn, p.grid_y), dim3(512), GEMM256S_LDS, (hipStream_t)stream, a, p.ntm,
-                       p.ntn, p.nk_per_split, stagger);
+    const int stagger = (p.ntm * p.ntn >= 3 * GEMM_CUS && p.grid_y == 1) ? gemm_tuning().stagger : 0;
+    const TailCut tc = {p.ntm * p.ntn - p.tail_tiles, p.tail_splits, p.tail_nk};
+    hipLaunchKernelGGL(kernel, dim3(tc.full + p.tail_tiles * tc.s, p.grid_y), dim3(512), GEMM256S_LDS,
+                       (hipStream_t)stream, a, p.ntm, p.ntn, p.nk_per_split, stagger, tc);
     return check_launch("pgca_gemm_bf16(256 phase-staggered)");
   });
 }
diff --git a/preference-guided-image-captioning-alignment_amd/csrc/gemm_phase_body.h b/preference-guided-image-captioning-alignment_amd/csrc/gemm_phase_body.h
--- a/preference-guided-image-captioning-alignment_amd/csrc/gemm_phase_body.h
+++ b/preference-guided-image-captioning-alignment_amd/csrc/gemm_phase_body.h
@@ -47,15 +47,16 @@
   } while (0)
 
 template <int LA, int LB>
-__device__ __forceinline__ void gemm256s_body(const pgca_gemm_args& a, int ntm, int ntn, int nk_per_split, int stagger,
-                                              int bid, unsigned char* smems) {
+__device__ __forceinline__ void gemm256s_body(const pgca_gemm_args& a, int ntm, int ntn, int nk_per_split, int ksplit,
+                                              int stagger, int bid, int tail_tt, int tail_split, int tail_s,
+                                              unsigned char* smems) {
 #ifdef PGCA_GEMM_TIMING
   unsigned long long ts0, ts1, ts2, ts3, tr0, tr3;
 #endif
   TSTAMP(ts0);
   TSTAMP_REAL(tr0);
 
-  if (stagger > 0 && gridDim.y == 1 && blockIdx.x < 256) {
+  if (stagger > 0 && gridDim.y == 1 && blockIdx.x < GEMM_CUS) {
     const int slot = (blockIdx.x >> 3) & 3;
     for (int i = 0; i < slot * stagger; ++i) __builtin_amdgcn_s_sleep(16);
   }
@@ -89,7 +90,7 @@
 #pragma unroll
       for (int j = 0; j < 4; ++j) acc[h][i][j] = (f32x4){0.f, 0.f, 0.f, 0.f};
 
-  const int kt0 = blockIdx.y * nk_per_split * 2;
+  const int kt0 = ksplit * nk_per_split * 2;
   const int nk = min(nk_per_split * 2, a.K / PBK - kt0);
   abase += (size_t)kt0 * astep;
   bbase += (size_t)kt0 * bstep;
@@ -193,6 +194,16 @@
   __syncthreads();
 
   TSTAMP(ts2);
+  if (tail_s > 1 && tail_split >= 0) {
+    const bool last = tail_meet(a, acc, tail_tt, tail_split, tail_s, smems + TAIL_FLAG_LDS);
+#if defined(PGCA_GEMM_TIMING) && !defined(PGCA_GEMM_TIMING2)
+    TSTAMP(ts3);
+    if (a.stat_sum && a.epilogue != PGCA_EPI_ROWSTATS && lane == 0)
+      a.stat_sum[((size_t)blockIdx.x * 8 + wave) * 8 + (last ? 1 : 0)] = (float)(ts3 - ts2);
+    ts2 = ts3;
+#endif
+    if (!last) return;
+  }
   run_epilogue(a, acc[0], smems, m0 + wm * 128, n0 + wn * 64, lane, wave);
   run_epilogue(a, acc[1], smems, m0 + wm * 128 + 64, n0 + wn * 64, lane, wave);
 #ifdef PGCA_GEMM_TIMING
diff --git a/preference-guided-image-captioning-alignment_amd/engine.py b/preference-guided-image-captioning-alignment_amd/engine.py
--- a/preference-guided-image-captioning-alignment_amd/engine.py
+++ b/preference-guided-image-captioning-alignment_amd/engine.py
@@ -59,6 +59,15 @@
         if zero:
             v.zero_()
         return v
+
+    def gemm_tail(self, M: int, N: int) -> Optional[torch.Tensor]:
+        if ((M + 255) // 256) * ((N + 255) // 256) <= 256 or self.device.type != "cuda":
+            return None
+        key = f"gemm_tail.{torch.cuda.current_stream().cuda_stream}"
+        t = self.bufs.get(key)
+        if t is None:
+            t = self.bufs[key] = torch.zeros(hip.tail_ws_bytes(), dtype=torch.uint8, device=self.device)
+        return t
 
     def cached(self, key: str, stamp: tuple, make) -> torch.Tensor:
         fresh = key not in self.bufs or self._stamps.get(key) != stamp
@@ -320,13 +329,13 @@
     keys: frozenset = frozenset()
 
 
-def _drive(steps):
+def _drive(steps, ws: "Workspace"):
     while True:
         try:
             args, kw = next(steps)
         except StopIteration as e:
             return e.value
-        hip.gemm(*args, **kw)
+        hip.gemm(*args, **kw, tail_ws=ws.gemm_tail(args[2], args[3]))
 
 
 def _drive_pair(steps0, steps1):
@@ -385,7 +394,7 @@
 
     def forward(self, h0: torch.Tensor, mask: Optional[torch.Tensor], Bq: int, S: int, save: bool,
                 drop=None, pack: Optional[RowPack] = None) -> torch.Tensor:
-        return _drive(self.forward_steps(h0, mask, Bq, S, save, drop, pack))
+        return _drive(self.forward_steps(h0, mask, Bq, S, save, drop, pack), self.ws)
 
     def forward_steps(self, h0: torch.Tensor, mask: Optional[torch.Tensor], Bq: int, S: int, save: bool,
                       drop=None, pack: Optional[RowPack] = None):
@@ -423,7 +432,7 @@
         return (f"rc{li & 1}." if name in self._WGRAD_OPERANDS else "rc.") + name
 
     def _layer_fwd(self, *args, **kw):
-        return _drive(self._layer_steps(*args, **kw))
+        return _drive(self._layer_steps(*args, **kw), self.ws)
 
     def _layer_steps(self, li: int, h: torch.Tensor, rw: SimpleNamespace, mask, S: int, drop, save: bool,
                      hn: Optional[torch.Tensor] = None, hm: Optional[torch.Tensor] = None, proj: bool = True):
@@ -544,6 +553,7 @@
         drop = sv["drop"]
         L = len(self.layers)
         main = torch.cuda.current_stream()
+        tail = ws.gemm_tail(M, H)
         side = None
         if self.overlap_wgrad and g.is_cuda:
             if self._wgrad_stream is None:
@@ -567,11 +577,11 @@
             nbr = (M + 63) // 64
             dpre_cs = self._buf("dpre_colsum", (nbr, I), F32)
             hip.gemm(g_bf, P["wpr"].b, M, I, H, hip.NT, epilogue=hip.EPI_MUL_AUX if self.GELU_PAIR else hip.EPI_DGELU_NEW,
-                     aux_in=s["pre"], out_bf16=dpre, colsum_part=dpre_cs)
+                     aux_in=s["pre"], out_bf16=dpre, colsum_part=dpre_cs, tail_ws=tail)
             hip.colsum_finish(dpre_cs, nbr, I, P["bfc"].g, accumulate=True)
             wgrads = [(s["act"], g_bf, I, H, M, P["wpr"].g)]
             dln = self._buf("dln", (M, H), BF16)
-            hip.gemm(dpre, P["wfc"].b, M, H, I, hip.NT, out_bf16=dln)
+            hip.gemm(dpre, P["wfc"].b, M, H, I, hip.NT, out_bf16=dln, tail_ws=tail)
             wgrads.append((s["ln2"], dpre, H, I, M, P["wfc"].g))
             g2 = self._buf("g_b" if (li & 1) else "g_a", (M, H), F32)
             g2_bf = self._buf("gbf_b" if (li & 1) else "gbf_a", (M, H), BF16)
@@ -580,12 +590,12 @@
                               drop_dx=_dsite(drop, li, KIND_RESID_ATTN), drop_rows=rw.ids)
             _ln_param_grads(part4, nb, H, P["ln2w"].g, P["ln2b"].g, P["bpr"].g, P["bo"].g)
             datt = self._buf("datt", (M, H), BF16)
-            hip.gemm(g2_bf, P["wo"].b, M, H, H, hip.NT, out_bf16=datt)
+            hip.gemm(g2_bf, P["wo"].b, M, H, H, hip.NT, out_bf16=datt, tail_ws=tail)
             wgrads.append((s["att"], g2_bf, H, H, M, P["wo"].g))
             dqkv = self._buf("dqkv" + par, (M, 3 * H), BF16)
             attention_backward(s["qkv"], s["att"], datt, s["lse"], sv["mask"], rw.nseq, S, a.heads, True, dqkv,
                                drop=_dsite(drop, li, KIND_ATTN), cu=rw.cu)
-            hip.gemm(dqkv, P["wqkv"].b, M, H, 3 * H, hip.NT, out_bf16=dln)
+            hip.gemm(dqkv, P["wqkv"].b, M, H, 3 * H, hip.NT, out_bf16=dln, tail_ws=tail)
             wgrads.append((s["ln1"], dqkv, H, 3 * H, M, P["wqkv"].g))
             if side is not None:
                 side.wait_stream(main)
@@ -739,7 +749,8 @@
             hip.gemm(y2, P["w1"].b, M, a.mlp, H, hip.NT, epilogue=hip.EPI_QUICK_GELU, bias=P["b1"].w, out_bf16=act,
                      aux_out=pre)
             xn = ws.get(f"vit.l{li + 1}.xin", (M, H), F32) if save else x
-            hip.gemm(act, P["w2"].b, M, H, a.mlp, hip.NT, bias=P["b2"].w, residual=xm, out_f32=xn)
+            hip.gemm(act, P["w2"].b, M, H, a.mlp, hip.NT, bias=P["b2"].w, residual=xm, out_f32=xn,
+                     tail_ws=self.ws.gemm_tail(M, H))
             if save:
                 sv[li] = dict(xin=x, y1=y, qkv=qkv, att=att, act=act, m1=m1, r1=r1, m2=m2, r2=r2, lse=lse, xm=xm, y2=y2,
                               pre=pre)
@@ -1068,7 +1079,8 @@
                      row_lse=s["lse"][r0:r0 + n], row_scale=rs[r0:r0 + n], out_bf16=dl, ld_out_bf16=self.Vp,
                      out_cols=self.Vp)
             hip.gemm(dl, self.wte_pad_bf, n, H, self.Vp, hip.NN, lda=self.Vp, ldb=H, out_f32=dhf[r0:r0 + n], accumulate=True)
-            hip.gemm(dl, hfc, self.V, H, n, hip.TN, lda=self.Vp, ldb=H, out_f32=self.wte.g, accumulate=True)
+            hip.gemm(dl, hfc, self.V, H, n, hip.TN, lda=self.Vp, ldb=H, out_f32=self.wte.g, accumulate=True,
+                     tail_ws=ws.gemm_tail(self.V, H))
         g = self.trunk._buf("g_top", (M, H), F32, zero=True)
         g_bf = self.trunk._buf("gbf_top", (M, H), BF16, zero=True)
         nb = hip.layernorm_bwd_blocks(Mc)
diff --git a/preference-guided-image-captioning-alignment_amd/hip.py b/preference-guided-image-captioning-alignment_amd/hip.py
--- a/preference-guided-image-captioning-alignment_amd/hip.py
+++ b/preference-guided-image-captioning-alignment_amd/hip.py
@@ -36,6 +36,7 @@
         ("drop_seed", C.c_uint32), ("drop_threshold", C.c_uint32), ("drop_scale", _f32),
         ("colsum_part", _vp), ("ld_colsum", _i32),
         ("drop_rows", _vp),
+        ("tail_ws", _vp), ("tail_ws_bytes", _i64),
     ]
 
 
@@ -61,6 +62,7 @@
 _SIGS = {
     "pgca_gemm_bf16": [C.POINTER(GemmArgs), _vp],
     "pgca_gemm_plan": [C.POINTER(GemmArgs)],
+    "pgca_gemm_tail_plan": [C.POINTER(GemmArgs), C.POINTER(_i32), C.POINTER(_i32)],
     "pgca_set_option": [C.c_char_p, _i32],
     "pgca_gemm_bf16_grouped": [C.POINTER(GemmArgs), _i32, _vp],
     "pgca_gemm_skinny": [C.POINTER(SkinnyArgs), _vp],
@@ -185,7 +187,7 @@
                targets: torch.Tensor = None, stat_max: torch.Tensor = None, stat_sum: torch.Tensor = None,
                stat_ld: int = 0, target_val: torch.Tensor = None, row_lse: torch.Tensor = None,
                row_scale: torch.Tensor = None, out_cols: int = 0, drop=None, colsum_part: torch.Tensor = None,
-               drop_rows: torch.Tensor = None, into: GemmArgs = None) -> GemmArgs:
+               drop_rows: torch.Tensor = None, tail_ws: torch.Tensor = None, into: GemmArgs = None) -> GemmArgs:
     a = GemmArgs() if into is None else into
     a.A, a.B = A.data_ptr(), B.data_ptr()
     a.M, a.N, a.K = M, N, K
@@ -206,7 +208,23 @@
         a.drop_rows = _p(drop_rows)
     if colsum_part is not None:
         a.colsum_part, a.ld_colsum = colsum_part.data_ptr(), colsum_part.shape[1]
+    if tail_ws is not None:
+        a.tail_ws, a.tail_ws_bytes = tail_ws.data_ptr(), tail_ws.numel() * tail_ws.element_size()
     return a
+
+
+TAIL_WS_HEADER, TAIL_SLOT_BYTES = 4096, 262144
+
+
+def tail_ws_bytes(slots: int = 256) -> int:
+    return TAIL_WS_HEADER + slots * TAIL_SLOT_BYTES
+
+
+def gemm_tail_plan(A=None, B=None, M=0, N=0, K=0, layout=NT, args: GemmArgs = None, **kw):
+    a = args if args is not None else _gemm_args(A, B, M, N, K, layout, **kw)
+    tt, s = _i32(0), _i32(0)
+    _check(load().pgca_gemm_tail_plan(C.byref(a), C.byref(tt), C.byref(s)), "pgca_gemm_tail_plan")
+    return tt.value, s.value
 
 
 def _probe_begin(first: GemmArgs):
```

Result: no change. 1992 pairs/s (-0.8%).
